# JunweiLiang/Multiverse

Measured on NVIDIA H100. Metric: trajectories/sec (obs8->pred12, K=20), higher is better.
Workload: dtype f32

## Files before the change

### include/multiverse_b200.h

```cpp
#ifndef MULTIVERSE_B200_H_
#define MULTIVERSE_B200_H_

#include <stdint.h>

#ifdef __cplusplus
extern "C" {
#endif

const char* mvb_last_error(void);
int mvb_abi_version(void);
long long mvb_launch_count(void);
void mvb_reset_launch_count(void);


int mvb_cell_cpad(int cx);

#define MVB_PLANES_F16F8 16
int mvb_pack_cell_weights(const float* kernel, const float* biases, void* w_planes,
                          float* bias_packed, int cx, int planes, int comp, void* stream);
int mvb_cell_last_variant(void);
long long mvb_cell_variants_seen(int reset);

int mvb_convlstm_cell_fwd(const void* xh_planes, const void* w_planes, const float* bias_packed,
                          const float* c_in, const int32_t* row_map, float* c_out, float* h32_out,
                          void* hp_out, int64_t hp_plane_stride, int cpad_out, int ch_off_out,
                          int64_t NS, int H, int W, int cpad, int planes, float forget_bias,
                          void* stream);

int mvb_cell_xfold_tables(const float* kernel, const float* biases, const float* We, const float* be,
                          int E, float* table_B, float* table_T2, void* stream);
int mvb_convlstm_cell_fwd_onehot(const void* xh_planes, const void* w_planes, const float* table_B,
                                 const float* table_T2, const int32_t* ids, const float* c_in,
                                 const int32_t* row_map, float* c_out, float* h32_out, void* hp_out,
                                 int64_t hp_plane_stride, int cpad_out, int ch_off_out, int64_t NS, int H,
                                 int W, int cpad, int planes, float forget_bias, void* stream);
int mvb_convlstm_cell_fwd_xdense(const void* xh_planes, const void* w_planes, const float* bias_packed,
                                 const float* x_in, const float* x_weights, const float* c_in, float* c_out,
                                 float* h32_out, void* hp_out, int64_t hp_plane_stride, int cpad_out, int ch_off_out,
                                 int64_t NS, int H, int W, int cpad, int planes, float forget_bias, void* stream);
int mvb_cell_xdense_weights(const float* kernel_tf, float* x_weights, void* stream);
int mvb_convlstm_cell_fwd_xsparse(const void* xh_planes, const void* w_planes, const float* bias_packed,
                                  const float* x_table, const int32_t* label, const float* c_in, float* c_out,
                                  float* h32_out, void* hp_out, int64_t hp_plane_stride, int cpad_out, int ch_off_out,
                                  int64_t NS, int H, int W, int cpad, int planes, float forget_bias, void* stream);
int mvb_cell_xsparse_weights(const float* kernel_tf, int cx, float* x_weights, void* stream);
int mvb_cell_xsparse_table(const float* scene_conv, const int32_t* frame_idx, const int32_t* label,
                           const float* x_weights, float* x_table, int64_t NS, int H, int W, void* stream);

int mvb_convlstm_cell_fwd_onehot_fanout(const void* xh_planes, const void* w_planes, const float* table_B,
                                        const float* table_T2, const int32_t* ids, const float* c_in,
                                        float* c_out, float* h32_out, float* workspace, int64_t NS, int fanout,
                                        int H, int W, int cpad, int planes, float forget_bias, void* stream);


int mvb_convlstm_cell_fwd_train(const void* xh_planes, const void* w_planes,
                                const float* bias_packed, const float* c_in, float* c_out,
                                float* h32_out, void* hp_out, int64_t hp_plane_stride, int cpad_out,
                                int ch_off_out, float* gates_out, int64_t NS, int H, int W, int cpad,
                                int planes, float forget_bias, void* stream);
int mvb_lstm_gates_bwd(const float* gates, const float* c_prev, const float* c_new, const float* dh,
                       const float* dc_in, void* dg_planes, int64_t plane_stride, float* dc_prev,
                       float* dbias_packed, int64_t NS, int H, int W, int planes, void* stream);
int mvb_pack_cell_weights_dgrad(const float* kernel, void* wd_planes, int cx, int planes,
                                void* stream);
int mvb_cell_dgrad(const void* dg_planes, const void* wd_planes, float* dxh, int64_t NS, int H,
                   int W, int cpad, int planes, int need_dx, void* stream);
int mvb_cell_wgrad_direct(const void* dg_planes, const void* xh_planes, float* dw_packed, int64_t NS,
                          int H, int W, int cpad, int planes, void* stream);
int mvb_unpack_cell_wgrad(const float* dw_packed, const float* dbias_packed, float* dkernel,
                          float* dbiases, int cx, int comp, int accumulate, int slabs, void* stream);
int mvb_cell_wgrad_slabs(int cpad);

int mvb_loss_fwd_bwd(const float* logits, const int32_t* labels, float* dlogits, int64_t rows, int V,
                     float cls_weight, const float* reg, const float* target, float* dreg,
                     int64_t nreg, float reg_weight, float* loss_out, void* stream);
int mvb_soft_ce_fwd_bwd(const float* logits, const float* labels, float* dlogits, int64_t rows, int V,
                        float cls_weight, float* loss_out, void* stream);
int mvb_fg_count(const float* soft_labels, const int32_t* labels, int64_t rows, int V, double* fg_count,
                 void* stream);
int mvb_masked_huber_fwd_bwd(const float* reg, const float* target, float* dreg, const float* soft_labels,
                             const int32_t* labels, int64_t rows, int V, const double* fg_count, float reg_weight,
                             float* loss_out, void* stream);
int mvb_head_bwd(const float* h32, const float* dout, const float* Wo, int Pout, float* dWo,
                 float* dh, int accumulate_dh, int64_t NS, int H, int W, void* stream);
int mvb_emb_bwd(const float* dxh, int cpad, const int32_t* ids, const float* in_map, const float* We,
                const float* be, int E, int Pout, float* dWe, float* dbe, float* d_in,
                int accumulate_din, int64_t NS, int H, int W, void* stream);
int mvb_gnn_attend_bwd(const float* h32, const float* scene_mean, const float* gout, float* work,
                       float* dh, int accumulate_dh, float* dscene_mean, int64_t NS, int H, int W,
                       void* stream);
int mvb_scene_conv_bwd(const float* in, const float* W, const float* out, const float* dout,
                       float* dW, float* db, float* din, int64_t F, int IH, int IW, int Cin, int Cout,
                       void* stream);
int mvb_enc_class_input_bwd(const float* dxh, int cpad, const int32_t* frame_idx,
                            const int32_t* label, float* dscene, int64_t NS, int H, int W,
                            void* stream);
int mvb_scene_time_mean_bwd(const float* dmean, const int32_t* frame_idx, float* dscene, int64_t N,
                            int T, int64_t HWC, void* stream);
int mvb_clip_adadelta(float* w, const float* grad, float* acc, float* acc_upd, int64_t n, float lr,
                      float rho, float eps, float clip, float wd, float grad_scale, void* stream);


int mvb_nhwc_to_planes(const float* src, void* dst_planes, int64_t plane_stride, int cpad,
                       int ch_off, int64_t NS, int H, int W, int C, int planes, int comp,
                       void* stream);
int mvb_nhwc_to_halo(const float* src, float* dst, int64_t NS, int H, int W, int C, void* stream);
int mvb_halo_to_nhwc(const float* src, float* dst, int64_t NS, int H, int W, int C, void* stream);

int mvb_enc_class_input(const float* scene_conv, const int32_t* frame_idx, const int32_t* label,
                        const int32_t* prev_label, void* xh_planes, int64_t plane_stride, int cpad,
                        int64_t NS, int H, int W, int planes, void* stream);

int mvb_scene_conv_fwd(const float* in, const float* W, const float* b, float* out, int64_t F,
                       int IH, int IW, int Cin, int Cout, void* stream);
int mvb_scene_time_mean(const float* scene_conv, const int32_t* frame_idx, float* out, int64_t N,
                        int T, int64_t HWC, void* stream);

int mvb_gnn_attend_fwd(const float* h32, const int32_t* row_map, const float* scene_mean,
                       int beam, void* hp_out, int64_t hp_plane_stride, int cpad_out,
                       int ch_off_out, int64_t NS, int H, int W, int planes, void* stream);

int mvb_head_class_fwd(const float* h32, const float* Wo, float* logits_out, int32_t* ids_out,
                       const float* We, const float* be, int E, void* xh_next,
                       int64_t plane_stride, int cpad, int64_t NS, int H, int W, int planes,
                       void* stream);
int mvb_head_class_fwd_dense(const float* h32, const float* Wo, float* logits_out, int32_t* ids_out,
                             const float* We, const float* be, int E, void* xh_next, int64_t plane_stride, int cpad,
                             int64_t NS, int H, int W, int planes, void* stream);
int mvb_head_reg_fwd(const float* h32, const float* Wo, float* off_out, const float* We,
                     const float* be, int E, void* xh_next, int64_t plane_stride, int cpad,
                     int64_t NS, int H, int W, int planes, void* stream);
int mvb_emb_onehot_fwd(const int32_t* ids, const float* We, const float* be, int E, void* xh_next,
                       int64_t plane_stride, int cpad, int64_t NS, int H, int W, int planes,
                       void* stream);
int mvb_emb_dense_fwd(const float* x, const float* We, const float* be, int E, void* xh_next,
                      int64_t plane_stride, int cpad, int64_t NS, int H, int W, int planes,
                      void* stream);

int mvb_beam_step(const float* logits, const float* score_in, float* score_out, int32_t* ids_out,
                  int32_t* parents_out, int32_t* row_map_out, int64_t N, int B, int V,
                  int first_step, int zero_scores, int diverse, float log_gamma, void* stream);
int mvb_clip_update(float* w, const float* grad, float* slot1, float* slot2, int64_t n, int kind, float lr, float p1,
                    float p2, float eps, float clip, float wd, float grad_scale, void* stream);

int mvb_adv_step(const float* x, const float* adv, const float* grad, float* out, float eps, float step, int64_t n,
                 void* stream);
int mvb_mix(const float* a, const float* b, float* out, float w, int64_t n, void* stream);
int mvb_ce_rows(const float* logits, const int32_t* labels, float* loss, int64_t rows, int V, void* stream);
int mvb_enc_class_input_mix(const float* scene_conv, const int32_t* frame_idx, const int32_t* label,
                            const int32_t* label2, float beta, void* xh_planes, int64_t plane_stride, int cpad,
                            int64_t NS, int H, int W, int planes, void* stream);
int mvb_enc_class_input_mix_bwd(const float* dxh, int cpad, const int32_t* frame_idx, const int32_t* label,
                                const int32_t* label2, float beta, float* dscene, int64_t NS, int H, int W,
                                void* stream);

int mvb_min_ade_fde(const float* pred, const float* gt, const int32_t* gt_len, double* ade_err, int32_t* ade_idx,
                    double* fde, int32_t* fde_idx, int64_t N, int G, int K, int Tp, int Tg, void* stream);
int mvb_beam_nll(const float* logits, const float* logprobs, const int32_t* gt_idx, const int32_t* steps, double* nll,
                 int32_t* count, int64_t N, int K, int Tp, int V, int J, int G, void* stream);

int mvb_beam_backtrace(const int32_t* step_ids, const int32_t* step_parents,
                       const float* step_logits, int32_t* out_ids, float* out_logits, int64_t N,
                       int B, int Tp, int V, void* stream);

int mvb_beam_gather_h_f16f8(const float* h32, const int32_t* row_map, void* hp_out, int64_t hp_plane_stride,
                            int cpad_out, int64_t NS, int H, int W, void* stream);

int mvb_traj_to_grid(const double* traj, const double* centers, double h_gap, double w_gap, int32_t* labels,
                     float* regress, int64_t NT, int H, int W, void* stream);

int mvb_decode_trajectories(const int32_t* ids, const float* offsets, const float* centers, float* out,
                            int64_t N, int K, int Tp, int V, void* stream);

#ifdef __cplusplus
}
#endif
#endif
```

### multiverse_b200/_lib.py

```python
from __future__ import annotations

import ctypes as C
import os

_HERE = os.path.dirname(os.path.abspath(__file__))
LIB_PATH = os.path.join(_HERE, "libmultiverse_b200.so")

_vp, _i, _i64, _f = C.c_void_p, C.c_int, C.c_int64, C.c_float

SIGNATURES = {
    "mvb_last_error": [],
    "mvb_abi_version": [],
    "mvb_launch_count": [],
    "mvb_reset_launch_count": [],
    "mvb_cell_cpad": [_i],
    "mvb_cell_last_variant": [],
    "mvb_cell_variants_seen": [_i],
    "mvb_pack_cell_weights": [_vp, _vp, _vp, _vp, _i, _i, _i, _vp],
    "mvb_convlstm_cell_fwd": [_vp, _vp, _vp, _vp, _vp, _vp, _vp, _vp, _i64, _i, _i, _i64, _i, _i,
                              _i, _i, _f, _vp],
    "mvb_cell_xfold_tables": [_vp, _vp, _vp, _vp, _i, _vp, _vp, _vp],
    "mvb_convlstm_cell_fwd_xdense": [_vp, _vp, _vp, _vp, _vp, _vp, _vp, _vp, _vp, _i64, _i, _i, _i64, _i, _i,
                                     _i, _i, _f, _vp],
    "mvb_cell_xdense_weights": [_vp, _vp, _vp],
    "mvb_convlstm_cell_fwd_xsparse": [_vp, _vp, _vp, _vp, _vp, _vp, _vp, _vp, _vp, _i64, _i, _i, _i64, _i, _i,
                                      _i, _i, _f, _vp],
    "mvb_cell_xsparse_weights": [_vp, _i, _vp, _vp],
    "mvb_cell_xsparse_table": [_vp, _vp, _vp, _vp, _vp, _i64, _i, _i, _vp],
    "mvb_convlstm_cell_fwd_onehot_fanout": [_vp, _vp, _vp, _vp, _vp, _vp, _vp, _vp, _vp, _i64, _i, _i, _i, _i, _i, _f, _vp],
    "mvb_convlstm_cell_fwd_onehot": [_vp, _vp, _vp, _vp, _vp, _vp, _vp, _vp, _vp, _vp, _i64, _i, _i, _i64,
                                     _i, _i, _i, _i, _f, _vp],
    "mvb_convlstm_cell_fwd_train": [_vp, _vp, _vp, _vp, _vp, _vp, _vp, _i64, _i, _i, _vp, _i64, _i, _i,
                                    _i, _i, _f, _vp],
    "mvb_lstm_gates_bwd": [_vp, _vp, _vp, _vp, _vp, _vp, _i64, _vp, _vp, _i64, _i, _i, _i, _vp],
    "mvb_pack_cell_weights_dgrad": [_vp, _vp, _i, _i, _vp],
    "mvb_cell_dgrad": [_vp, _vp, _vp, _i64, _i, _i, _i, _i, _i, _vp],
    "mvb_cell_wgrad_direct": [_vp, _vp, _vp, _i64, _i, _i, _i, _i, _vp],
    "mvb_unpack_cell_wgrad": [_vp, _vp, _vp, _vp, _i, _i, _i, _i, _vp],
    "mvb_cell_wgrad_slabs": [_i],
    "mvb_loss_fwd_bwd": [_vp, _vp, _vp, _i64, _i, _f, _vp, _vp, _vp, _i64, _f, _vp, _vp],
    "mvb_soft_ce_fwd_bwd": [_vp, _vp, _vp, _i64, _i, _f, _vp, _vp],
    "mvb_fg_count": [_vp, _vp, _i64, _i, _vp, _vp],
    "mvb_masked_huber_fwd_bwd": [_vp, _vp, _vp, _vp, _vp, _i64, _i, _vp, _f, _vp, _vp],
    "mvb_head_bwd": [_vp, _vp, _vp, _i, _vp, _vp, _i, _i64, _i, _i, _vp],
    "mvb_emb_bwd": [_vp, _i, _vp, _vp, _vp, _vp, _i, _i, _vp, _vp, _vp, _i, _i64, _i, _i, _vp],
    "mvb_gnn_attend_bwd": [_vp, _vp, _vp, _vp, _vp, _i, _vp, _i64, _i, _i, _vp],
    "mvb_scene_conv_bwd": [_vp, _vp, _vp, _vp, _vp, _vp, _vp, _i64, _i, _i, _i, _i, _vp],
    "mvb_enc_class_input_bwd": [_vp, _i, _vp, _vp, _vp, _i64, _i, _i, _vp],
    "mvb_scene_time_mean_bwd": [_vp, _vp, _vp, _i64, _i, _i64, _vp],
    "mvb_clip_adadelta": [_vp, _vp, _vp, _vp, _i64, _f, _f, _f, _f, _f, _f, _vp],
    "mvb_nhwc_to_planes": [_vp, _vp, _i64, _i, _i, _i64, _i, _i, _i, _i, _i, _vp],
    "mvb_nhwc_to_halo": [_vp, _vp, _i64, _i, _i, _i, _vp],
    "mvb_halo_to_nhwc": [_vp, _vp, _i64, _i, _i, _i, _vp],
    "mvb_enc_class_input": [_vp, _vp, _vp, _vp, _vp, _i64, _i, _i64, _i, _i, _i, _vp],
    "mvb_scene_conv_fwd": [_vp, _vp, _vp, _vp, _i64, _i, _i, _i, _i, _vp],
    "mvb_scene_time_mean": [_vp, _vp, _vp, _i64, _i, _i64, _vp],
    "mvb_gnn_attend_fwd": [_vp, _vp, _vp, _i, _vp, _i64, _i, _i, _i64, _i, _i, _i, _vp],
    "mvb_head_class_fwd": [_vp, _vp, _vp, _vp, _vp, _vp, _i, _vp, _i64, _i, _i64, _i, _i, _i, _vp],
    "mvb_head_class_fwd_dense": [_vp, _vp, _vp, _vp, _vp, _vp, _i, _vp, _i64, _i, _i64, _i, _i, _i, _vp],
    "mvb_head_reg_fwd": [_vp, _vp, _vp, _vp, _vp, _i, _vp, _i64, _i, _i64, _i, _i, _i, _vp],
    "mvb_emb_onehot_fwd": [_vp, _vp, _vp, _i, _vp, _i64, _i, _i64, _i, _i, _i, _vp],
    "mvb_emb_dense_fwd": [_vp, _vp, _vp, _i, _vp, _i64, _i, _i64, _i, _i, _i, _vp],
    "mvb_beam_step": [_vp, _vp, _vp, _vp, _vp, _vp, _i64, _i, _i, _i, _i, _i, _f, _vp],
    "mvb_traj_to_grid": [_vp, _vp, C.c_double, C.c_double, _vp, _vp, _i64, _i, _i, _vp],
    "mvb_decode_trajectories": [_vp, _vp, _vp, _vp, _i64, _i, _i, _i, _vp],
    "mvb_clip_update": [_vp, _vp, _vp, _vp, _i64, _i, _f, _f, _f, _f, _f, _f, _f, _vp],
    "mvb_adv_step": [_vp, _vp, _vp, _vp, _f, _f, _i64, _vp],
    "mvb_ce_rows": [_vp, _vp, _vp, _i64, _i, _vp],
    "mvb_enc_class_input_mix": [_vp, _vp, _vp, _vp, _f, _vp, _i64, _i, _i64, _i, _i, _i, _vp],
    "mvb_enc_class_input_mix_bwd": [_vp, _i, _vp, _vp, _vp, _f, _vp, _i64, _i, _i, _vp],
    "mvb_mix": [_vp, _vp, _vp, _f, _i64, _vp],
    "mvb_min_ade_fde": [_vp, _vp, _vp, _vp, _vp, _vp, _vp, _i64, _i, _i, _i, _i, _vp],
    "mvb_beam_nll": [_vp, _vp, _vp, _vp, _vp, _vp, _i64, _i, _i, _i, _i, _i, _vp],
    "mvb_beam_backtrace": [_vp, _vp, _vp, _vp, _vp, _i64, _i, _i, _i, _vp],
    "mvb_beam_gather_h_f16f8": [_vp, _vp, _vp, _i64, _i, _i64, _i, _i, _vp],
}
_RESTYPES = {"mvb_last_error": C.c_char_p, "mvb_launch_count": C.c_longlong, "mvb_cell_variants_seen": C.c_longlong,
             "mvb_reset_launch_count": None}

_lib = None


def load():
  global _lib
  if _lib is not None:
    return _lib
  if not os.path.exists(LIB_PATH):
    raise RuntimeError(
        "libmultiverse_b200.so is not built (%s). Run `python -m multiverse_b200.build`; "
        "there is no CPU or PyTorch fallback for the hot path." % LIB_PATH)
  lib = C.CDLL(LIB_PATH)
  for name, args in SIGNATURES.items():
    fn = getattr(lib, name)
    fn.argtypes = args
    fn.restype = _RESTYPES.get(name, C.c_int)
  _lib = lib
  return lib


def check(rc, what):
  if rc != 0:
    msg = load().mvb_last_error()
    raise RuntimeError("%s failed (code %d): %s" % (what, rc, msg.decode() if msg else "?"))


def call(name, *args):
  check(getattr(load(), name)(*args), name)
```

### multiverse_b200/csrc/mvb_api.cu

```cuda
#include "mvb_common.cuh"
#include "mvb_kernels.h"
#include "../../include/multiverse_b200.h"

#include <string.h>

namespace mvb {

static thread_local char g_err[512] = "";
static thread_local long long g_launches = 0;

void set_error(const char* fmt, ...) {
  va_list ap;
  va_start(ap, fmt);
  vsnprintf(g_err, sizeof(g_err), fmt, ap);
  va_end(ap);
}
const char* get_error() { return g_err; }
void count_launch(int n) { g_launches += n; }

typedef CUresult (*EncodeTiledFn)(CUtensorMap*, CUtensorMapDataType, cuuint32_t, void*,
                                  const cuuint64_t*, const cuuint64_t*, const cuuint32_t*,
                                  const cuuint32_t*, CUtensorMapInterleave, CUtensorMapSwizzle,
                                  CUtensorMapL2promotion, CUtensorMapFloatOOBfill);

// ... 13 lines not shown
}

static int encode_tmap_3d_any(CUtensorMapDataType dt, CUtensorMap* out, const void* base, uint64_t d0, uint64_t d1, uint64_t d2,
                        uint64_t stride1_bytes, uint64_t stride2_bytes, uint32_t b0, uint32_t b1,
                        uint32_t b2, int swizzle_bytes) {
  EncodeTiledFn fn = get_encode_fn();
  if (!fn) return MVB_ERR_DRIVER;
  cuuint64_t dims[3] = {d0, d1, d2};
  cuuint64_t strides[2] = {stride1_bytes, stride2_bytes};
  cuuint32_t box[3] = {b0, b1, b2};
  cuuint32_t estr[3] = {1, 1, 1};
  CUtensorMapSwizzle sw = swizzle_bytes == 128  ? CU_TENSOR_MAP_SWIZZLE_128B
                          : swizzle_bytes == 64 ? CU_TENSOR_MAP_SWIZZLE_64B
                          : swizzle_bytes == 32 ? CU_TENSOR_MAP_SWIZZLE_32B
                                                : CU_TENSOR_MAP_SWIZZLE_NONE;
  CUresult r = fn(out, dt, 3, const_cast<void*>(base), dims, strides,
                  box, estr, CU_TENSOR_MAP_INTERLEAVE_NONE, sw, CU_TENSOR_MAP_L2_PROMOTION_L2_256B,
                  CU_TENSOR_MAP_FLOAT_OOB_FILL_NONE);
  if (r != CUDA_SUCCESS) {
    set_error("cuTensorMapEncodeTiled failed with CUresult %d (dims %llu,%llu,%llu box %u,%u,%u)",
              (int)r, (unsigned long long)d0, (unsigned long long)d1, (unsigned long long)d2, b0,
              b1, b2);
    return MVB_ERR_DRIVER;
  }
  return MVB_OK;
}

int encode_tmap_3d_bf16(CUtensorMap* out, const void* base, uint64_t d0, uint64_t d1, uint64_t d2,
                        uint64_t stride1_bytes, uint64_t stride2_bytes, uint32_t b0, uint32_t b1,
                        uint32_t b2, int swizzle_bytes) {
  return encode_tmap_3d_any(CU_TENSOR_MAP_DATA_TYPE_BFLOAT16, out, base, d0, d1, d2, stride1_bytes, stride2_bytes,
                            b0, b1, b2, swizzle_bytes);
}
int encode_tmap_3d_u8(CUtensorMap* out, const void* base, uint64_t d0, uint64_t d1, uint64_t d2,
                      uint64_t stride1_bytes, uint64_t stride2_bytes, uint32_t b0, uint32_t b1, uint32_t b2,
                      int swizzle_bytes) {
  return encode_tmap_3d_any(CU_TENSOR_MAP_DATA_TYPE_UINT8, out, base, d0, d1, d2, stride1_bytes, stride2_bytes,
                            b0, b1, b2, swizzle_bytes);
}

static int encode_tmap_4d_any(CUtensorMapDataType dt, CUtensorMap* out, const void* base, const uint64_t (&dims)[4],
                              const uint64_t (&strides_bytes)[3], const uint32_t (&box)[4], int swizzle_bytes) {
  EncodeTiledFn fn = get_encode_fn();
  if (!fn) return MVB_ERR_DRIVER;
  cuuint64_t d[4] = {dims[0], dims[1], dims[2], dims[3]};
  cuuint64_t st[3] = {strides_bytes[0], strides_bytes[1], strides_bytes[2]};
  cuuint32_t bx[4] = {box[0], box[1], box[2], box[3]};
  cuuint32_t estr[4] = {1, 1, 1, 1};
  CUtensorMapSwizzle sw = swizzle_bytes == 128  ? CU_TENSOR_MAP_SWIZZLE_128B
                          : swizzle_bytes == 64 ? CU_TENSOR_MAP_SWIZZLE_64B
                          : swizzle_bytes == 32 ? CU_TENSOR_MAP_SWIZZLE_32B
                                                : CU_TENSOR_MAP_SWIZZLE_NONE;
  CUresult r = fn(out, dt, 4, const_cast<void*>(base), d, st, bx, estr,
                  CU_TENSOR_MAP_INTERLEAVE_NONE, sw, CU_TENSOR_MAP_L2_PROMOTION_L2_256B,
                  CU_TENSOR_MAP_FLOAT_OOB_FILL_NONE);
  if (r != CUDA_SUCCESS) {
    set_error("cuTensorMapEncodeTiled(4d) failed with CUresult %d (dims %llu,%llu,%llu,%llu)", (int)r,
              (unsigned long long)dims[0], (unsigned long long)dims[1], (unsigned long long)dims[2],
              (unsigned long long)dims[3]);
    return MVB_ERR_DRIVER;
  }
  return MVB_OK;
}

int encode_tmap_4d_bf16(CUtensorMap* out, const void* base, const uint64_t (&dims)[4],
                        const uint64_t (&strides_bytes)[3], const uint32_t (&box)[4],
                        int swizzle_bytes) {
  return encode_tmap_4d_any(CU_TENSOR_MAP_DATA_TYPE_BFLOAT16, out, base, dims, strides_bytes, box, swizzle_bytes);
}
int encode_tmap_4d_u8(CUtensorMap* out, const void* base, const uint64_t (&dims)[4],
                      const uint64_t (&strides_bytes)[3], const uint32_t (&box)[4], int swizzle_bytes) {
  return encode_tmap_4d_any(CU_TENSOR_MAP_DATA_TYPE_UINT8, out, base, dims, strides_bytes, box, swizzle_bytes);
}

}

using namespace mvb;

static inline cudaStream_t S(void* s) { return reinterpret_cast<cudaStream_t>(s); }

extern "C" {

const char* mvb_last_error(void) { return get_error(); }
int mvb_abi_version(void) { return 14; }
int mvb_cell_last_variant(void) { return cell_last_variant(); }
long long mvb_cell_variants_seen(int reset) { return (long long)cell_variants_seen(reset); }
long long mvb_launch_count(void) { return g_launches; }
void mvb_reset_launch_count(void) { g_launches = 0; }

int mvb_cell_cpad(int cx) { return (cx + 31) / 32 * 32 + kHidden; }

int mvb_pack_cell_weights(const float* kernel, const float* biases, void* w_planes,
                          float* bias_packed, int cx, int planes, int comp, void* stream) {
  return pack_cell_weights(kernel, biases, w_planes, bias_packed, cx, planes, comp, S(stream));
}

int mvb_convlstm_cell_fwd(const void* xh_planes, const void* w_planes, const float* bias_packed,
                          const float* c_in, const int32_t* row_map, float* c_out, float* h32_out,
                          void* hp_out, int64_t hp_plane_stride, int cpad_out, int ch_off_out,
                          int64_t NS, int H, int W, int cpad, int planes, float forget_bias,
                          void* stream) {
  CellStep s{};
  s.xh = xh_planes; s.w = w_planes; s.bias = bias_packed; s.c_in = c_in; s.row_map = row_map; s.c_out = c_out;
  s.h32_out = h32_out; s.hp_out = hp_out; s.hp_plane_stride = hp_plane_stride; s.cpad_out = cpad_out;
  s.ch_off_out = ch_off_out; s.NS = NS; s.H = H; s.W = W; s.cpad = cpad; s.planes = planes; s.forget_bias = forget_bias;
  return cell_fwd(s, S(stream));
}
int mvb_cell_xfold_tables(const float* kernel, const float* biases, const float* We, const float* be,
                          int E, float* table_B, float* table_T2, void* stream) {
  return cell_xfold_tables(kernel, biases, We, be, E, table_B, table_T2, S(stream));
}
int mvb_convlstm_cell_fwd_onehot(const void* xh_planes, const void* w_planes, const float* table_B,
                                 const float* table_T2, const int32_t* ids, const float* c_in,
                                 const int32_t* row_map, float* c_out, float* h32_out, void* hp_out,
                                 int64_t hp_plane_stride, int cpad_out, int ch_off_out, int64_t NS, int H,
                                 int W, int cpad, int planes, float forget_bias, void* stream) {
  CellStep s{};
  s.xh = xh_planes; s.w = w_planes; s.xf_B = table_B; s.xf_T2 = table_T2; s.xf_ids = ids; s.c_in = c_in;
  s.row_map = row_map; s.c_out = c_out; s.h32_out = h32_out; s.hp_out = hp_out; s.hp_plane_stride = hp_plane_stride;
  s.cpad_out = cpad_out; s.ch_off_out = ch_off_out; s.NS = NS; s.H = H; s.W = W; s.cpad = cpad; s.planes = planes;
  s.forget_bias = forget_bias;
  return cell_fwd(s, S(stream));
}
int mvb_convlstm_cell_fwd_xdense(const void* xh_planes, const void* w_planes, const float* bias_packed,
                                 const float* x_in, const float* x_weights, const float* c_in, float* c_out,
                                 float* h32_out, void* hp_out, int64_t hp_plane_stride, int cpad_out, int ch_off_out,
                                 int64_t NS, int H, int W, int cpad, int planes, float forget_bias, void* stream) {
  MVB_REQUIRE(x_in && x_weights, "mvb_convlstm_cell_fwd_xdense: null x input / weights");
  CellStep s{};
  s.xh = xh_planes; s.w = w_planes; s.bias = bias_packed; s.xr_in = x_in; s.xr_W = x_weights; s.c_in = c_in;
  s.c_out = c_out; s.h32_out = h32_out; s.hp_out = hp_out; s.hp_plane_stride = hp_plane_stride; s.cpad_out = cpad_out;
  s.ch_off_out = ch_off_out; s.NS = NS; s.H = H; s.W = W; s.cpad = cpad; s.planes = planes; s.forget_bias = forget_bias;
  return cell_fwd(s, S(stream));
}
int mvb_cell_xdense_weights(const float* kernel_tf, float* x_weights, void* stream) {
  return cell_xdense_weights(kernel_tf, x_weights, S(stream));
}
int mvb_convlstm_cell_fwd_xsparse(const void* xh_planes, const void* w_planes, const float* bias_packed,
                                  const float* x_table, const int32_t* label, const float* c_in, float* c_out,
                                  float* h32_out, void* hp_out, int64_t hp_plane_stride, int cpad_out, int ch_off_out,
                                  int64_t NS, int H, int W, int cpad, int planes, float forget_bias, void* stream) {
  MVB_REQUIRE(x_table && label, "mvb_convlstm_cell_fwd_xsparse: null table / labels");
  CellStep s{};
  s.xh = xh_planes; s.w = w_planes; s.bias = bias_packed; s.xs_tab = x_table; s.xs_label = label; s.c_in = c_in;
  s.c_out = c_out; s.h32_out = h32_out; s.hp_out = hp_out; s.hp_plane_stride = hp_plane_stride; s.cpad_out = cpad_out;
  s.ch_off_out = ch_off_out; s.NS = NS; s.H = H; s.W = W; s.cpad = cpad; s.planes = planes; s.forget_bias = forget_bias;
  return cell_fwd(s, S(stream));
}
int mvb_cell_xsparse_weights(const float* kernel_tf, int cx, float* x_weights, void* stream) {
  return cell_xsparse_weights(kernel_tf, cx, x_weights, S(stream));
}
int mvb_cell_xsparse_table(const float* scene_conv, const int32_t* frame_idx, const int32_t* label,
                           const float* x_weights, float* x_table, int64_t NS, int H, int W, void* stream) {
  return cell_xsparse_table(scene_conv, frame_idx, label, x_weights, x_table, NS, H, W, S(stream));
}
int mvb_convlstm_cell_fwd_onehot_fanout(const void* xh_planes, const void* w_planes, const float* table_B,
                                        const float* table_T2, const int32_t* ids, const float* c_in,
                                        float* c_out, float* h32_out, float* workspace, int64_t NS, int fanout, int H,
                                        int W, int cpad, int planes, float forget_bias, void* stream) {
  CellStep s{};
  s.xh = xh_planes; s.w = w_planes; s.xf_B = table_B; s.xf_T2 = table_T2; s.xf_ids = ids; s.c_in = c_in;
  s.c_out = c_out; s.h32_out = h32_out; s.fanout_ws = workspace; s.NS = NS; s.fanout = fanout; s.H = H; s.W = W;
  s.cpad = cpad; s.planes = planes; s.forget_bias = forget_bias;
  return cell_fwd(s, S(stream));
}

int mvb_convlstm_cell_fwd_train(const void* xh_planes, const void* w_planes,
                                const float* bias_packed, const float* c_in, float* c_out,
                                float* h32_out, void* hp_out, int64_t hp_plane_stride, int cpad_out,
                                int ch_off_out, float* gates_out, int64_t NS, int H, int W, int cpad,
                                int planes, float forget_bias, void* stream) {
  CellStep s{};
  s.xh = xh_planes; s.w = w_planes; s.bias = bias_packed; s.c_in = c_in; s.c_out = c_out; s.h32_out = h32_out;
  s.hp_out = hp_out; s.hp_plane_stride = hp_plane_stride; s.cpad_out = cpad_out; s.ch_off_out = ch_off_out;
  s.gates_out = gates_out; s.NS = NS; s.H = H; s.W = W; s.cpad = cpad; s.planes = planes; s.forget_bias = forget_bias;
  return cell_fwd(s, S(stream));
}
int mvb_lstm_gates_bwd(const float* gates, const float* c_prev, const float* c_new, const float* dh,
                       const float* dc_in, void* dg_planes, int64_t plane_stride, float* dc_prev,
                       float* dbias_packed, int64_t NS, int H, int W, int planes, void* stream) {
  return lstm_gates_bwd(gates, c_prev, c_new, dh, dc_in, dg_planes, plane_stride, dc_prev,
                        dbias_packed, NS, H, W, planes, S(stream));
}
int mvb_pack_cell_weights_dgrad(const float* kernel, void* wd_planes, int cx, int planes,
                                void* stream) {
  return pack_cell_weights_dgrad(kernel, wd_planes, cx, planes, S(stream));
}
int mvb_cell_dgrad(const void* dg_planes, const void* wd_planes, float* dxh, int64_t NS, int H,
                   int W, int cpad, int planes, int need_dx, void* stream) {
  return cell_dgrad(dg_planes, wd_planes, dxh, NS, H, W, cpad, planes, need_dx, S(stream));
}
int mvb_cell_wgrad_direct(const void* dg_planes, const void* xh_planes, float* dw_packed, int64_t NS,
                          int H, int W, int cpad, int planes, void* stream) {
  return cell_wgrad_mn(dg_planes, xh_planes, dw_packed, NS, H, W, cpad, planes, S(stream));
}
int mvb_unpack_cell_wgrad(const float* dw_packed, const float* dbias_packed, float* dkernel,
                          float* dbiases, int cx, int comp, int accumulate, int slabs, void* stream) {
  return unpack_cell_wgrad(dw_packed, dbias_packed, dkernel, dbiases, cx, comp, accumulate, slabs,
                           S(stream));
}
int mvb_cell_wgrad_slabs(int cpad) { return cell_wgrad_mn_slabs(cpad); }

int mvb_loss_fwd_bwd(const float* logits, const int32_t* labels, float* dlogits, int64_t rows, int V,
                     float cls_weight, const float* reg, const float* target, float* dreg,
// ... 91 lines not shown
int mvb_head_class_fwd(const float* h32, const float* Wo, float* logits_out, int32_t* ids_out,
                       const float* We, const float* be, int E, void* xh_next,
                       int64_t plane_stride, int cpad, int64_t NS, int H, int W, int planes,
                       void* stream) {
  return head_fwd(h32, Wo, 1, logits_out, ids_out, We, be, E, xh_next, plane_stride, cpad, NS, H,
                  W, planes, S(stream));
}
int mvb_head_class_fwd_dense(const float* h32, const float* Wo, float* logits_out, int32_t* ids_out,
                             const float* We, const float* be, int E, void* xh_next, int64_t plane_stride, int cpad,
                             int64_t NS, int H, int W, int planes, void* stream) {
  return head_class_fwd_dense(h32, Wo, logits_out, ids_out, We, be, E, xh_next, plane_stride, cpad, NS, H, W,
                              planes, S(stream));
}
int mvb_head_reg_fwd(const float* h32, const float* Wo, float* off_out, const float* We,
                     const float* be, int E, void* xh_next, int64_t plane_stride, int cpad,
                     int64_t NS, int H, int W, int planes, void* stream) {
  return head_fwd(h32, Wo, 2, off_out, nullptr, We, be, E, xh_next, plane_stride, cpad, NS, H, W,
                  planes, S(stream));
}
int mvb_emb_onehot_fwd(const int32_t* ids, const float* We, const float* be, int E, void* xh_next,
                       int64_t plane_stride, int cpad, int64_t NS, int H, int W, int planes,
                       void* stream) {
  return emb_onehot_fwd(ids, We, be, E, xh_next, plane_stride, cpad, NS, H, W, planes, S(stream));
}
int mvb_emb_dense_fwd(const float* x, const float* We, const float* be, int E, void* xh_next,
                      int64_t plane_stride, int cpad, int64_t NS, int H, int W, int planes,
                      void* stream) {
  return emb_dense_fwd(x, We, be, E, xh_next, plane_stride, cpad, NS, H, W, planes, S(stream));
}

int mvb_beam_step(const float* logits, const float* score_in, float* score_out, int32_t* ids_out,
                  int32_t* parents_out, int32_t* row_map_out, int64_t N, int B, int V,
                  int first_step, int zero_scores, int diverse, float log_gamma, void* stream) {
  return beam_step(logits, score_in, score_out, ids_out, parents_out, row_map_out, N, B, V,
                   first_step, zero_scores, diverse, log_gamma, S(stream));
}
int mvb_decode_trajectories(const int32_t* ids, const float* offsets, const float* centers, float* out,
                            int64_t N, int K, int Tp, int V, void* stream) {
  return decode_trajectories(ids, offsets, centers, out, N, K, Tp, V, S(stream));
}
int mvb_clip_update(float* w, const float* grad, float* slot1, float* slot2, int64_t n, int kind, float lr, float p1,
                    float p2, float eps, float clip, float wd, float grad_scale, void* stream) {
  return clip_update(w, grad, slot1, slot2, n, kind, lr, p1, p2, eps, clip, wd, grad_scale, S(stream));
}
int mvb_adv_step(const float* x, const float* adv, const float* grad, float* out, float eps, float step, int64_t n,
                 void* stream) {
  return adv_step(x, adv, grad, out, eps, step, n, S(stream));
}
int mvb_mix(const float* a, const float* b, float* out, float w, int64_t n, void* stream) {
  return mix(a, b, out, w, n, S(stream));
}
int mvb_ce_rows(const float* logits, const int32_t* labels, float* loss, int64_t rows, int V, void* stream) {
  return ce_rows(logits, labels, loss, rows, V, S(stream));
}
int mvb_enc_class_input_mix(const float* scene_conv, const int32_t* frame_idx, const int32_t* label,
                            const int32_t* label2, float beta, void* xh_planes, int64_t plane_stride, int cpad,
                            int64_t NS, int H, int W, int planes, void* stream) {
  return enc_class_input_mix(scene_conv, frame_idx, label, label2, beta, xh_planes, plane_stride, cpad, NS, H, W,
                             planes, S(stream));
}
int mvb_enc_class_input_mix_bwd(const float* dxh, int cpad, const int32_t* frame_idx, const int32_t* label,
                                const int32_t* label2, float beta, float* dscene, int64_t NS, int H, int W,
                                void* stream) {
  return enc_class_input_mix_bwd(dxh, cpad, frame_idx, label, label2, beta, dscene, NS, H, W, S(stream));
}
int mvb_min_ade_fde(const float* pred, const float* gt, const int32_t* gt_len, double* ade_err, int32_t* ade_idx,
                    double* fde, int32_t* fde_idx, int64_t N, int G, int K, int Tp, int Tg, void* stream) {
  return min_ade_fde(pred, gt, gt_len, ade_err, ade_idx, fde, fde_idx, N, G, K, Tp, Tg, S(stream));
}
int mvb_beam_nll(const float* logits, const float* logprobs, const int32_t* gt_idx, const int32_t* steps, double* nll,
                 int32_t* count, int64_t N, int K, int Tp, int V, int J, int G, void* stream) {
  return beam_nll(logits, logprobs, gt_idx, steps, nll, count, N, K, Tp, V, J, G, S(stream));
}
int mvb_beam_backtrace(const int32_t* step_ids, const int32_t* step_parents,
                       const float* step_logits, int32_t* out_ids, float* out_logits, int64_t N,
                       int B, int Tp, int V, void* stream) {
  return beam_backtrace(step_ids, step_parents, step_logits, out_ids, out_logits, N, B, Tp, V,
                        S(stream));
}
int mvb_beam_gather_h_f16f8(const float* h32, const int32_t* row_map, void* hp_out, int64_t hp_plane_stride,
                            int cpad_out, int64_t NS, int H, int W, void* stream) {
  return beam_gather_h(h32, row_map, hp_out, hp_plane_stride, cpad_out, NS, H, W, S(stream));
}

}
```

### multiverse_b200/csrc/mvb_beam.cu

```cuda
#include <cstdlib>
#include "mvb_common.cuh"
#include "mvb_kernels.h"

namespace mvb {

constexpr int BEAM_THREADS = 256;

__device__ __forceinline__ void block_argmax(float& v, int& i, float* red_v, int* red_i) {
  const int warp = threadIdx.x >> 5, lane = threadIdx.x & 31;
#pragma unroll
  for (int o = 16; o > 0; o >>= 1) {
    const float ov = __shfl_xor_sync(0xffffffffu, v, o);
    const int oi = __shfl_xor_sync(0xffffffffu, i, o);
    if (ov > v || (ov == v && oi < i)) { v = ov; i = oi; }
  }
  if (lane == 0) { red_v[warp] = v; red_i[warp] = i; }
  __syncthreads();
  if (threadIdx.x == 0) {
    float bv = red_v[0]; int bi = red_i[0];
    for (int w = 1; w < BEAM_THREADS / 32; ++w)
      if (red_v[w] > bv || (red_v[w] == bv && red_i[w] < bi)) { bv = red_v[w]; bi = red_i[w]; }
    red_v[0] = bv; red_i[0] = bi;
  }
  __syncthreads();
// ... 179 lines not shown
    const int id = ids[i];
    const float2 c = *reinterpret_cast<const float2*>(centers + 2 * id);
    const float2 o = *reinterpret_cast<const float2*>(offs + (((long long)t * N + n) * V + id) * 2);
    *reinterpret_cast<float2*>(out + 2 * i) = make_float2(c.x + o.x, c.y + o.y);
  }
}

int decode_trajectories(const int* ids, const float* offs, const float* centers, float* out, long long N,
                        int K, int Tp, int V, cudaStream_t stream) {
  MVB_REQUIRE(ids && offs && centers && out && N > 0 && K > 0 && Tp > 0 && V > 0, "decode_trajectories: bad args");
  const long long total = N * K * Tp;
  const int blocks = (int)((total + 255) / 256 < sm_count() * 8 ? (total + 255) / 256 : sm_count() * 8);
  decode_traj_kernel<<<blocks, 256, 0, stream>>>(ids, offs, centers, out, N, K, Tp, V);
  MVB_CHECK_CUDA(cudaGetLastError());
  count_launch(1);
  return MVB_OK;
}

int beam_step(const float* logits, const float* score_in, float* score_out, int* ids_out,
              int* parents_out, int* row_map_out, long long N, int B, int V, int first_step,
              int zero_scores, int diverse, float log_gamma, cudaStream_t stream) {
  MVB_REQUIRE(logits && score_out && ids_out && parents_out && row_map_out, "beam_step: null pointer");
  MVB_REQUIRE(N > 0 && B >= 1 && V >= B, "beam_step: bad sizes N=%lld B=%d V=%d", N, B, V);
  const char* full = getenv("MVB_BEAM_FULL_RANK");
  if ((!diverse || log_gamma <= 0.f) && !(full && full[0] == '1')) {
    const size_t smem_t = sizeof(float) * ((size_t)B * V + 2 * (size_t)B * B);
    MVB_REQUIRE(smem_t <= 227 * 1024, "beam_step: B*V=%d too large for shared memory", B * V);
    static SmemOptIn opt_t;
    if (smem_t > 48 * 1024) MVB_CHECK_CUDA(smem_opt_in(opt_t, beam_step_topk_kernel, smem_t));
    beam_step_topk_kernel<<<(unsigned)N, BEAM_THREADS, smem_t, stream>>>(logits, score_in, score_out, ids_out,
                                                                         parents_out, row_map_out, B, V, first_step,
                                                                         zero_scores, diverse, log_gamma);
    MVB_CHECK_CUDA(cudaGetLastError());
    count_launch(1);
    return MVB_OK;
  }
  const size_t smem = sizeof(float) * 2 * (size_t)B * V;
  MVB_REQUIRE(smem <= 227 * 1024, "beam_step: B*V=%d too large for shared memory", B * V);
  static SmemOptIn opt;
  if (smem > 48 * 1024) MVB_CHECK_CUDA(smem_opt_in(opt, beam_step_kernel, smem));
  beam_step_kernel<<<(unsigned)N, BEAM_THREADS, smem, stream>>>(logits, score_in, score_out, ids_out,
                                                                parents_out, row_map_out, B, V, first_step,
                                                                zero_scores, diverse, log_gamma);
  MVB_CHECK_CUDA(cudaGetLastError());
  count_launch(1);
  return MVB_OK;
}

__global__ void __launch_bounds__(256)
beam_gather_h_kernel(const float* __restrict__ h32, const int* __restrict__ row_map, __nv_bfloat16* __restrict__ hp_out,
                     long long plane_stride, int cpad_out, long long cells, Grid g) {
  const int lane = threadIdx.x & 31;
  const long long cell = (long long)blockIdx.x * 8 + (threadIdx.x >> 5);
  if (cell >= cells) return;
  const long long hw = (long long)g.H * g.W;
  const long long s = cell / hw;
  const int p = (int)(cell - s * hw);
  const int y = p / g.W, x = p - y * g.W;
  const long long off = (long long)y * g.Wp + x;
  const float4* src = reinterpret_cast<const float4*>(h32 + ((long long)row_map[s] * g.S + off) * kHidden + lane * 8);
  const float4 a = __ldg(src), b = __ldg(src + 1);
  const float v[8] = {a.x, a.y, a.z, a.w, b.x, b.y, b.z, b.w};
  store_f16f8_x8(hp_out, plane_stride, s * g.S + off, cpad_out - kHidden + lane * 8, cpad_out, v);
}

int beam_gather_h(const float* h32, const int* row_map, void* hp_out, long long hp_plane_stride, int cpad_out,
                  long long NS, int H, int W, cudaStream_t stream) {
  MVB_REQUIRE(h32 && row_map && hp_out, "beam_gather_h: null pointer");
  MVB_REQUIRE(NS > 0 && H > 0 && W > 0, "beam_gather_h: bad sizes NS=%lld H=%d W=%d", NS, H, W);
  MVB_REQUIRE(cpad_out >= kHidden && cpad_out % 32 == 0,
              "beam_gather_h: cpad_out=%d is not an operand pitch (a multiple of 32, >= 256)", cpad_out);
  const Grid g = make_grid(H, W);
  MVB_REQUIRE(hp_plane_stride == NS * g.S * (long long)cpad_out,
              "beam_gather_h: plane stride %lld is not NS*(H+1)*(W+1)*cpad_out", hp_plane_stride);
  const long long cells = NS * H * W;
  MVB_REQUIRE((cells + 7) / 8 < (1ll << 31), "beam_gather_h: NS=%lld too large", NS);
  beam_gather_h_kernel<<<(unsigned)((cells + 7) / 8), 256, 0, stream>>>(
      h32, row_map, reinterpret_cast<__nv_bfloat16*>(hp_out), hp_plane_stride, cpad_out, cells, g);
  MVB_CHECK_CUDA(cudaGetLastError());
  count_launch(1);
  return MVB_OK;
}

int beam_backtrace(const int* step_ids, const int* step_parents, const float* step_logits,
                   int* out_ids, float* out_logits, long long N, int B, int Tp, int V,
                   cudaStream_t stream) {
  MVB_REQUIRE(step_ids && step_parents && step_logits && out_ids && out_logits, "beam_backtrace: null pointer");
  MVB_REQUIRE(N > 0 && B >= 1 && Tp >= 1 && V >= 1, "beam_backtrace: bad sizes");
  beam_backtrace_kernel<<<(unsigned)(N * B), 256, sizeof(int) * Tp, stream>>>(
      step_ids, step_parents, step_logits, out_ids, out_logits, N, B, Tp, V);
  MVB_CHECK_CUDA(cudaGetLastError());
  count_launch(1);
  return MVB_OK;
}

}
```

### multiverse_b200/csrc/mvb_cell.cu

```cuda
#include "mvb_common.cuh"
#include "mvb_kernels.h"
#include <stdlib.h>

namespace mvb {

constexpr int BLOCK_M = 128;
constexpr int BLOCK_N = 256;
constexpr int XPAD = 32;
constexpr int kMaxXBlock = 256;
constexpr int CHUNK = 64;
constexpr int ROW_BYTES = 128;
constexpr int MMA_K = 16;
constexpr int TILE_CH = 64;
constexpr int N_TILES = kGates / BLOCK_N;
constexpr int NUM_THREADS = 384;
constexpr int B_SLOT_BYTES = BLOCK_N * ROW_BYTES;
constexpr uint32_t SW128_LAYOUT = kSwizzle128B;
constexpr uint32_t SW128_SBO = 8 * ROW_BYTES;

constexpr int kSmemLimit = 227 * 1024;
constexpr int kSmemExtra = 1024  + 512 ;
constexpr int kMaxBSlots = 8;
constexpr int kMaxAStages = 4;
static_assert((2 * kMaxBSlots + 2 * kMaxAStages) * 8 <= 512, "the barrier area holds every ring's barriers");

struct CellRing {
  int b_slots, a_stages, a_stage_bytes;
  constexpr int smem_bytes() const { return b_slots * B_SLOT_BYTES + a_stages * a_stage_bytes + kSmemExtra; }
};

template <int FMT>
struct CellCfg {
  static constexpr int MAX_RA8 = 256;
  static constexpr CellRing ring(int ra8) {
    if (FMT == 0) {
      const int a = kBf16Planes * ra8 * ROW_BYTES;
      return CellRing{(4 * B_SLOT_BYTES + 2 * a + 2048 <= kSmemLimit) ? 4 : 3, 2, a};
    }
    const int a = ra8 * ROW_BYTES;
    int b = (kSmemLimit - kSmemExtra - 2 * a) / B_SLOT_BYTES;
    if (b > kMaxBSlots) b = kMaxBSlots;
    return CellRing{b, CellRing{b, 3, a}.smem_bytes() <= kSmemLimit ? 3 : 2, a};
  }
};
static_assert(CellCfg<1>::ring(168).b_slots == 5 && CellCfg<1>::ring(168).a_stages == 3, "36x18: 5 slots, 3 stages");
static_assert(CellCfg<1>::ring(152).b_slots == 5 && CellCfg<1>::ring(152).a_stages == 3, "18x9: 5 slots, 3 stages");
static_assert(CellCfg<1>::ring(200).b_slots == 5 && CellCfg<1>::ring(200).a_stages == 2, "18x32: 5 slots, 2 stages");
static_assert(CellCfg<1>::ring(256).b_slots == 5 && CellCfg<1>::ring(256).a_stages == 2 &&
              CellCfg<1>::ring(256).smem_bytes() <= kSmemLimit, "4x62: 5 slots, 2 stages");
static_assert(CellCfg<0>::ring(168).b_slots == 4 && CellCfg<0>::ring(200).b_slots == 3, "bf16x2 rings unchanged");

enum CellProbePhase {
  kProbeFullWait, kProbeAFullWait, kProbeMmaWait, kProbeEpilogue, kProbeConsumer,
  kProbeEmptyWait, kProbeAEmptyWait, kProbeProducer,
  kProbeFreeWait, kProbeStagedWait, kProbeEpiBusy,
  kProbeTiles, kProbePhases
};
#ifdef MVB_CELL_PROBE
__device__ unsigned long long g_cell_probe[kProbePhases];
#define CELL_PROBE(...) __VA_ARGS__
#define CELL_PROBED(ph, ...) do { const long long t0_ = clock64(); __VA_ARGS__; probe[ph] += clock64() - t0_; } while (0)
#else
#define CELL_PROBE(...)
#define CELL_PROBED(ph, ...) __VA_ARGS__
#endif

struct CellParams {
  const float* bias;
  const float* col_scale;
  const float* c_in;
  const int* row_map;
  float* c_out;
  float* h32_out;
  float* gates_out;
  const float* xf_B;
  const float* xf_T2;
  const int* xf_ids;
  int skip_x;
  const float* xs_tab;
  const int* xs_label;
  const float* xr_in;
  const float* xr_W;
  int order;
  CellRing ring;
  float* preact_out;
  int hp_mixed;
  __nv_bfloat16* hp_out;
  long long hp_plane_stride;
  int cpad_out;
  int ch_off_out;
  long long R;
  int H, W;
  int cpad;
  float forget_bias;
};

struct GateOut { float ai, aj, af, ao, c, h; };
__device__ __forceinline__ GateOut lstm_update(float xi, float xj, float xf, float xo, float cprev, float forget_bias) {
  GateOut r;
  r.ai = sigmoid_acc(xi); r.aj = tanh_acc(xj); r.af = sigmoid_acc(__fadd_rn(xf, forget_bias)); r.ao = sigmoid_acc(xo);
  r.c = __fmaf_rn(r.af, cprev, __fmul_rn(r.ai, r.aj));
  r.h = __fmul_rn(tanh_acc(r.c), r.ao);
  return r;
}
template <int FMT>
__device__ __forceinline__ float preact(float acc, float scale, float q) {
  return FMT ? __fmaf_rn(acc, scale, q) : __fadd_rn(acc, q);
}

struct EpiRow {
  long long row, src_row, psmp;
  int py, px;
  bool valid;
  const float* xfb;
  const float* xft;
};

__device__ __forceinline__ EpiRow epi_row(const CellParams& prm, const Grid& g, long long row) {
  EpiRow r;
  r.row = row; r.src_row = row; r.psmp = 0; r.py = 0; r.px = 0; r.xfb = nullptr; r.xft = nullptr;
  r.valid = row < prm.R;
  if (!r.valid) return r;
  const long long smp = row / g.S;
  const int rem = (int)(row - smp * g.S);
  const int y = rem / g.Wp, x = rem - y * g.Wp;
  r.valid = (x < g.W) && (y < g.H);
  if (!r.valid) return r;
  if (prm.row_map) r.src_row = (long long)prm.row_map[smp] * g.S + rem;
  r.py = y; r.px = x; r.psmp = smp;
  if (prm.xf_B) {
    const int cy = y == 0 ? 0 : (y == g.H - 1 ? 2 : 1), cx = x == 0 ? 0 : (x == g.W - 1 ? 2 : 1);
    r.xfb = prm.xf_B + (cy * 3 + cx) * kGates;
    const int a = prm.xf_ids[smp];
    const int ay = a / g.W, ax = a - ay * g.W;
    const int ry = y - ay, rx = x - ax;
    if (ry >= -2 && ry <= 2 && rx >= -2 && rx <= 2) {
      const int acy = ay == 0 ? 0 : (ay == g.H - 1 ? 2 : 1), acx = ax == 0 ? 0 : (ax == g.W - 1 ? 2 : 1);
      r.xft = prm.xf_T2 + ((long long)(acy * 3 + acx) * 25 + (ry + 2) * 5 + (rx + 2)) * kGates;
    }
  }
  if (prm.xs_tab) {
    const int l = prm.xs_label[smp];
    if (l >= 0 && l < g.H * g.W) {
      const int ly = l / g.W, dy = ly - y, dx = (l - ly * g.W) - x;
      if (dy >= -1 && dy <= 1 && dx >= -1 && dx <= 1)
        r.xft = prm.xs_tab + ((long long)smp * 9 + (dy + 1) * 3 + (dx + 1)) * kGates;
    }
  }
  return r;
}

__device__ __forceinline__ float2 epi_cprev(const CellParams& prm, const EpiRow& r, int ch) {
  return (prm.c_in && !prm.preact_out && r.valid)
             ? __ldg(reinterpret_cast<const float2*>(prm.c_in + r.src_row * kHidden + ch)) : make_float2(0.f, 0.f);
}

struct EpiIn { float q[4][2], sc[4][2]; };
template <int FMT>
__device__ __forceinline__ EpiIn epi_inputs(const CellParams& prm, const Grid& g, const EpiRow& r, int nt, int j) {
  EpiIn in = {};
  if (prm.preact_out || !r.valid) return in;
  const int col = nt * BLOCK_N + j;
  const float* bptr = (r.xfb ? r.xfb : prm.bias) + col;
  float (&q)[4][2] = in.q;
#pragma unroll
  for (int gt = 0; gt < 4; ++gt) {
    const float2 b = __ldg(reinterpret_cast<const float2*>(bptr + gt * TILE_CH));
    q[gt][0] = b.x; q[gt][1] = b.y;
  }
  if (r.xft) {
#pragma unroll
    for (int gt = 0; gt < 4; ++gt) {
      const float2 t = __ldg(reinterpret_cast<const float2*>(r.xft + col + gt * TILE_CH));
      q[gt][0] = __fadd_rn(q[gt][0], t.x); q[gt][1] = __fadd_rn(q[gt][1], t.y);
    }
  }
  if (prm.xr_W) {
#pragma unroll 1
    for (int k = 0; k < 18; ++k) {
      const int tp = k >> 1, yy = r.py + tp / 3 - 1, xx = r.px + tp % 3 - 1;
      const float xk = (yy >= 0 && yy < g.H && xx >= 0 && xx < g.W)
                           ? __ldg(prm.xr_in + ((r.psmp * g.H + yy) * g.W + xx) * 2 + (k & 1)) : 0.f;
#pragma unroll
      for (int gt = 0; gt < 4; ++gt) {
        const float2 w = __ldg(reinterpret_cast<const float2*>(prm.xr_W + k * kGates + col + gt * TILE_CH));
        q[gt][0] = __fmaf_rn(xk, w.x, q[gt][0]); q[gt][1] = __fmaf_rn(xk, w.y, q[gt][1]);
      }
    }
  }
  if (FMT == 1) {
#pragma unroll
    for (int gt = 0; gt < 4; ++gt) {
      const float2 s2 = __ldg(reinterpret_cast<const float2*>(prm.col_scale + col + gt * TILE_CH));
      in.sc[gt][0] = s2.x; in.sc[gt][1] = s2.y;
    }
  }
  return in;
}

template <int FMT>
__device__ __forceinline__ void epi_pair(const CellParams& prm, const EpiRow& r, int nt, int j, const float (&a)[4][2],
                                         float2 cprev, const EpiIn& in) {
  const int col = nt * BLOCK_N + j;
  const int ch = nt * TILE_CH + j;
  if (prm.preact_out) {
    float* gp = prm.preact_out + r.row * kGates + col;
#pragma unroll
    for (int gt = 0; gt < 4; ++gt) *reinterpret_cast<float2*>(gp + gt * TILE_CH) = make_float2(a[gt][0], a[gt][1]);
    return;
  }
  const float (&q)[4][2] = in.q;
  const float (&sc)[4][2] = in.sc;
  GateOut o[2];
#pragma unroll
  for (int e = 0; e < 2; ++e)
    o[e] = lstm_update(preact<FMT>(a[0][e], sc[0][e], q[0][e]), preact<FMT>(a[1][e], sc[1][e], q[1][e]),
                       preact<FMT>(a[2][e], sc[2][e], q[2][e]), preact<FMT>(a[3][e], sc[3][e], q[3][e]),
                       e ? cprev.y : cprev.x, prm.forget_bias);
  if (prm.gates_out) {
    float* gp = prm.gates_out + r.row * kGates + col;
    *reinterpret_cast<float2*>(gp + 0 * TILE_CH) = make_float2(o[0].ai, o[1].ai);
    *reinterpret_cast<float2*>(gp + 1 * TILE_CH) = make_float2(o[0].aj, o[1].aj);
    *reinterpret_cast<float2*>(gp + 2 * TILE_CH) = make_float2(o[0].af, o[1].af);
    *reinterpret_cast<float2*>(gp + 3 * TILE_CH) = make_float2(o[0].ao, o[1].ao);
  }
  *reinterpret_cast<float2*>(prm.c_out + r.row * kHidden + ch) = make_float2(o[0].c, o[1].c);
  if (prm.h32_out) *reinterpret_cast<float2*>(prm.h32_out + r.row * kHidden + ch) = make_float2(o[0].h, o[1].h);
  if (prm.hp_out && prm.hp_mixed) {
    uint32_t h2, e0, e1;
    split_f16f8_x2(o[0].h, o[1].h, h2, e0, e1);
    const int c = prm.ch_off_out + ch;
    *reinterpret_cast<uint32_t*>(reinterpret_cast<__half*>(prm.hp_out) + r.row * prm.cpad_out + c) = h2;
    uint8_t* b8 = reinterpret_cast<uint8_t*>(prm.hp_out) + 2 * prm.hp_plane_stride + r.row * 2 * prm.cpad_out;
    *reinterpret_cast<uint16_t*>(b8 + f8_off(c, 0, prm.cpad_out)) = (uint16_t)e0;
    *reinterpret_cast<uint16_t*>(b8 + f8_off(c, 1, prm.cpad_out)) = (uint16_t)e1;
  } else if (prm.hp_out) {
    __nv_bfloat16 p0[kBf16Planes], p1[kBf16Planes];
    split_planes(o[0].h, p0);
    split_planes(o[1].h, p1);
#pragma unroll
    for (int p = 0; p < kBf16Planes; ++p)
      *reinterpret_cast<uint32_t*>(prm.hp_out + p * prm.hp_plane_stride + r.row * prm.cpad_out + prm.ch_off_out + ch) =
          pack_bf16x2(p0[p], p1[p]);
  }
}

__device__ __forceinline__ void x_chunk_steps(int q, int cxp, int cpad, int& ks16, int& ks8, uint32_t& poff) {
  const int c16 = q * CHUNK, width = cxp - c16 < CHUNK ? cxp - c16 : CHUNK;
  ks16 = width / MMA_K;
  ks8 = width / 32;
  poff = (uint32_t)(f8_off(c16, 1, cpad) - f8_off(c16, 0, cpad)) >> 4;
}

template <bool MC, int FMT>
__global__ void __launch_bounds__(NUM_THREADS, 1)
cell_fwd_kernel(const __grid_constant__ CUtensorMap tmA, const __grid_constant__ CUtensorMap tmB,
                const __grid_constant__ CUtensorMap tmA8, const __grid_constant__ CUtensorMap tmB8,
                const CellParams prm) {
  extern __shared__ uint8_t smem_raw[];
  const uint32_t raw_addr = smem_u32(smem_raw);
  uint8_t* smem = smem_raw + ((1024u - (raw_addr & 1023u)) & 1023u);
  const int ra8 = (BLOCK_M + 2 * (prm.W + 2) + 7) & ~7;
  const int a_stage_bytes = prm.ring.a_stage_bytes;
  const int a_load_bytes = FMT ? ra8 * ROW_BYTES : a_stage_bytes;
  const int b_slots = prm.ring.b_slots, a_stages = prm.ring.a_stages;
  uint8_t* smem_a = smem + b_slots * B_SLOT_BYTES;
  uint64_t* full_bar = reinterpret_cast<uint64_t*>(smem_a + a_stages * a_stage_bytes);
  uint64_t* empty_bar = full_bar + kMaxBSlots;
  uint64_t* afull_bar = empty_bar + kMaxBSlots;
  uint64_t* aempty_bar = afull_bar + kMaxAStages;
  CELL_PROBE(long long probe[kProbePhases] = {};)

  const int warp = threadIdx.x >> 5;
  const int lane = threadIdx.x & 31;
  const int wg = warp >> 2;
  const Grid g = make_grid(prm.H, prm.W);
  const int cxp = prm.cpad - kHidden;
  const int nqx = (cxp + CHUNK - 1) / CHUNK;
  const int q_begin = prm.skip_x ? nqx : 0;
  const int NQ = nqx + kHidden / CHUNK;
  constexpr int NPASS = FMT ? 2 : 1;
  constexpr int NS = FMT ? 1 : kBf16Planes;
  const long long num_m_tiles = (prm.R + BLOCK_M - 1) / BLOCK_M;
  const uint32_t rank = MC ? cluster_ctarank() : 0u;
  const long long num_tiles = (MC ? (num_m_tiles + 1) / 2 : num_m_tiles) * N_TILES;
  const long long w_begin = MC ? (long long)(blockIdx.x >> 1) : (long long)blockIdx.x;
  const long long w_step = MC ? (long long)(gridDim.x >> 1) : (long long)gridDim.x;
  auto work_index = [&](long long it) -> long long {
    return prm.order ? (w_begin + (it / N_TILES) * w_step) * N_TILES + it % N_TILES : w_begin + it * w_step;
  };
  auto tile_m0 = [&](long long w) -> long long { return ((w / N_TILES) * (MC ? 2 : 1) + rank) * BLOCK_M; };

  if (warp == 0 && lane == 0) {
    prefetch_tmap(&tmA);
    prefetch_tmap(&tmB);
    if (FMT == 1) { prefetch_tmap(&tmA8); prefetch_tmap(&tmB8); }
#pragma unroll 1
    for (int s = 0; s < b_slots; ++s) { mbar_init(&full_bar[s], 1); mbar_init(&empty_bar[s], MC ? 4 : 2); }
#pragma unroll 1
    for (int s = 0; s < a_stages; ++s) { mbar_init(&afull_bar[s], 1); mbar_init(&aempty_bar[s], 2); }
    fence_barrier_init();
  }
  __syncthreads();
  if (MC) cluster_sync_all();

  if (wg == 0) {
    regs_dealloc<40>();
    if (warp == 0 && lane == 0) {
      int slot = 0, astage = 0; uint32_t phase = 0, aphase = 0;
      CELL_PROBE(const long long probe_t0 = clock64();)
      for (long long it = 0, t; (t = work_index(it)) < num_tiles; ++it) {
        const long long m0 = tile_m0(t);
        const int n0 = (int)(t % N_TILES) * BLOCK_N;
        for (int pass = 0; pass < NPASS; ++pass)
        for (int q = q_begin; q < NQ; ++q) {
          const int c16 = q < nqx ? q * CHUNK : cxp + (q - nqx) * CHUNK;
          const int c8 = f8_off(c16, 0, prm.cpad);
          const bool f8 = FMT == 1 && pass == 0;
          CELL_PROBED(kProbeAEmptyWait, mbar_wait(&aempty_bar[astage], aphase ^ 1));
          uint8_t* sa = smem_a + astage * a_stage_bytes;
          mbar_expect_tx(&afull_bar[astage], a_load_bytes);
          if (f8) tma_load_3d(sa, &tmA8, &afull_bar[astage], c8, (int)(m0 - g.Wp - 1), 0);
          else tma_load_3d(sa, &tmA, &afull_bar[astage], c16, (int)(m0 - g.Wp - 1), 0);
          if (++astage == a_stages) { astage = 0; aphase ^= 1; }
          for (int tap = 0; tap < 9; ++tap) {
#pragma unroll
            for (int sl = 0; sl < NS; ++sl) {
              CELL_PROBED(kProbeEmptyWait, mbar_wait(&empty_bar[slot], phase ^ 1));
              uint8_t* sb = smem + slot * B_SLOT_BYTES;
              mbar_expect_tx(&full_bar[slot], B_SLOT_BYTES);
              const CUtensorMap* tm = f8 ? &tmB8 : &tmB;
              const int kcol = f8 ? tap * 2 * prm.cpad + c8 : tap * prm.cpad + c16;
              if (MC) tma_load_3d_mc(sb + rank * (B_SLOT_BYTES / 2), tm, &full_bar[slot], kcol,
                                     n0 + (int)rank * (BLOCK_N / 2), sl, (uint16_t)3);
              else tma_load_3d(sb, tm, &full_bar[slot], kcol, n0, sl);
              if (++slot == b_slots) { slot = 0; phase ^= 1; }
            }
          }
        }
      }
#ifdef MVB_CELL_PROBE
      atomicAdd(&g_cell_probe[kProbeEmptyWait], (unsigned long long)probe[kProbeEmptyWait]);
      atomicAdd(&g_cell_probe[kProbeAEmptyWait], (unsigned long long)probe[kProbeAEmptyWait]);
      atomicAdd(&g_cell_probe[kProbeProducer], (unsigned long long)(clock64() - probe_t0));
#endif
    }
  } else {
    regs_alloc<232>();
    const int c = wg - 1;
    const bool leader = (threadIdx.x & 127) == 0;
    constexpr uint32_t kHi = smem_desc_hi(SW128_SBO, SW128_LAYOUT);
    const uint32_t a_plane_lo = (uint32_t)(ra8 * ROW_BYTES) >> 4;
    const uint32_t a_wg_lo = (uint32_t)(64 * c) * (ROW_BYTES >> 4);
    int slot = 0, astage = 0; uint32_t phase = 0, aphase = 0;
    float acc[128];
    int rel_slot = -1, rel_astage = -1;
    auto release = [&]() {
      if (leader && rel_slot >= 0) {
        if (MC) { mbar_arrive_remote(&empty_bar[rel_slot], 0); mbar_arrive_remote(&empty_bar[rel_slot], 1); }
        else mbar_arrive(&empty_bar[rel_slot]);
        if (rel_astage >= 0) mbar_arrive(&aempty_bar[rel_astage]);
      }
      rel_slot = -1; rel_astage = -1;
    };
    CELL_PROBE(const long long probe_t0 = clock64();)
    for (long long it = 0, t; (t = work_index(it)) < num_tiles; ++it) {
      CELL_PROBE(++probe[kProbeTiles];)
      const long long m0 = tile_m0(t);
      const int nt = (int)(t % N_TILES);
      uint32_t fresh = 1;
      auto mma16 = [&](uint32_t a_lo, uint32_t b_lo) {
        if (FMT == 1) wgmma_f16<256, 0, 0>(acc, desc_of(a_lo, kHi), desc_of(b_lo, kHi), fresh ^ 1u);
        else wgmma_bf16<256, 0, 0>(acc, desc_of(a_lo, kHi), desc_of(b_lo, kHi), fresh ^ 1u);
        fresh = 0;
      };
      auto mma8 = [&](uint32_t a_lo, uint32_t b_lo) {
        wgmma_e4m3_n256(acc, desc_of(a_lo, kHi), desc_of(b_lo, kHi), fresh ^ 1u);
        fresh = 0;
      };
      for (int pass = 0; pass < NPASS; ++pass)
      for (int q = q_begin; q < NQ; ++q) {
        const bool f8 = FMT == 1 && pass == 0;
        CELL_PROBED(kProbeAFullWait, mbar_wait(&afull_bar[astage], aphase));
        const uint32_t sa_lo = (smem_u32(smem_a + astage * a_stage_bytes) >> 4) + a_wg_lo;
        for (int tap = 0; tap < 9; ++tap) {
          const uint32_t a_lo = sa_lo + (uint32_t)((tap / 3) * g.Wp + (tap % 3)) * (ROW_BYTES >> 4);
#pragma unroll
          for (int sl = 0; sl < NS; ++sl) {
            CELL_PROBED(kProbeFullWait, mbar_wait(&full_bar[slot], phase));
            const uint32_t b_lo = smem_u32(smem + slot * B_SLOT_BYTES) >> 4;
            wgmma_fence_regs(acc);
            wgmma_fence();
            if (q >= nqx) {
              if (f8) {
                for (int k = 0; k < 4; ++k) mma8(a_lo + 2 * k, b_lo + 2 * k);
              } else {
#pragma unroll
                for (int pa = 0; pa < (FMT ? 1 : kBf16Planes - sl); ++pa)
#pragma unroll
                  for (int k = 0; k < 4; ++k) mma16(a_lo + pa * a_plane_lo + 2 * k, b_lo + 2 * k);
              }
            } else {
              int ks16, ks8; uint32_t poff;
              x_chunk_steps(q, cxp, prm.cpad, ks16, ks8, poff);
              if (f8) {
                for (int pk = 0; pk < 2 * ks8; ++pk) {
                  const uint32_t o = (pk / ks8) * poff + (pk % ks8) * 2;
                  mma8(a_lo + o, b_lo + o);
                }
              } else {
                for (int pa = 0; pa < (FMT ? 1 : kBf16Planes - sl); ++pa)
                  for (int k = 0; k < ks16; ++k) mma16(a_lo + pa * a_plane_lo + 2 * k, b_lo + 2 * k);
              }
            }
            wgmma_commit();
            wgmma_fence_regs(acc);
            CELL_PROBED(kProbeMmaWait, wgmma_wait<1>());
            release();
            rel_slot = slot;
            if (tap == 8 && sl == NS - 1) rel_astage = astage;
            if (++slot == b_slots) { slot = 0; phase ^= 1; }
          }
        }
        if (++astage == a_stages) { astage = 0; aphase ^= 1; }
      }
      CELL_PROBE(const long long probe_e0 = clock64();)
      const long long rbase = m0 + 64 * c + 16 * (warp & 3) + (lane >> 2);
      EpiRow rows[2];
      float2 cprev[2][8];
#pragma unroll
      for (int hr = 0; hr < 2; ++hr) {
        rows[hr] = epi_row(prm, g, rbase + 8 * hr);
#pragma unroll
        for (int ip = 0; ip < 8; ++ip) cprev[hr][ip] = epi_cprev(prm, rows[hr], nt * TILE_CH + 8 * ip + 2 * (lane & 3));
      }
      CELL_PROBE(const long long probe_w0 = clock64();)
      wgmma_wait<0>();
      CELL_PROBE(const long long probe_w = clock64() - probe_w0; probe[kProbeMmaWait] += probe_w;)
      wgmma_fence_regs(acc);
      release();
#pragma unroll
      for (int ip = 0; ip < 8; ++ip) {
        const int j = 8 * ip + 2 * (lane & 3);
        EpiIn in[2];
#pragma unroll
        for (int hr = 0; hr < 2; ++hr) in[hr] = epi_inputs<FMT>(prm, g, rows[hr], nt, j);
#pragma unroll
        for (int hr = 0; hr < 2; ++hr) {
          if (!rows[hr].valid) continue;
          float a[4][2];
#pragma unroll
          for (int gt = 0; gt < 4; ++gt) {
            a[gt][0] = acc[4 * (8 * gt + ip) + 2 * hr];
            a[gt][1] = acc[4 * (8 * gt + ip) + 2 * hr + 1];
          }
          epi_pair<FMT>(prm, rows[hr], nt, j, a, cprev[hr][ip], in[hr]);
        }
      }
      CELL_PROBE(probe[kProbeEpilogue] += clock64() - probe_e0 - probe_w;)
    }
#ifdef MVB_CELL_PROBE
    if (leader) {
      for (int p = kProbeFullWait; p <= kProbeEpilogue; ++p) atomicAdd(&g_cell_probe[p], (unsigned long long)probe[p]);
      atomicAdd(&g_cell_probe[kProbeConsumer], (unsigned long long)(clock64() - probe_t0));
      atomicAdd(&g_cell_probe[kProbeTiles], (unsigned long long)probe[kProbeTiles]);
    }
#endif
  }

  __syncthreads();
  if (MC) cluster_sync_all();
}

constexpr int EW_BLOCK_N = 128;
constexpr int EW_TILE_CH = EW_BLOCK_N / 4;
constexpr int EW_N_TILES = kGates / EW_BLOCK_N;
constexpr int EW_THREADS = 512;
constexpr int EW_SLOT_BYTES = EW_BLOCK_N * ROW_BYTES;
constexpr int EW_STAGING_BYTES = BLOCK_M * EW_BLOCK_N * 4;
constexpr int kEwRegsProducer = 40, kEwRegsMma = 152, kEwRegsEpi = 168;
static_assert(128 * (kEwRegsProducer + 2 * kEwRegsMma + kEwRegsEpi) <= 65536, "the four warpgroups fit the register file");

struct CellEpiCfg {
  static constexpr int slots(int a, int stages) {
    const int b = (kSmemLimit - kSmemExtra - EW_STAGING_BYTES - stages * a) / EW_SLOT_BYTES;
    return b > kMaxBSlots ? kMaxBSlots : b;
  }
  static constexpr CellRing ring(int ra8) {
    const int a = ra8 * ROW_BYTES;
    return slots(a, 3) >= 6 ? CellRing{slots(a, 3), 3, a} : CellRing{slots(a, 2), 2, a};
  }
  static constexpr int smem_bytes(const CellRing& r) {
    return EW_STAGING_BYTES + r.b_slots * EW_SLOT_BYTES + r.a_stages * r.a_stage_bytes + kSmemExtra;
  }
};
static_assert((2 * kMaxBSlots + 2 * kMaxAStages + 2) * 8 <= 512, "the barrier area holds the staging barriers too");
static_assert(CellEpiCfg::ring(168).b_slots == 6 && CellEpiCfg::ring(168).a_stages == 3 &&
              CellEpiCfg::smem_bytes(CellEpiCfg::ring(168)) <= kSmemLimit, "36x18: 6 slots, 3 stages");
static_assert(CellEpiCfg::ring(152).b_slots == 6 && CellEpiCfg::ring(152).a_stages == 3 &&
              CellEpiCfg::smem_bytes(CellEpiCfg::ring(152)) <= kSmemLimit, "18x9: 6 slots, 3 stages");
static_assert(CellEpiCfg::ring(200).b_slots == 6 && CellEpiCfg::ring(200).a_stages == 2 && CellEpiCfg::smem_bytes(CellEpiCfg::ring(200)) <= kSmemLimit,
              "18x32: 6 slots, 2 stages");
static_assert(CellEpiCfg::ring(256).b_slots == 6 && CellEpiCfg::ring(256).a_stages == 2 && CellEpiCfg::smem_bytes(CellEpiCfg::ring(256)) <= kSmemLimit,
              "4x62: 6 slots, 2 stages");

__device__ __forceinline__ int staging_off(int r, int col) {
  return r * EW_BLOCK_N + ((((col >> 2) ^ ((r & 3) << 1))) << 2) + (col & 3);
}

template <bool MC>
__global__ void __launch_bounds__(EW_THREADS, 1)
cell_fwd_epi_kernel(const __grid_constant__ CUtensorMap tmA, const __grid_constant__ CUtensorMap tmB,
                    const __grid_constant__ CUtensorMap tmA8, const __grid_constant__ CUtensorMap tmB8,
                    const CellParams prm) {
  extern __shared__ uint8_t smem_raw[];
  const uint32_t raw_addr = smem_u32(smem_raw);
  uint8_t* smem = smem_raw + ((1024u - (raw_addr & 1023u)) & 1023u);
  const int ra8 = (BLOCK_M + 2 * (prm.W + 2) + 7) & ~7;
  const int a_stage_bytes = prm.ring.a_stage_bytes;
  const int b_slots = prm.ring.b_slots, a_stages = prm.ring.a_stages;
  float* staging = reinterpret_cast<float*>(smem);
  uint8_t* smem_b = smem + EW_STAGING_BYTES;
  uint8_t* smem_a = smem_b + b_slots * EW_SLOT_BYTES;
  uint64_t* full_bar = reinterpret_cast<uint64_t*>(smem_a + a_stages * a_stage_bytes);
  uint64_t* empty_bar = full_bar + kMaxBSlots;
  uint64_t* afull_bar = empty_bar + kMaxBSlots;
  uint64_t* aempty_bar = afull_bar + kMaxAStages;
  uint64_t* staged_bar = aempty_bar + kMaxAStages;
  uint64_t* free_bar = staged_bar + 1;
  CELL_PROBE(long long probe[kProbePhases] = {};)

  const int warp = threadIdx.x >> 5;
  const int lane = threadIdx.x & 31;
  const int wg = warp >> 2;
  const Grid g = make_grid(prm.H, prm.W);
  const int cxp = prm.cpad - kHidden;
  const int nqx = (cxp + CHUNK - 1) / CHUNK;
  const int q_begin = prm.skip_x ? nqx : 0;
  const int NQ = nqx + kHidden / CHUNK;
  const long long num_m_tiles = (prm.R + BLOCK_M - 1) / BLOCK_M;
  const uint32_t rank = MC ? cluster_ctarank() : 0u;
  const long long num_tiles = (MC ? (num_m_tiles + 1) / 2 : num_m_tiles) * EW_N_TILES;
  const long long w_begin = MC ? (long long)(blockIdx.x >> 1) : (long long)blockIdx.x;
  const long long w_step = MC ? (long long)(gridDim.x >> 1) : (long long)gridDim.x;
  auto work_index = [&](long long it) -> long long {
    return prm.order ? (w_begin + (it / EW_N_TILES) * w_step) * EW_N_TILES + it % EW_N_TILES : w_begin + it * w_step;
  };
  auto tile_m0 = [&](long long w) -> long long { return ((w / EW_N_TILES) * (MC ? 2 : 1) + rank) * BLOCK_M; };

  if (warp == 0 && lane == 0) {
    prefetch_tmap(&tmA); prefetch_tmap(&tmB); prefetch_tmap(&tmA8); prefetch_tmap(&tmB8);
#pragma unroll 1
    for (int s = 0; s < b_slots; ++s) { mbar_init(&full_bar[s], 1); mbar_init(&empty_bar[s], MC ? 4 : 2); }
#pragma unroll 1
    for (int s = 0; s < a_stages; ++s) { mbar_init(&afull_bar[s], 1); mbar_init(&aempty_bar[s], 2); }
    mbar_init(staged_bar, 256);
    mbar_init(free_bar, 128);
    fence_barrier_init();
  }
  __syncthreads();
  if (MC) cluster_sync_all();

  if (wg == 0) {
    regs_dealloc<kEwRegsProducer>();
    if (warp == 0 && lane == 0) {
      int slot = 0, astage = 0; uint32_t phase = 0, aphase = 0;
      CELL_PROBE(const long long probe_t0 = clock64();)
      for (long long it = 0, t; (t = work_index(it)) < num_tiles; ++it) {
        const long long m0 = tile_m0(t);
        const int nt = (int)(t % EW_N_TILES);
        const int half = nt & 1, tg0 = (nt >> 1) * 4;
        for (int pass = 0; pass < 2; ++pass)
        for (int q = q_begin; q < NQ; ++q) {
          const int c16 = q < nqx ? q * CHUNK : cxp + (q - nqx) * CHUNK;
          const int c8 = f8_off(c16, 0, prm.cpad);
          const bool f8 = pass == 0;
          CELL_PROBED(kProbeAEmptyWait, mbar_wait(&aempty_bar[astage], aphase ^ 1));
          uint8_t* sa = smem_a + astage * a_stage_bytes;
          mbar_expect_tx(&afull_bar[astage], a_stage_bytes);
          if (f8) tma_load_3d(sa, &tmA8, &afull_bar[astage], c8, (int)(m0 - g.Wp - 1), 0);
          else tma_load_3d(sa, &tmA, &afull_bar[astage], c16, (int)(m0 - g.Wp - 1), 0);
          if (++astage == a_stages) { astage = 0; aphase ^= 1; }
          for (int tap = 0; tap < 9; ++tap) {
            CELL_PROBED(kProbeEmptyWait, mbar_wait(&empty_bar[slot], phase ^ 1));
            uint8_t* sb = smem_b + slot * EW_SLOT_BYTES;
            mbar_expect_tx(&full_bar[slot], EW_SLOT_BYTES);
            const CUtensorMap* tm = f8 ? &tmB8 : &tmB;
            const int kcol = f8 ? tap * 2 * prm.cpad + c8 : tap * prm.cpad + c16;
            if (MC) tma_load_4d_mc(sb + rank * (EW_SLOT_BYTES / 2), tm, &full_bar[slot], kcol, 0, half,
                                   tg0 + 2 * (int)rank, (uint16_t)3);
            else tma_load_4d(sb, tm, &full_bar[slot], kcol, 0, half, tg0);
            if (++slot == b_slots) { slot = 0; phase ^= 1; }
          }
        }
      }
#ifdef MVB_CELL_PROBE
      atomicAdd(&g_cell_probe[kProbeEmptyWait], (unsigned long long)probe[kProbeEmptyWait]);
      atomicAdd(&g_cell_probe[kProbeAEmptyWait], (unsigned long long)probe[kProbeAEmptyWait]);
      atomicAdd(&g_cell_probe[kProbeProducer], (unsigned long long)(clock64() - probe_t0));
#endif
    }
  } else if (wg < 3) {
    regs_alloc<kEwRegsMma>();
    const int c = wg - 1;
    const bool leader = (threadIdx.x & 127) == 0;
    constexpr uint32_t kHi = smem_desc_hi(SW128_SBO, SW128_LAYOUT);
    const uint32_t a_wg_lo = (uint32_t)(64 * c) * (ROW_BYTES >> 4);
    int slot = 0, astage = 0; uint32_t phase = 0, aphase = 0, free_phase = 0;
    float acc[64];
    constexpr int D = 2;
    int rq_slot[D], rq_astage[D];
#pragma unroll
    for (int i = 0; i < D; ++i) { rq_slot[i] = -1; rq_astage[i] = -1; }
    auto release_one = [&](int rs, int ra) {
      if (leader && rs >= 0) {
        if (MC) { mbar_arrive_remote(&empty_bar[rs], 0); mbar_arrive_remote(&empty_bar[rs], 1); }
        else mbar_arrive(&empty_bar[rs]);
        if (ra >= 0) mbar_arrive(&aempty_bar[ra]);
      }
    };
    CELL_PROBE(const long long probe_t0 = clock64();)
    for (long long it = 0, t; (t = work_index(it)) < num_tiles; ++it) {
      CELL_PROBE(++probe[kProbeTiles];)
      uint32_t fresh = 1;
      for (int pass = 0; pass < 2; ++pass)
      for (int q = q_begin; q < NQ; ++q) {
        const bool f8 = pass == 0;
        CELL_PROBED(kProbeAFullWait, mbar_wait(&afull_bar[astage], aphase));
        const uint32_t sa_lo = (smem_u32(smem_a + astage * a_stage_bytes) >> 4) + a_wg_lo;
        for (int tap = 0; tap < 9; ++tap) {
          const uint32_t a_lo = sa_lo + (uint32_t)((tap / 3) * g.Wp + (tap % 3)) * (ROW_BYTES >> 4);
          CELL_PROBED(kProbeFullWait, mbar_wait(&full_bar[slot], phase));
          const uint32_t b_lo = smem_u32(smem_b + slot * EW_SLOT_BYTES) >> 4;
          wgmma_fence_regs(acc);
          wgmma_fence();
          if (q >= nqx) {
            if (f8) {
              for (int k = 0; k < 4; ++k) {
                wgmma_e4m3_n128(acc, desc_of(a_lo + 2 * k, kHi), desc_of(b_lo + 2 * k, kHi), fresh ^ 1u);
                fresh = 0;
              }
            } else {
#pragma unroll
              for (int k = 0; k < 4; ++k) {
                wgmma_f16<128, 0, 0>(acc, desc_of(a_lo + 2 * k, kHi), desc_of(b_lo + 2 * k, kHi), fresh ^ 1u);
                fresh = 0;
              }
            }
          } else {
            int ks16, ks8; uint32_t poff;
            x_chunk_steps(q, cxp, prm.cpad, ks16, ks8, poff);
            if (f8) {
              for (int pk = 0; pk < 2 * ks8; ++pk) {
                const uint32_t o = (pk / ks8) * poff + (pk % ks8) * 2;
                wgmma_e4m3_n128(acc, desc_of(a_lo + o, kHi), desc_of(b_lo + o, kHi), fresh ^ 1u);
                fresh = 0;
              }
            } else {
              for (int k = 0; k < ks16; ++k) {
                wgmma_f16<128, 0, 0>(acc, desc_of(a_lo + 2 * k, kHi), desc_of(b_lo + 2 * k, kHi), fresh ^ 1u);
                fresh = 0;
              }
            }
          }
          wgmma_commit();
          wgmma_fence_regs(acc);
          CELL_PROBED(kProbeMmaWait, wgmma_wait<D>());
          release_one(rq_slot[0], rq_astage[0]);
#pragma unroll
          for (int i = 0; i + 1 < D; ++i) { rq_slot[i] = rq_slot[i + 1]; rq_astage[i] = rq_astage[i + 1]; }
          rq_slot[D - 1] = slot;
          rq_astage[D - 1] = tap == 8 ? astage : -1;
          if (++slot == b_slots) { slot = 0; phase ^= 1; }
        }
        if (++astage == a_stages) { astage = 0; aphase ^= 1; }
      }
      CELL_PROBED(kProbeMmaWait, wgmma_wait<0>());
      wgmma_fence_regs(acc);
#pragma unroll
      for (int i = 0; i < D; ++i) { release_one(rq_slot[i], rq_astage[i]); rq_slot[i] = -1; rq_astage[i] = -1; }
      CELL_PROBED(kProbeFreeWait, mbar_wait(free_bar, free_phase ^ 1));
      free_phase ^= 1;
      CELL_PROBE(const long long probe_e0 = clock64();)
      const int r0 = 64 * c + 16 * (warp & 3) + (lane >> 2);
#pragma unroll
      for (int i = 0; i < EW_BLOCK_N / 8; ++i)
#pragma unroll
        for (int hr = 0; hr < 2; ++hr)
          *reinterpret_cast<float2*>(staging + staging_off(r0 + 8 * hr, 8 * i + 2 * (lane & 3))) =
              make_float2(acc[4 * i + 2 * hr], acc[4 * i + 2 * hr + 1]);
      mbar_arrive(staged_bar);
      CELL_PROBE(probe[kProbeEpilogue] += clock64() - probe_e0;)
    }
#ifdef MVB_CELL_PROBE
    if (leader) {
      for (int p = kProbeFullWait; p <= kProbeEpilogue; ++p) atomicAdd(&g_cell_probe[p], (unsigned long long)probe[p]);
      atomicAdd(&g_cell_probe[kProbeFreeWait], (unsigned long long)probe[kProbeFreeWait]);
      atomicAdd(&g_cell_probe[kProbeConsumer], (unsigned long long)(clock64() - probe_t0));
      atomicAdd(&g_cell_probe[kProbeTiles], (unsigned long long)probe[kProbeTiles]);
    }
#endif
  } else {
    regs_alloc<kEwRegsEpi>();
    const int ew = warp & 3, lc = 2 * (lane & 3);
    uint32_t staged_phase = 0;
    CELL_PROBE(const long long probe_t0 = clock64();)
    for (long long it = 0, t; (t = work_index(it)) < num_tiles; ++it) {
      const long long m0 = tile_m0(t);
      const int nt = (int)(t % EW_N_TILES);
      const int tn = nt >> 1, jh = (nt & 1) * EW_TILE_CH;
      const int rb = 32 * ew + (lane >> 2);
#pragma unroll 1
      for (int k2 = 0; k2 < 4; k2 += 2) {
        EpiRow rows[2];
        float2 cprev[2][4];
#pragma unroll
        for (int hr = 0; hr < 2; ++hr) {
          rows[hr] = epi_row(prm, g, m0 + rb + 8 * (k2 + hr));
#pragma unroll
          for (int ip = 0; ip < 4; ++ip) cprev[hr][ip] = epi_cprev(prm, rows[hr], tn * TILE_CH + jh + 8 * ip + lc);
        }
        if (k2 == 0) {
          CELL_PROBED(kProbeStagedWait, mbar_wait(staged_bar, staged_phase));
          staged_phase ^= 1;
        }
#pragma unroll
        for (int ip = 0; ip < 4; ++ip) {
          const int j = jh + 8 * ip + lc;
          EpiIn in[2];
#pragma unroll
          for (int hr = 0; hr < 2; ++hr) in[hr] = epi_inputs<1>(prm, g, rows[hr], tn, j);
#pragma unroll
          for (int hr = 0; hr < 2; ++hr) {
            if (!rows[hr].valid) continue;
            float a[4][2];
#pragma unroll
            for (int gt = 0; gt < 4; ++gt) {
              const float2 v = *reinterpret_cast<const float2*>(
                  staging + staging_off(rb + 8 * (k2 + hr), gt * EW_TILE_CH + 8 * ip + lc));
              a[gt][0] = v.x; a[gt][1] = v.y;
            }
            epi_pair<1>(prm, rows[hr], tn, j, a, cprev[hr][ip], in[hr]);
          }
        }
      }
      mbar_arrive(free_bar);
    }
#ifdef MVB_CELL_PROBE
    if ((threadIdx.x & 127) == 0) {
      atomicAdd(&g_cell_probe[kProbeStagedWait], (unsigned long long)probe[kProbeStagedWait]);
      atomicAdd(&g_cell_probe[kProbeEpiBusy],
                (unsigned long long)(clock64() - probe_t0 - probe[kProbeStagedWait]));
    }
#endif
  }

  __syncthreads();
  if (MC) cluster_sync_all();
}

template <int FMT>
__global__ void __launch_bounds__(256)
fanout_children_kernel(const float* __restrict__ acc, const float* __restrict__ col_scale,
                       const float* __restrict__ xf_B, const float* __restrict__ xf_T2, const int* __restrict__ ids,
                       const float* __restrict__ c_in, float* __restrict__ c_out, float* __restrict__ h32_out,
                       long long NS, int K, Grid g, float forget_bias) {
  const long long wid = (blockIdx.x * (long long)blockDim.x + threadIdx.x) >> 5;
  const int lane = threadIdx.x & 31;
  const int hw = g.H * g.W;
  if (wid >= NS * hw) return;
  const long long smp = wid / hw;
  const int cell = (int)(wid - smp * hw);
  const int y = cell / g.W, x = cell - y * g.W;
  const int rem = y * g.Wp + x;
  const long long prow = smp * g.S + rem;
  const int ch0 = lane * 8;
  const int col0 = (ch0 / TILE_CH) * BLOCK_N + ch0 % TILE_CH;
  const int cy = y == 0 ? 0 : (y == g.H - 1 ? 2 : 1), cx = x == 0 ? 0 : (x == g.W - 1 ? 2 : 1);
  float a[4][8], q0[4][8], sc[4][8], cp[8];
#pragma unroll
  for (int gt = 0; gt < 4; ++gt) {
    const float4* ap = reinterpret_cast<const float4*>(acc + prow * kGates + col0 + gt * TILE_CH);
    const float4* bp = reinterpret_cast<const float4*>(xf_B + (cy * 3 + cx) * kGates + col0 + gt * TILE_CH);
    const float4* sp = reinterpret_cast<const float4*>((FMT ? col_scale : xf_B) + col0 + gt * TILE_CH);
#pragma unroll
    for (int v = 0; v < 2; ++v) {
      const float4 av = __ldg(ap + v), bv = __ldg(bp + v), sv = __ldg(sp + v);
      a[gt][4 * v] = av.x; a[gt][4 * v + 1] = av.y; a[gt][4 * v + 2] = av.z; a[gt][4 * v + 3] = av.w;
      q0[gt][4 * v] = bv.x; q0[gt][4 * v + 1] = bv.y; q0[gt][4 * v + 2] = bv.z; q0[gt][4 * v + 3] = bv.w;
      sc[gt][4 * v] = sv.x; sc[gt][4 * v + 1] = sv.y; sc[gt][4 * v + 2] = sv.z; sc[gt][4 * v + 3] = sv.w;
    }
  }
  {
    const float4* cq = reinterpret_cast<const float4*>(c_in + prow * kHidden + ch0);
    const float4 c0 = __ldg(cq), c1 = __ldg(cq + 1);
    cp[0] = c0.x; cp[1] = c0.y; cp[2] = c0.z; cp[3] = c0.w; cp[4] = c1.x; cp[5] = c1.y; cp[6] = c1.z; cp[7] = c1.w;
  }
  for (int k = 0; k < K; ++k) {
    const long long osmp = smp * K + k;
    const int id = ids[osmp];
    const int ay = id / g.W, ax = id - ay * g.W;
// ... 218 lines not shown
static int launch_cell_epi(const CellMaps& tm, const CellParams& prm_in, int num_sms, bool multicast,
                           cudaStream_t stream) {
  CellParams prm = prm_in;
  static SmemOptIn opt_plain, opt_mc;
  const int ra8 = (BLOCK_M + 2 * (prm.W + 2) + 7) & ~7;
  prm.ring = CellEpiCfg::ring(ra8);
  const int smem_bytes = CellEpiCfg::smem_bytes(prm.ring);
  MVB_REQUIRE(ra8 <= CellCfg<1>::MAX_RA8 && smem_bytes <= kSmemLimit && prm.ring.b_slots >= 2,
              "cell_fwd: grid width W=%d too large (A stage of %d rows: %d weight slots, %d B shared memory)",
              prm.W, ra8, prm.ring.b_slots, smem_bytes);
  CELL_PROBE(g_probe_ring = prm.ring;)
  MVB_CHECK_CUDA(smem_opt_in(opt_plain, cell_fwd_epi_kernel<false>, smem_bytes));
  MVB_CHECK_CUDA(smem_opt_in(opt_mc, cell_fwd_epi_kernel<true>, smem_bytes));
  const long long m_tiles = (prm.R + BLOCK_M - 1) / BLOCK_M;
  if (multicast && m_tiles >= 2 * (long long)num_sms) {
    prm.order = pick_order(prm_in.order, (m_tiles + 1) / 2, num_sms / 2, EW_N_TILES);
    cudaLaunchConfig_t cfg = {};
    cfg.gridDim = dim3((unsigned)(num_sms / 2 * 2)); cfg.blockDim = dim3(EW_THREADS);
    cfg.dynamicSmemBytes = smem_bytes; cfg.stream = stream;
    cudaLaunchAttribute attr[1];
    attr[0].id = cudaLaunchAttributeClusterDimension;
    attr[0].val.clusterDim.x = 2; attr[0].val.clusterDim.y = 1; attr[0].val.clusterDim.z = 1;
    cfg.attrs = attr; cfg.numAttrs = 1;
    MVB_CHECK_CUDA(cudaLaunchKernelEx(&cfg, cell_fwd_epi_kernel<true>, tm.A, tm.Bqh, tm.A8, tm.B8qh, prm));
    count_launch(1);
    note_variant(1, 1);
    return MVB_OK;
  }
  const long long num_tiles = m_tiles * EW_N_TILES;
  const int grid = (int)(num_tiles < num_sms ? num_tiles : num_sms);
  prm.order = pick_order(prm_in.order, m_tiles, grid, EW_N_TILES);
  cell_fwd_epi_kernel<false><<<grid, EW_THREADS, smem_bytes, stream>>>(tm.A, tm.Bq, tm.A8, tm.B8q, prm);
  MVB_CHECK_CUDA(cudaGetLastError());
  count_launch(1);
  note_variant(1, 0);
  return MVB_OK;
}

constexpr long long kEpiWgMinTilesPerSm = 64;

template <int FMT>
static int launch_cell(const CellMaps& tm, const CellParams& prm_in, int num_sms, bool multicast, int epi_wg,
                       cudaStream_t stream) {
  CellParams prm = prm_in;
  static SmemOptIn opt_plain, opt_mc;
  static const bool format_rings = [] { const char* e = getenv("MVB_CELL_FORMAT_RINGS"); return !(e && e[0] == '0'); }();
  if (FMT == 1 && (epi_wg == 1 || (epi_wg == 2 && (prm.R + BLOCK_M - 1) / BLOCK_M >= kEpiWgMinTilesPerSm * num_sms)))
    return launch_cell_epi(tm, prm, num_sms, multicast, stream);
  const int ra8 = (BLOCK_M + 2 * (prm.W + 2) + 7) & ~7;
  prm.ring = format_rings ? CellCfg<FMT>::ring(ra8) : CellCfg<0>::ring(ra8);
  const int smem_bytes = prm.ring.smem_bytes();
  MVB_REQUIRE(ra8 <= CellCfg<FMT>::MAX_RA8 && smem_bytes <= kSmemLimit && prm.ring.b_slots >= 2 &&
              prm.ring.b_slots <= kMaxBSlots && prm.ring.a_stages >= 2 && prm.ring.a_stages <= kMaxAStages,
              "cell_fwd: grid width W=%d too large (A stage of %d rows: %d weight slots, %d A stages, %d B shared memory)",
              prm.W, ra8, prm.ring.b_slots, prm.ring.a_stages, smem_bytes);
  CELL_PROBE(g_probe_ring = prm.ring;)
  MVB_CHECK_CUDA(smem_opt_in(opt_plain, cell_fwd_kernel<false, FMT>, smem_bytes));
  MVB_CHECK_CUDA(smem_opt_in(opt_mc, cell_fwd_kernel<true, FMT>, smem_bytes));
  const long long m_tiles = (prm.R + BLOCK_M - 1) / BLOCK_M;
  if (multicast && m_tiles >= 2 * (long long)num_sms) {
    prm.order = pick_order(prm_in.order, (m_tiles + 1) / 2, num_sms / 2, N_TILES);
    cudaLaunchConfig_t cfg = {};
    cfg.gridDim = dim3((unsigned)(num_sms / 2 * 2)); cfg.blockDim = dim3(NUM_THREADS);
    cfg.dynamicSmemBytes = smem_bytes; cfg.stream = stream;
    cudaLaunchAttribute attr[1];
    attr[0].id = cudaLaunchAttributeClusterDimension;
    attr[0].val.clusterDim.x = 2; attr[0].val.clusterDim.y = 1; attr[0].val.clusterDim.z = 1;
    cfg.attrs = attr; cfg.numAttrs = 1;
    MVB_CHECK_CUDA(cudaLaunchKernelEx(&cfg, cell_fwd_kernel<true, FMT>, tm.A, tm.Bh, tm.A8, tm.B8h, prm));
    count_launch(1);
    note_variant(FMT, 1);
    return MVB_OK;
  }
  const long long num_tiles = m_tiles * N_TILES;
  const int grid = (int)(num_tiles < num_sms ? num_tiles : num_sms);
  prm.order = pick_order(prm_in.order, m_tiles, grid, N_TILES);
  cell_fwd_kernel<false, FMT><<<grid, NUM_THREADS, smem_bytes, stream>>>(tm.A, tm.B, tm.A8, tm.B8, prm);
  MVB_CHECK_CUDA(cudaGetLastError());
  count_launch(1);
  note_variant(FMT, 0);
  return MVB_OK;
}

int cell_fwd(const CellStep& s, cudaStream_t stream) {
  const int P = s.planes & 0xFF, P_out = (s.planes >> 8) ? (s.planes >> 8) : P;
  MVB_REQUIRE(valid_planes(P) && valid_planes(P_out), "cell_fwd: planes P=%d (output planes %d) not 2 or %d", P, P_out,
              kPlanesF16F8);
  const bool mixed = P == kPlanesF16F8, fan = s.fanout > 1;
  const int x_sources = !!s.xf_B + !!s.xs_tab + !!s.xr_W;
  const long long NS = s.NS; const int H = s.H, W = s.W, cpad = s.cpad;
  MVB_REQUIRE(!mixed || !s.gates_out, "cell_fwd: the f16f8 format is an inference format (no gates_out)");
  MVB_REQUIRE(x_sources <= 1, "cell_fwd: at most one x source (x-fold, sparse or dense x)");
  MVB_REQUIRE(!s.row_map || !(s.xs_tab || s.xr_W), "cell_fwd: a row map goes with the x-fold tables or no x source");
  MVB_REQUIRE(!fan || (s.xf_B && s.c_in && s.h32_out && s.fanout_ws && !s.row_map && !s.hp_out),
              "cell_fwd: fanout=%d needs the x-fold tables, c_in, h32_out, a [R,1024] fp32 workspace and no row_map / hp_out", s.fanout);
  MVB_REQUIRE(!s.xf_B || (s.xf_T2 && s.xf_ids && H >= 3 && W >= 3), "cell_fwd: x-fold needs its tables, ids and a grid of at least 3x3");
  MVB_REQUIRE((!s.xs_tab || s.xs_label) && (!s.xr_W || s.xr_in), "cell_fwd: the sparse x path needs its labels, the dense one its input");
  MVB_REQUIRE(cpad % XPAD == 0 && cpad >= kHidden + XPAD && cpad <= kHidden + kMaxXBlock,
              "cell_fwd: cpad=%d must be a multiple of %d from %d to %d (x block of 32 to %d channels)", cpad, XPAD,
              kHidden + XPAD, kHidden + kMaxXBlock, kMaxXBlock);
  MVB_REQUIRE(NS > 0 && H > 0 && W > 0, "cell_fwd: bad sizes NS=%lld H=%d W=%d", NS, H, W);
  MVB_REQUIRE(s.xh && s.w && (s.bias || s.xf_B) && s.c_out, "cell_fwd: null pointer");
  if (s.hp_out) MVB_REQUIRE(s.cpad_out % 8 == 0 && s.ch_off_out % 8 == 0, "cell_fwd: hp_out pitch/offset must be multiples of 8");
  const Grid g = make_grid(H, W);
  const long long R = NS * g.S;
  MVB_REQUIRE(R + 2LL * g.Wp + 256 < 0x7fffffffLL, "cell_fwd: too many rows (%lld) for int32 TMA coordinates", R);

  static const bool multicast = [] { const char* e = getenv("MVB_CELL_MULTICAST"); return !(e && e[0] == '0'); }();
  static const int epi_wg = [] {
    const char* e = getenv("MVB_CELL_EPI_WG"), *r = getenv("MVB_CELL_FORMAT_RINGS");
    if ((e && e[0] == '0') || (r && r[0] == '0')) return 0;
    return (e && e[0] == '1') ? 1 : 2;
  }();
  CellMaps tm;
  const int P16 = mixed ? 1 : kBf16Planes;
  const uint32_t ra8 = (uint32_t)((BLOCK_M + 2 * (W + 2) + 7) & ~7);
  MVB_REQUIRE(ra8 <= 256, "cell_fwd: grid width W=%d too large for the halo'd A stage (%u rows > 256)", W, ra8);
  int rc = encode_tmap_3d_bf16(&tm.A, s.xh, (uint64_t)cpad, (uint64_t)R, (uint64_t)P16,
                               (uint64_t)cpad * 2, (uint64_t)R * cpad * 2, CHUNK, ra8, P16, 128);
  if (rc) return rc;
  const uint64_t ktot = 9ull * cpad;
  rc = encode_tmap_3d_bf16(&tm.B, s.w, ktot, (uint64_t)kGates, (uint64_t)P16, ktot * 2,
                           ktot * kGates * 2, CHUNK, BLOCK_N, 1, 128);
  if (rc) return rc;
  rc = encode_tmap_3d_bf16(&tm.Bh, s.w, ktot, (uint64_t)kGates, (uint64_t)P16, ktot * 2,
                           ktot * kGates * 2, CHUNK, BLOCK_N / 2, 1, 128);
  if (rc) return rc;
  tm.A8 = tm.A; tm.B8 = tm.B; tm.B8h = tm.Bh;
  const float* col_scale = nullptr;
  if (mixed) {
    const uint8_t* a8 = reinterpret_cast<const uint8_t*>(s.xh) + 2ull * R * cpad;
    const uint8_t* b8 = reinterpret_cast<const uint8_t*>(s.w) + 2ull * kGates * ktot;
    rc = encode_tmap_3d_u8(&tm.A8, a8, 2ull * cpad, (uint64_t)R, 1, 2ull * cpad, 2ull * R * cpad, ROW_BYTES, ra8, 1, 128);
    if (rc) return rc;
    rc = encode_tmap_3d_u8(&tm.B8, b8, 2 * ktot, (uint64_t)kGates, 1, 2 * ktot, 2 * ktot * kGates, ROW_BYTES, BLOCK_N, 1, 128);
    if (rc) return rc;
    rc = encode_tmap_3d_u8(&tm.B8h, b8, 2 * ktot, (uint64_t)kGates, 1, 2 * ktot, 2 * ktot * kGates, ROW_BYTES, BLOCK_N / 2, 1, 128);
    if (rc) return rc;
    col_scale = reinterpret_cast<const float*>(b8 + 2ull * kGates * ktot);
  }
  if (mixed && epi_wg) {
    const uint8_t* b8 = reinterpret_cast<const uint8_t*>(s.w) + 2ull * kGates * ktot;
    const uint64_t d16[4] = {ktot, 32, 2, 16}, s16[3] = {ktot * 2, 32 * ktot * 2, 64 * ktot * 2};
    const uint64_t d8[4] = {2 * ktot, 32, 2, 16}, s8[3] = {2 * ktot, 32 * 2 * ktot, 64 * 2 * ktot};
    const uint32_t q16[4] = {CHUNK, 32, 1, 4}, q16h[4] = {CHUNK, 32, 1, 2};
    const uint32_t q8[4] = {ROW_BYTES, 32, 1, 4}, q8h[4] = {ROW_BYTES, 32, 1, 2};
    if ((rc = encode_tmap_4d_bf16(&tm.Bq, s.w, d16, s16, q16, 128))) return rc;
    if ((rc = encode_tmap_4d_bf16(&tm.Bqh, s.w, d16, s16, q16h, 128))) return rc;
    if ((rc = encode_tmap_4d_u8(&tm.B8q, b8, d8, s8, q8, 128))) return rc;
    if ((rc = encode_tmap_4d_u8(&tm.B8qh, b8, d8, s8, q8h, 128))) return rc;
  }

  CellParams prm;
  prm.bias = s.bias; prm.col_scale = col_scale; prm.c_in = s.c_in; prm.row_map = s.row_map; prm.c_out = s.c_out;
  prm.h32_out = s.h32_out; prm.gates_out = s.gates_out;
  prm.preact_out = fan ? s.fanout_ws : nullptr;
  prm.xf_B = s.xf_B; prm.xf_T2 = s.xf_T2; prm.xf_ids = s.xf_ids;
  prm.xs_tab = s.xs_tab; prm.xs_label = s.xs_label; prm.xr_in = s.xr_in; prm.xr_W = s.xr_W;
  prm.skip_x = x_sources;
  static const int order = [] { const char* e = getenv("MVB_CELL_ORDER"); return e ? atoi(e) : -1; }();
  prm.order = order;
  prm.hp_mixed = P_out == kPlanesF16F8;
  prm.hp_out = reinterpret_cast<__nv_bfloat16*>(s.hp_out);
  prm.hp_plane_stride = s.hp_plane_stride; prm.cpad_out = s.cpad_out; prm.ch_off_out = s.ch_off_out;
  prm.R = R; prm.H = H; prm.W = W; prm.cpad = cpad; prm.forget_bias = s.forget_bias;

  int dev = 0, num_sms = 0;
  MVB_CHECK_CUDA(cudaGetDevice(&dev));
  MVB_CHECK_CUDA(cudaDeviceGetAttribute(&num_sms, cudaDevAttrMultiProcessorCount, dev));
  rc = mixed ? launch_cell<1>(tm, prm, num_sms, multicast, epi_wg, stream)
             : launch_cell<0>(tm, prm, num_sms, multicast, 0, stream);
  if (rc || !fan) return rc;
  const unsigned blocks = (unsigned)((NS * H * W * 32 + 255) / 256);
  auto children = mixed ? fanout_children_kernel<1> : fanout_children_kernel<0>;
  children<<<blocks, 256, 0, stream>>>(s.fanout_ws, col_scale, s.xf_B, s.xf_T2, s.xf_ids, s.c_in, s.c_out, s.h32_out,
                                       NS, s.fanout, g, s.forget_bias);
  MVB_CHECK_CUDA(cudaGetLastError());
  count_launch(1);
  return MVB_OK;
}

__device__ __forceinline__ float packed_weight(const float* __restrict__ kernel, int n, int k, int cx, int cxp,
                                               int cpad) {
  const int tap = k / cpad, kcn = k - tap * cpad;
  const int tile = n / BLOCK_N, gate = (n % BLOCK_N) / TILE_CH, j = n % TILE_CH;
  const int col = gate * kHidden + tile * TILE_CH + j;
  int cin = -1;
  if (kcn >= cxp) cin = cx + (kcn - cxp);
  else if (kcn < cx) cin = kcn;
  return (cin >= 0) ? kernel[((long long)tap * (cx + kHidden) + cin) * kGates + col] : 0.f;
}

__global__ void colscale_kernel(const float* __restrict__ kernel, float* __restrict__ col_scale, int cx) {
  const int n = (blockIdx.x * blockDim.x + threadIdx.x) >> 5, lane = threadIdx.x & 31;
  if (n >= kGates) return;
  const int tile = n / BLOCK_N, gate = (n % BLOCK_N) / TILE_CH, j = n % TILE_CH;
  const int col = gate * kHidden + tile * TILE_CH + j;
  float m = 0.f;
  for (int r = lane; r < 9 * (cx + kHidden); r += 32) m = fmaxf(m, fabsf(kernel[(long long)r * kGates + col]));
  m = warp_max(m);
  if (lane == 0) {
    int e = 0;
    if (m > 0.f) frexpf(m, &e);
    const int S = m > 0.f ? 13 - (e - 1) : 0;
    col_scale[n] = ldexpf(1.0f, -S);
  }
}

__global__ void pack_weights_f16f8_kernel(const float* __restrict__ kernel, const float* __restrict__ biases,
                                          __half* __restrict__ w16, uint8_t* __restrict__ w8,
                                          const float* __restrict__ col_scale, float* __restrict__ bias_packed,
                                          int cx, int cxp, int cpad) {
  const long long ktot = 9LL * cpad;
  const long long total = (long long)kGates * ktot;
  for (long long i = blockIdx.x * (long long)blockDim.x + threadIdx.x; i < total;
       i += (long long)gridDim.x * blockDim.x) {
    const int n = (int)(i / ktot);
    const int k = (int)(i - (long long)n * ktot);
    const float v = packed_weight(kernel, n, k, cx, cxp, cpad) / col_scale[n];
    const __half b0 = __float2half_rn(v);
    const float f0 = __half2float(b0);
    w16[i] = b0;
    const int tap = k / cpad, kcn = k - tap * cpad;
    uint8_t* w8row = w8 + ((long long)n * 9 + tap) * 2 * cpad;
    w8row[f8_off(kcn, 0, cpad)] = to_e4m3(v - f0);
    w8row[f8_off(kcn, 1, cpad)] = to_e4m3(f0 * (1.0f / kF8ResidualScale));
    if (k == 0) {
      const int tile = n / BLOCK_N, gate = (n % BLOCK_N) / TILE_CH, j = n % TILE_CH;
      bias_packed[n] = biases[gate * kHidden + tile * TILE_CH + j];
    }
  }
}


int pack_cell_weights(const float* kernel, const float* biases, void* w_planes, float* bias_packed,
                      int cx, int P, int comp, cudaStream_t stream) {
  MVB_REQUIRE(valid_planes(P), "pack_cell_weights: planes P=%d not 2 or %d", P, kPlanesF16F8);
  MVB_REQUIRE(cx >= 1, "pack_cell_weights: cx=%d", cx);
  const int cxp = (cx + XPAD - 1) / XPAD * XPAD;
  const int cpad = cxp + kHidden;
  if (P == kPlanesF16F8) {
    MVB_REQUIRE(!comp, "pack_cell_weights: the compensated x block exists for bf16 planes only");
    const long long total = (long long)kGates * 9 * cpad;
    __half* w16 = reinterpret_cast<__half*>(w_planes);
    uint8_t* w8 = reinterpret_cast<uint8_t*>(w_planes) + 2 * total;
    float* col_scale = reinterpret_cast<float*>(w8 + 2 * total);
    colscale_kernel<<<kGates / 8, 256, 0, stream>>>(kernel, col_scale, cx);
    pack_weights_f16f8_kernel<<<1184, 256, 0, stream>>>(kernel, biases, w16, w8, col_scale, bias_packed, cx, cxp, cpad);
    MVB_CHECK_CUDA(cudaGetLastError());
    count_launch(2);
    return MVB_OK;
  }
  MVB_REQUIRE(!comp || 4 * cx <= cxp, "pack_cell_weights: compensated x block needs 4*cx <= %d", cxp);
  pack_weights_kernel<<<1184, 256, 0, stream>>>(kernel, biases, reinterpret_cast<__nv_bfloat16*>(w_planes), bias_packed,
                                                cx, cxp, cpad, comp);
  MVB_CHECK_CUDA(cudaGetLastError());
  count_launch(1);
  return MVB_OK;
}

}
```

### multiverse_b200/csrc/mvb_kernels.h

```cpp
#pragma once
#include <cuda_runtime.h>
#include <stdint.h>

namespace mvb {

void count_launch(int n);

struct CellStep {
  const void *xh, *w;
  const float *bias, *c_in;
  const int* row_map;
  float *c_out, *h32_out;
  void* hp_out;
  long long hp_plane_stride; int cpad_out, ch_off_out;
  long long NS; int H, W, cpad;
  int planes; float forget_bias;
  float* gates_out;
  const float *xf_B, *xf_T2; const int* xf_ids;
  const float* xs_tab; const int* xs_label;
  const float *xr_in, *xr_W;
  int fanout;
  float* fanout_ws;
};
int cell_fwd(const CellStep& s, cudaStream_t stream);
int cell_xdense_weights(const float* kernel, float* out, cudaStream_t stream);
int cell_xsparse_weights(const float* kernel, int cx, float* out, cudaStream_t stream);
int cell_xsparse_table(const float* scene_conv, const int* frame_idx, const int* label, const float* Wx, float* tab,
                       long long NS, int H, int W, cudaStream_t stream);
int cell_last_variant();
unsigned long long cell_variants_seen(int reset);
int cell_xfold_tables(const float* kernel, const float* biases, const float* We, const float* be, int E,
                      float* Bt, float* T2, cudaStream_t stream);
int pack_cell_weights(const float* kernel, const float* biases, void* w_planes, float* bias_packed,
                      int cx, int P, int comp, cudaStream_t stream);

int nhwc_to_planes(const float* src, void* dst_planes, long long plane_stride, int cpad, int ch_off,
                   long long NS, int H, int W, int C, int P, int comp, cudaStream_t stream);
int traj_to_grid(const double* traj, const double* centers, double h_gap, double w_gap, int* labels,
                 float* regress, long long NT, int H, int W, cudaStream_t stream);
int nhwc_halo_copy(const float* src, float* dst, long long NS, int H, int W, int C, int to_nhwc,
                   cudaStream_t stream);
int enc_class_input(const float* scene_conv, const int* frame_idx, const int* label,
                    const int* prev_label, void* xh_planes, long long plane_stride, int cpad,
                    long long NS, int H, int W, int P, cudaStream_t stream);

int scene_conv_fwd(const float* in, const float* W, const float* b, float* out, long long F, int IH,
                   int IW, int Cin, int Cout, cudaStream_t stream);
int scene_time_mean(const float* scene_conv, const int* frame_idx, float* out, long long N, int T,
                    long long HWC, cudaStream_t stream);

int gnn_attend_fwd(const float* h32, const int* row_map, const float* scene_mean, int beam,
                   void* hp_out, long long hp_plane_stride, int cpad_out, int ch_off_out,
                   long long NS, int H, int W, int P, cudaStream_t stream);

int head_fwd(const float* h32, const float* Wo, int Pout, float* out, int* ids_out, const float* We,
             const float* be, int E, void* xh_next, long long plane_stride, int cpad, long long NS,
             int H, int W, int P, cudaStream_t stream);
int head_class_fwd_dense(const float* h32, const float* Wo, float* out, int* ids_out, const float* We,
                         const float* be, int E, void* xh_next, long long plane_stride, int cpad, long long NS,
                         int H, int W, int P, cudaStream_t stream);
int emb_onehot_fwd(const int* ids, const float* We, const float* be, int E, void* xh_next,
                   long long plane_stride, int cpad, long long NS, int H, int W, int P,
                   cudaStream_t stream);
int emb_dense_fwd(const float* x, const float* We, const float* be, int E, void* xh_next,
                  long long plane_stride, int cpad, long long NS, int H, int W, int P,
                  cudaStream_t stream);

int decode_trajectories(const int* ids, const float* offs, const float* centers, float* out, long long N,
                        int K, int Tp, int V, cudaStream_t stream);
int beam_step(const float* logits, const float* score_in, float* score_out, int* ids_out,
              int* parents_out, int* row_map_out, long long N, int B, int V, int first_step,
              int zero_scores, int diverse, float log_gamma, cudaStream_t stream);
int beam_backtrace(const int* step_ids, const int* step_parents, const float* step_logits,
                   int* out_ids, float* out_logits, long long N, int B, int Tp, int V,
                   cudaStream_t stream);
int beam_gather_h(const float* h32, const int* row_map, void* hp_out, long long hp_plane_stride, int cpad_out,
                  long long NS, int H, int W, cudaStream_t stream);

int min_ade_fde(const float* pred, const float* gt, const int* gt_len, double* ade_err, int* ade_idx, double* fde,
                int* fde_idx, long long N, int G, int K, int Tp, int Tg, cudaStream_t stream);
int beam_nll(const float* logits, const float* logprobs, const int* gt_idx, const int* steps, double* nll, int* count,
             long long N, int K, int Tp, int V, int J, int G, cudaStream_t stream);

int cell_dgrad(const void* dg_planes, const void* wd_planes, float* dxh, long long NS, int H, int W,
               int cpad, int P, int need_x, cudaStream_t stream);
int cell_wgrad_mn(const void* dg_planes, const void* xh_planes, float* dwp, long long NS, int H, int W,
                  int cpad, int P, cudaStream_t stream);
int lstm_gates_bwd(const float* gates, const float* c_prev, const float* c_new, const float* dh,
                   const float* dc_in, void* dg_planes, long long plane_stride, float* dc_prev,
                   float* dbias_packed, long long NS, int H, int W, int P, cudaStream_t stream);
int pack_cell_weights_dgrad(const float* kernel, void* wd_planes, int cx, int P, cudaStream_t stream);
int unpack_cell_wgrad(const float* dwp, const float* dbias_packed, float* dkernel, float* dbiases,
                      int cx, int comp, int accumulate, int slabs, cudaStream_t stream);
int cell_wgrad_mn_slabs(int cpad);

int loss_fwd_bwd(const float* logits, const int* labels, float* dlogits, long long rows, int V,
                 float cls_scale, const float* reg, const float* target, float* dreg, long long nreg,
                 float reg_scale, float* loss_out, cudaStream_t stream);
int soft_ce_fwd_bwd(const float* logits, const float* labels, float* dlogits, long long rows, int V, float cls_scale,
                    float* loss_out, cudaStream_t stream);
int fg_count(const float* soft, const int* labels, long long rows, int V, double* count, cudaStream_t stream);
int masked_huber_fwd_bwd(const float* reg, const float* target, float* dreg, const float* soft, const int* labels,
                         long long rows, int V, const double* count, float reg_scale, float* loss_out,
                         cudaStream_t stream);
int head_bwd(const float* h32, const float* dout, const float* Wo, int Pout, float* dWo, float* dh,
             int accumulate_dh, long long NS, int H, int W, cudaStream_t stream);
int emb_bwd(const float* dxh, int cpad, const int* ids, const float* in_map, const float* We,
            const float* be, int E, int Pout, float* dWe, float* dbe, float* d_in, int accumulate_din,
            long long NS, int H, int W, cudaStream_t stream);
int gnn_bwd(const float* h32, const float* scene_mean, const float* gout, float* work, float* dh,
            int accumulate_dh, float* dscene_mean, long long NS, int H, int W, cudaStream_t stream);
int scene_conv_bwd(const float* in, const float* W, const float* out, const float* dout, float* dW,
                   float* db, float* din, long long F, int IH, int IW, int Cin, int Cout,
                   cudaStream_t stream);
int enc_class_input_bwd(const float* dxh, int cpad, const int* frame_idx, const int* label,
                        float* dscene, long long NS, int H, int W, cudaStream_t stream);
int scene_mean_bwd(const float* dmean, const int* frame_idx, float* dscene, long long N, int T,
                   long long HWC, cudaStream_t stream);
int clip_update(float* w, const float* grad, float* s1, float* s2, long long n, int kind, float lr, float p1, float p2,
                float eps, float clip, float wd, float gscale, cudaStream_t stream);
int adv_step(const float* x, const float* adv, const float* grad, float* out, float eps, float step, long long n,
             cudaStream_t stream);
int mix(const float* a, const float* b, float* out, float w, long long n, cudaStream_t stream);
int ce_rows(const float* logits, const int* labels, float* loss, long long rows, int V, cudaStream_t stream);
int enc_class_input_mix(const float* scene_conv, const int* frame_idx, const int* label, const int* label2, float beta,
                        void* xh_planes, long long plane_stride, int cpad, long long NS, int H, int W, int P,
                        cudaStream_t stream);
int enc_class_input_mix_bwd(const float* dxh, int cpad, const int* frame_idx, const int* label, const int* label2,
                            float beta, float* dscene, long long NS, int H, int W, cudaStream_t stream);
int clip_adadelta(float* w, const float* grad, float* acc, float* acc_upd, long long n, float lr,
                  float rho, float eps, float clip, float wd, float gscale, cudaStream_t stream);

}
```

### multiverse_b200/engine.py

```python
from __future__ import annotations

import torch

from . import ops

P_ = "person_pred/"
ENC_EMB = (P_ + "grid_emb/W", P_ + "grid_emb/b")


def _names(i):
  return dict(
      enc_class=(P_ + "encoder_grid_class_%d/enc_grid_%d/kernel" % (i, i),
                 P_ + "encoder_grid_class_%d/enc_grid_%d/biases" % (i, i)),
      enc_reg=(P_ + "encoder_grid_reg_%d/enc_grid_regress_%d/kernel" % (i, i),
               P_ + "encoder_grid_reg_%d/enc_grid_regress_%d/biases" % (i, i)),
      dec_class=(P_ + "decoder_grid_class_%d/decoder_rnn/dec_grid_%d/kernel" % (i, i),
                 P_ + "decoder_grid_class_%d/decoder_rnn/dec_grid_%d/biases" % (i, i)),
      dec_reg=(P_ + "decoder_grid_reg_%d/decoder_rnn/dec_grid_reg_%d/kernel" % (i, i),
               P_ + "decoder_grid_reg_%d/decoder_rnn/dec_grid_reg_%d/biases" % (i, i)),
      emb_class=(P_ + "decoder_grid_class_%d/decoder_rnn/grid_emb/W" % i,
                 P_ + "decoder_grid_class_%d/decoder_rnn/grid_emb/b" % i),
      emb_reg=(P_ + "decoder_grid_reg_%d/decoder_rnn/grid_emb/W" % i,
               P_ + "decoder_grid_reg_%d/decoder_rnn/grid_emb/b" % i),
      head_class=P_ + "hidden2grid_decoder_grid_class_%d/out_dec_grid/W" % i,
      head_reg=P_ + "hidden2grid_decoder_grid_reg_%d/out_dec_grid/W" % i)


class ScaleWeights(object):

  def __init__(self, weights, i, planes, fast_class=False, fast=False, scene_enc=True):
    nm = _names(i)
    f = lambda n: weights[n].detach().to(torch.float32).contiguous()
    fp = ops.PLANES_F16F8 if fast else planes
    self.enc_class = ops.PackedCell(f(nm["enc_class"][0]), f(nm["enc_class"][1]), fp)
    self.enc_reg = ops.PackedCell(f(nm["enc_reg"][0]), f(nm["enc_reg"][1]), planes, comp=True)
    self.enc_class_xs = None
    if fast and scene_enc and weights[nm["enc_class"][0]].shape[2] == 64 + ops.HIDDEN:
      self.enc_class_xs = ops.XSparse(f(nm["enc_class"][0]))
    self.enc_reg_fast = self.enc_reg_xd = None
    if fast and weights[nm["enc_reg"][0]].shape[2] == 2 + ops.HIDDEN:
      self.enc_reg_fast = ops.PackedCell(f(nm["enc_reg"][0]), f(nm["enc_reg"][1]), ops.PLANES_F16F8)
      self.enc_reg_xd = ops.XDense(f(nm["enc_reg"][0]))
    self.dec_class = ops.PackedCell(f(nm["dec_class"][0]), f(nm["dec_class"][1]),
                                    ops.PLANES_F16F8 if fast_class else planes)
    self.dec_reg = ops.PackedCell(f(nm["dec_reg"][0]), f(nm["dec_reg"][1]), fp)
    self.emb_class = (f(nm["emb_class"][0]), f(nm["emb_class"][1]))
    self.emb_reg = (f(nm["emb_reg"][0]), f(nm["emb_reg"][1]))
    self.head_class = f(nm["head_class"])
    self.head_reg = f(nm["head_reg"])
    self.dec_class_xf = ops.XFold(f(nm["dec_class"][0]), f(nm["dec_class"][1]), *self.emb_class)
    self.enc_emb = self._enc_class_xf = None
    if not scene_enc:
      self.enc_emb = (f(ENC_EMB[0]), f(ENC_EMB[1]))
      self._enc_cell = (f(nm["enc_class"][0]), f(nm["enc_class"][1]))

  def enc_class_fold(self):
    if self._enc_class_xf is None:
      self._enc_class_xf = ops.XFold(*self._enc_cell, *self.enc_emb)
    return self._enc_class_xf


class ConvRNNEngine(object):
  GRAPH_CACHE = 4
  ALLOW_F16F8 = True

  def __init__(self, cfg, weights, device=None, planes=ops.PLANES_BF16X2):
    assert planes == ops.PLANES_BF16X2, \
        "planes=%r: the engines run the bf16x2 operand format (planes=2), with f16f8 where inference allows" % (planes,)
    self.cfg = cfg
    self.device = device or torch.device("cuda", torch.cuda.current_device())
    self.planes = planes
    self.fast_class = self.ALLOW_F16F8 and bool(cfg.use_gnn or cfg.use_beam_search)
    self.class_planes = ops.PLANES_F16F8 if self.fast_class else self.planes
    self.fast = self.ALLOW_F16F8
    self.fast_planes = ops.PLANES_F16F8 if self.fast else self.planes
    assert cfg.enc_hidden_size == ops.HIDDEN and cfg.dec_hidden_size == ops.HIDDEN, \
        "the kernels are specialised for hidden size 256 (every published config)"
    assert cfg.convlstm_kernel == 3 and cfg.scene_conv_kernel == 3
    assert cfg.scene_conv_dim == 64
    assert getattr(cfg, "activation_func", "tanh") in ("tanh",) or \
        getattr(cfg.activation_func, "__name__", "") == "tanh", "kernels implement tanh"
    self.set_weights(weights)
    self._bufs = {}
    self.cell_events = None
    self._graphs = {}
    self._graph_seen = set()

  @property
  def gnn_scene_in_greedy(self):
    return bool(self.scene_enc and getattr(self.cfg, "gnn_scene_in_greedy", True))

  @property
  def scene_enc(self):
    return bool(getattr(self.cfg, "use_scene_enc", True))

  def set_weights(self, weights):
    dev = self.device
    if getattr(self, "_graphs", None) is not None:
      self._graphs.clear()
      self._graph_seen.clear()
    w = {k: (v if torch.is_tensor(v) else torch.as_tensor(v)).to(dev) for k, v in weights.items()}
    scene_enc = self.scene_enc
    self.scene_w = [(w[P_ + "scene_conv%d/W" % (i + 1)].float().contiguous(),
                     w[P_ + "scene_conv%d/b" % (i + 1)].float().contiguous())
                    for i in range(len(self.cfg.scene_grid_strides))] if scene_enc else []
    self.scales = [ScaleWeights(w, i, self.planes, self.fast_class, self.fast, scene_enc) if self.cfg.use_grids[i]
                   else None for i in range(len(self.cfg.scene_grids))]

  def _buf(self, key, maker):
    b = self._bufs.get(key)
    if b is None:
      b = maker()
      self._bufs[key] = b
    return b

  def _xh(self, tag, ns, h, w, cpad, planes=None):
    planes = planes or self.planes
    return [self._buf((tag, j, ns, h, w, cpad, planes),
                      lambda: ops.alloc_xh(ns, h, w, cpad, planes, self.device))
            for j in range(2)]

  def _state(self, tag, ns, h, w):
    return self._buf((tag, ns, h, w), lambda: ops.alloc_state(ns, h, w, self.device))

  def _cell(self, tag, shape, launch, *args, **kw):
    if self.cell_events is None:
      return launch(*args, **kw)
    e0, e1 = torch.cuda.Event(enable_timing=True), torch.cuda.Event(enable_timing=True)
    e0.record()
    launch(*args, **kw)
    e1.record()
    self.cell_events.append((tag, shape, e0, e1))

  def scene_cnn(self, scene_feat, obs_scene):
    if not self.scene_enc:
      return [None] * len(self.cfg.scene_grids), [None] * len(self.cfg.scene_grids)
    x = scene_feat
    convs, means = [], []
    for (W, b) in self.scene_w:
      x = ops.scene_conv_fwd(x, W, b)
      convs.append(x)
      means.append(ops.scene_time_mean(x, obs_scene))
# ... 60 lines not shown
      return c[t_len % 2], h32
    xh = self._xh("enc_reg", n, h, w, sw.enc_reg.cpad)
    c = [self._state("encr_c0", n, h, w), self._state("encr_c1", n, h, w)]
    h32 = self._state("encr_h32", n, h, w)
    xh[0][:, :, sw.enc_reg.cxp:].zero_()
    for t in range(t_len):
      cur, nxt = xh[t % 2], xh[(t + 1) % 2]
      ops.nhwc_to_planes(obs_reg_t[t], cur, 0, h, w, comp=sw.enc_reg.comp)
      last = t == t_len - 1
      self._cell("enc_reg", (h, w, n), ops.cell_fwd, cur, sw.enc_reg, None if t == 0 else c[t % 2],
                 c[(t + 1) % 2], h32 if last else None, xh_out if last else nxt, h, w, n)
    return c[t_len % 2], h32

  def decode_class_greedy(self, i, c_enc, h32_enc, first_ids, scene_mean, pred_len):
    cfg = self.cfg
    h, w = cfg.scene_grids[i]
    n = first_ids.shape[0]
    sw = self.scales[i]
    xh = self._xh("dec_class", n, h, w, sw.dec_class.cpad, self.class_planes)
    c = [self._state("dec_c0", n, h, w), self._state("dec_c1", n, h, w)]
    h32 = self._state("dec_h32", n, h, w)
    logits = torch.empty((pred_len, n, h * w), dtype=torch.float32, device=self.device)
    ids = torch.empty((pred_len, n), dtype=torch.int32, device=self.device)
    h_src, c_src, ids_prev = h32_enc, c_enc, first_ids
    for t in range(pred_len):
      cur, nxt = xh[t % 2], xh[(t + 1) % 2]
      if cfg.use_gnn:
        ops.gnn_attend_fwd(h_src, scene_mean if self.gnn_scene_in_greedy else None, cur, h, w, n)
      self._cell("dec_class", (h, w, n), ops.cell_fwd_onehot, cur, sw.dec_class, sw.dec_class_xf, ids_prev, c_src,
                 c[(t + 1) % 2], h32, None if cfg.use_gnn else nxt, h, w, n)
      c_src, h_src = c[(t + 1) % 2], h32
      ops.head_class_fwd(h32, sw.head_class, logits[t], ids[t], None, None, None, h, w, n,
                         planes=self.planes)
      ids_prev = ids[t]
    return logits, ids

  def decode_reg(self, i, c_enc, first_input, pred_len, xh):
    h, w = self.cfg.scene_grids[i]
    n = first_input.shape[0]
    sw = self.scales[i]
    c = [self._state("decr_c0", n, h, w), self._state("decr_c1", n, h, w)]
    h32 = self._state("decr_h32", n, h, w)
    offs = torch.empty((pred_len, n, h * w, 2), dtype=torch.float32, device=self.device)
    We, be = sw.emb_reg
    ops.emb_dense_fwd(first_input, We, be, xh[0], h, w)
    c_src = c_enc
    for t in range(pred_len):
      cur, nxt = xh[t % 2], xh[(t + 1) % 2]
      self._cell("dec_reg", (h, w, n), ops.cell_fwd, cur, sw.dec_reg, c_src, c[(t + 1) % 2], h32, nxt, h, w, n)
      c_src = c[(t + 1) % 2]
      last = t == pred_len - 1
      ops.head_reg_fwd(h32, sw.head_reg, offs[t], None if last else We, None if last else be,
                       None if last else nxt, h, w, n, planes=self.planes)
    return offs

  def decode_class_beam(self, i, c_enc, h32_enc, first_ids, scene_mean, pred_len):
    cfg = self.cfg
    h, w = cfg.scene_grids[i]
    n, b, v = first_ids.shape[0], cfg.beam_size, h * w
    ns = n * b
    dev = self.device
    sw = self.scales[i]
    xh = self._xh("beam", ns, h, w, sw.dec_class.cpad, self.class_planes)
    c = [self._state("beam_c0", ns, h, w), self._state("beam_c1", ns, h, w)]
    h32 = self._state("beam_h32", ns, h, w)
    step_logits = torch.empty((pred_len, n, b, v), dtype=torch.float32, device=dev)
    step_ids = torch.empty((pred_len, n, b), dtype=torch.int32, device=dev)
    step_par = torch.empty((pred_len, n, b), dtype=torch.int32, device=dev)
    scores = [torch.zeros((n, b), dtype=torch.float32, device=dev) for _ in range(2)]
    row_map = torch.empty((ns,), dtype=torch.int32, device=dev)
    xf = sw.dec_class_xf
    assert cfg.use_gnn or self.class_planes == ops.PLANES_F16F8, \
        "beam search without use_gnn runs on f16f8 operands (inference engine)"
    xh1 = self._xh("beam_t0", n, h, w, sw.dec_class.cpad, self.class_planes)
    c_t0 = self._state("beam_c_t0", n, h, w)
    h32_t0 = self._state("beam_h32_t0", n, h, w)
    logits_t0 = torch.empty((n, v), dtype=torch.float32, device=dev)
    if cfg.use_gnn:
      ops.gnn_attend_fwd(h32_enc, scene_mean, xh1[0], h, w, n, beam=1, row_map=None)
    self._cell("beam_t0", (h, w, n), ops.cell_fwd_onehot, xh1[0], sw.dec_class, xf, first_ids.contiguous(), c_enc,
               c_t0, h32_t0, None if cfg.use_gnn else xh1[1], h, w, n)
    ops.head_class_fwd(h32_t0, sw.head_class, logits_t0, None, None, None, None, h, w, n, planes=self.planes)
    step_logits[0].copy_(logits_t0.unsqueeze(1).expand(n, b, v))
    h_src, c_src, cur_c = h32_t0, c_t0, 1
    for time in range(1, pred_len + 1):
      if time > 1:
        ops.head_class_fwd(h32, sw.head_class, step_logits[time - 1], None, None, None, None, h, w,
                           ns, planes=self.planes)
      s_in, s_out = scores[(time - 1) % 2], scores[time % 2]
      ops.beam_step(step_logits[time - 1], s_in, s_out, step_ids[time - 1], step_par[time - 1],
                    row_map, n, b, v, first_step=(time <= 1),
                    zero_scores=(time <= cfg.fix_num_timestep), diverse=cfg.diverse_beam,
                    gamma=cfg.diverse_gamma)
      if time == pred_len:
        break
      nxt = xh[time % 2]
      if time == 1:
        if cfg.use_gnn:
          ops.gnn_attend_fwd(h32_t0, scene_mean, xh1[1], h, w, n, beam=1, row_map=None)
        ws = self._buf(("beam_fanout_ws", n, h, w), lambda: torch.empty(
            (ops.halo_rows(n, h, w), 4 * ops.HIDDEN), dtype=torch.float32, device=dev))
        self._cell("beam_fanout", (h, w, n), ops.cell_fwd_onehot_fanout, xh1[1], sw.dec_class, xf,
                   step_ids[0].view(-1), c_t0, c[1 - cur_c], h32, h, w, n, b, workspace=ws)
      else:
        if cfg.use_gnn:
          ops.gnn_attend_fwd(h_src, scene_mean, nxt, h, w, ns, beam=b, row_map=row_map)
        else:
          ops.beam_gather_h(h_src, row_map, nxt, h, w, ns)
        self._cell("beam", (h, w, ns), ops.cell_fwd_onehot, nxt, sw.dec_class, xf, step_ids[time - 1].view(-1), c_src,
                   c[1 - cur_c], h32, None, h, w, ns, row_map=row_map)
      cur_c = 1 - cur_c
      h_src, c_src = h32, c[cur_c]
    out_ids = torch.empty((n, b, pred_len), dtype=torch.int32, device=dev)
    out_logits = torch.empty((n, b, pred_len, v), dtype=torch.float32, device=dev)
    ops.beam_backtrace(step_ids, step_par, step_logits, out_ids, out_logits)
    return out_logits, out_ids, scores[pred_len % 2], dict(ids=step_ids, parents=step_par,
                                                           logits=step_logits)

  def branches(self):
    return [(kind, i) for i in range(len(self.cfg.scene_grids)) if self.cfg.use_grids[i] for kind in ("class", "reg")]

  def forward(self, feeds, pred_len=None, on_output=None, branches=None):
    cfg = self.cfg
    emit = on_output if on_output is not None else (lambda *a: None)
    run = set(self.branches() if branches is None else branches)
    tp = int(pred_len) if pred_len else cfg.pred_len
    obs_scene = feeds["obs_scene"].to(torch.int32).contiguous()
    obs_scene_t = obs_scene.t().contiguous()
    n = obs_scene.shape[0]
    convs = means = None
    if any(kind == "class" for kind, _ in run):
      convs, means = self.scene_cnn(feeds["scene_feat"].float().contiguous(), obs_scene)
    out = dict(grid_pred_decoded=[], grid_pred_reg_decoded=[], beam_outputs=None)
    for i, (h, w) in enumerate(cfg.scene_grids):
      if not cfg.use_grids[i]:
        out["grid_pred_decoded"].append([])
        out["grid_pred_reg_decoded"].append([])
        continue
      sw = self.scales[i]
      dec = reg = None
      if ("class", i) in run:
        labels = feeds["grid_obs_labels"][i].to(torch.int32)
        labels_t = labels.t().contiguous()
        xh_dec = self._xh("beam_t0" if cfg.use_beam_search and not cfg.use_gnn else "dec_class", n, h, w,
                          sw.dec_class.cpad, self.class_planes)
        c_e, h_e = self.encode_class(i, convs[i], obs_scene_t, labels_t,
                                     None if cfg.use_gnn else xh_dec[0])
        if cfg.use_beam_search:
          logits, ids, logprobs, _ = self.decode_class_beam(i, c_e, h_e, labels_t[-1].contiguous(),
                                                            means[i], tp)
          out["beam_outputs"] = [logits, ids, logprobs]
          dec = logits[:, 0].reshape(n, tp, h, w, 1)
          for j, t in enumerate(out["beam_outputs"]):
            emit("beam_outputs", j, t)
        else:
          lg, _ = self.decode_class_greedy(i, c_e, h_e, labels_t[-1].contiguous(), means[i], tp)
          dec = lg.permute(1, 0, 2).reshape(n, tp, h, w, 1)
        emit("grid_pred_decoded", i, dec)
      if ("reg", i) in run:
        obs_reg = feeds["grid_obs_regress"][i].float()
        obs_reg_t = obs_reg.transpose(0, 1).contiguous()
        xh_reg = self._xh("dec_reg", n, h, w, sw.dec_reg.cpad, self.fast_planes)
        c_r, _ = self.encode_reg(i, obs_reg_t, xh_reg[0])
        offs = self.decode_reg(i, c_r, obs_reg_t[-1], tp, xh_reg)
        reg = offs.permute(1, 0, 2, 3).reshape(n, tp, h, w, 2)
        emit("grid_pred_reg_decoded", i, reg)
        out.setdefault("_offs", {})[i] = offs
      out["grid_pred_decoded"].append(dec)
      out["grid_pred_reg_decoded"].append(reg)
    return out

  @staticmethod
  def _flat_feeds(feeds):
    items = [("scene_feat", feeds["scene_feat"]), ("obs_scene", feeds["obs_scene"])]
    for name in ("grid_obs_labels", "grid_obs_regress"):
      for i, t in enumerate(feeds[name]):
        if t is not None:
          items.append(("%s/%d" % (name, i), t))
    return items

  def forward_graph(self, feeds, pred_len=None, on_output=None):
    tp = int(pred_len) if pred_len else self.cfg.pred_len
    sf = feeds["scene_feat"]
    f_pad = -(-int(sf.shape[0]) // 64) * 64
    flat = self._flat_feeds(feeds)
    key = (tp, f_pad) + tuple((k, tuple(t.shape[1:] if k == "scene_feat" else t.shape), t.dtype) for k, t in flat)
    ent = self._graphs.get(key)
    main = torch.cuda.current_stream(self.device)
    if ent is None:
      if self.cell_events is not None:
        raise RuntimeError("forward_graph: per-launch event recording (cell_events) is an eager-mode feature")
      if key not in self._graph_seen:
        if len(self._graph_seen) >= 64:
          self._graph_seen.clear()
        self._graph_seen.add(key)
        return self.forward(feeds, tp, on_output=on_output)
      static = dict(scene_feat=torch.zeros((f_pad,) + tuple(sf.shape[1:]), dtype=sf.dtype, device=sf.device),
                    obs_scene=feeds["obs_scene"].clone(),
                    grid_obs_labels=[None if t is None else t.clone() for t in feeds["grid_obs_labels"]],
                    grid_obs_regress=[None if t is None else t.clone() for t in feeds["grid_obs_regress"]])
      static["scene_feat"][:sf.shape[0]].copy_(sf)
      self.forward(static, tp)
      torch.cuda.synchronize(self.device)
      chains = []
      for bi, br in enumerate(self.branches()):
        stream = self._buf(("graph_stream", bi), lambda: torch.cuda.Stream(device=self.device,
                                                                          priority=-1 if br[0] == "class" else 0))
        done = []
        stream.wait_stream(main)
        with torch.cuda.stream(stream):
          graph = torch.cuda.CUDAGraph()
          graph.capture_begin(capture_error_mode="thread_local")
          try:
            part = self.forward(static, tp, branches=[br], on_output=lambda *a: done.append(a))
          finally:
            graph.capture_end()
        main.wait_stream(stream)
        chains.append((br, stream, graph, done, part))
      out = dict(grid_pred_decoded=[[] for _ in self.cfg.scene_grids],
                 grid_pred_reg_decoded=[[] for _ in self.cfg.scene_grids], beam_outputs=None)
      for (kind, i), _, _, _, part in chains:
        if kind == "class":
          out["grid_pred_decoded"][i] = part["grid_pred_decoded"][i]
          if part["beam_outputs"] is not None:
            out["beam_outputs"] = part["beam_outputs"]
        else:
          out["grid_pred_reg_decoded"][i] = part["grid_pred_reg_decoded"][i]
          out.setdefault("_offs", {})[i] = part["_offs"][i]
      ent = (chains, static, out)
      while len(self._graphs) >= self.GRAPH_CACHE:
        self._graphs.pop(next(iter(self._graphs)))
      self._graphs[key] = ent
    chains, static, out = ent
    for (name, dst), (_, src) in zip(self._flat_feeds(static), flat):
      (dst[:src.shape[0]] if name == "scene_feat" else dst).copy_(src, non_blocking=True)
    fed = main.record_event()
    for br, stream, graph, done, _ in sorted(chains, key=lambda c: c[0][0] != "reg"):
      stream.wait_event(fed)
      with torch.cuda.stream(stream):
        graph.replay()
        if on_output is not None:
          for name, index, t in done:
            on_output(name, index, t)
    for _, stream, _, _, _ in chains:
      main.wait_stream(stream)
    return out

  def grid_feeds_from_traj(self, obs_traj, centers=None, video_h=1080, video_w=1920):
    import numpy as np
    cfg = self.cfg
    vh, vw = getattr(cfg, "video_h", video_h), getattr(cfg, "video_w", video_w)
    if torch.is_tensor(obs_traj):
      traj = obs_traj.to(self.device, torch.float64).contiguous()
    else:
      a = np.ascontiguousarray(obs_traj, dtype=np.float64)
      stage = self._buf(("traj_stage", a.shape), lambda: torch.empty(a.shape, dtype=torch.float64).pin_memory())
      ev = self._bufs.get(("traj_stage_event", a.shape))
      if ev is not None:
        ev.synchronize()
      stage.copy_(torch.from_numpy(a))
      traj = stage.to(self.device, non_blocking=True)
      ev = torch.cuda.Event()
      ev.record(torch.cuda.current_stream(self.device))
      self._bufs[("traj_stage_event", a.shape)] = ev
    n, t = traj.shape[0], traj.shape[1]
    labels, regress = [], []
    for i, (h, w) in enumerate(cfg.scene_grids):
      if not cfg.use_grids[i]:
        labels.append(None); regress.append(None)
# ... 39 lines not shown
```

### multiverse_b200/ops.py

```python
from __future__ import annotations

import ctypes as C
import math

import torch

from . import _lib

HIDDEN = 256
PLANES_BF16X2 = 2
PLANES_F16F8 = 16


def planes_of(t):
  return getattr(t, "mvb_planes", t.shape[0])


def cell_variants_seen(reset=False):
  m = int(_lib.load().mvb_cell_variants_seen(int(bool(reset))))
  return {((PLANES_BF16X2, PLANES_F16F8)[b // 2], bool(b % 2)) for b in range(4) if m >> b & 1}


def cell_last_variant():
  return int(_lib.load().mvb_cell_last_variant())
# ... 65 lines not shown
  t = torch.zeros((2, halo_rows(ns, h, w), cpad), dtype=torch.bfloat16, device=device)
  if planes == PLANES_F16F8:
    t.mvb_planes = PLANES_F16F8
  return t


def operand_values(xh):
  if planes_of(xh) != PLANES_F16F8:
    return xh.float().sum(0), None
  r, cpad = xh.shape[1], xh.shape[2]
  raw = xh.view(torch.uint8).reshape(-1)
  n = r * cpad
  a0 = raw[:2 * n].view(torch.float16).reshape(r, cpad).float()
  f8 = raw[2 * n:].view(torch.float8_e4m3fn).reshape(r, 2 * cpad).float()
  cxp = cpad - HIDDEN
  c = torch.arange(cpad, device=xh.device)
  c0 = torch.where(c >= cxp, cxp + (c - cxp) // 64 * 64, c // 64 * 64)
  width = torch.where(c >= cxp, 64, (cxp - c0).clamp(max=64))
  off0 = 2 * c0 + (c - c0)
  off1 = off0 + width
  return a0 + f8[:, off1] / 4096.0, f8[:, off0]


def alloc_state(ns, h, w, device, zero=True):
  f = torch.zeros if zero else torch.empty
  return f((halo_rows(ns, h, w), HIDDEN), dtype=torch.float32, device=device)


def cell_fwd(xh, packed, c_in, c_out, h32_out, xh_next, h, w, ns, row_map=None,
             forget_bias=1.0):
  hp = _hp_out(xh, packed, xh_next)
  _lib.call("mvb_convlstm_cell_fwd", _p(xh), _p(packed.w), _p(packed.bias), _p(c_in), _p(row_map), _p(c_out),
            _p(h32_out), *hp, ns, h, w, packed.cpad, _planes_arg(packed, xh_next), float(forget_bias), _stream())


class XDense(object):

  def __init__(self, kernel):
    assert kernel.dim() == 4 and kernel.shape[2] == 2 + HIDDEN, "the dense x path is for 2-channel inputs"
    self.W = torch.empty((18, 4 * HIDDEN), dtype=torch.float32, device=kernel.device)
    _lib.call("mvb_cell_xdense_weights", _p(kernel.detach().float().contiguous()), _p(self.W), _stream())


def cell_fwd_xdense(xh, packed, xdense, x_in, c_in, c_out, h32_out, xh_next, h, w, ns, forget_bias=1.0):
  hp = _hp_out(xh, packed, xh_next)
  assert x_in.dtype == torch.float32 and x_in.is_contiguous() and x_in.numel() == ns * h * w * 2
  _lib.call("mvb_convlstm_cell_fwd_xdense", _p(xh), _p(packed.w), _p(packed.bias), _p(x_in), _p(xdense.W), _p(c_in),
            _p(c_out), _p(h32_out), *hp, ns, h, w, packed.cpad, _planes_arg(packed, xh_next), float(forget_bias),
            _stream())


class XSparse(object):

  def __init__(self, kernel):
    assert kernel.dim() == 4 and kernel.shape[2] == 64 + HIDDEN, "the sparse x path is for the 64 scene channels"
    self.W = torch.empty((9 * 64, 4 * HIDDEN), dtype=torch.float32, device=kernel.device)
    _lib.call("mvb_cell_xsparse_weights", _p(kernel.detach().float().contiguous()), 64, _p(self.W), _stream())


def cell_xsparse_table(scene_conv, frame_idx, label, xsparse, table, h, w):
  _lib.call("mvb_cell_xsparse_table", _p(scene_conv), _p(frame_idx), _p(label), _p(xsparse.W), _p(table),
            label.shape[0], h, w, _stream())


def cell_fwd_xsparse(xh, packed, table, label, c_in, c_out, h32_out, xh_next, h, w, ns, forget_bias=1.0):
  hp = _hp_out(xh, packed, xh_next)
  _lib.call("mvb_convlstm_cell_fwd_xsparse", _p(xh), _p(packed.w), _p(packed.bias), _p(table), _p(label), _p(c_in),
            _p(c_out), _p(h32_out), *hp, ns, h, w, packed.cpad, _planes_arg(packed, xh_next), float(forget_bias),
            _stream())


class XFold(object):

  def __init__(self, kernel, biases, We, be):
    dev = kernel.device
    self.B = torch.empty((9, 4 * HIDDEN), dtype=torch.float32, device=dev)
    self.T2 = torch.empty((9, 25, 4 * HIDDEN), dtype=torch.float32, device=dev)
    _lib.call("mvb_cell_xfold_tables", _p(kernel.detach().float().contiguous()),
              _p(biases.detach().float().contiguous()), _p(We), _p(be), We.shape[3], _p(self.B),
              _p(self.T2), _stream())


def cell_fwd_onehot(xh, packed, xf, ids, c_in, c_out, h32_out, xh_next, h, w, ns, row_map=None,
                    forget_bias=1.0):
  hp = _hp_out(xh, packed, xh_next)
  _lib.call("mvb_convlstm_cell_fwd_onehot", _p(xh), _p(packed.w), _p(xf.B), _p(xf.T2), _p(ids), _p(c_in),
            _p(row_map), _p(c_out), _p(h32_out), *hp, ns, h, w, packed.cpad, _planes_arg(packed, xh_next),
            float(forget_bias), _stream())


def cell_fwd_onehot_fanout(xh, packed, xf, ids, c_in, c_out, h32_out, h, w, ns, fanout, forget_bias=1.0,
                           workspace=None):
  assert xh.shape[2] == packed.cpad and planes_of(xh) == packed.planes
  if workspace is None:
    workspace = torch.empty((halo_rows(ns, h, w), 4 * HIDDEN), dtype=torch.float32, device=xh.device)
  assert workspace.numel() >= halo_rows(ns, h, w) * 4 * HIDDEN and workspace.dtype == torch.float32
  _lib.call("mvb_convlstm_cell_fwd_onehot_fanout", _p(xh), _p(packed.w), _p(xf.B), _p(xf.T2), _p(ids), _p(c_in),
            _p(c_out), _p(h32_out), _p(workspace), ns, fanout, h, w, packed.cpad, packed.planes, float(forget_bias),
            _stream())


def nhwc_to_planes(src, xh, ch_off, h, w, comp=False):
  ns, c = src.shape[0], src.shape[-1]
  _lib.call("mvb_nhwc_to_planes", _p(src), _p(xh), xh.stride(0), xh.shape[2], ch_off, ns, h, w,
            c, planes_of(xh), int(comp), _stream())


def nhwc_to_halo(src, dst, h, w):
  _lib.call("mvb_nhwc_to_halo", _p(src), _p(dst), src.shape[0], h, w, src.shape[-1], _stream())


def halo_to_nhwc(src, dst, h, w):
  _lib.call("mvb_halo_to_nhwc", _p(src), _p(dst), dst.shape[0], h, w, dst.shape[-1], _stream())


def enc_class_input(scene_conv, frame_idx, label, prev_label, xh, h, w):
  _lib.call("mvb_enc_class_input", _p(scene_conv), _p(frame_idx), _p(label), _p(prev_label),
            _p(xh), xh.stride(0), xh.shape[2], label.shape[0], h, w, planes_of(xh), _stream())


def enc_class_input_mix(scene_conv, frame_idx, label, label2, beta, xh, h, w):
  _lib.call("mvb_enc_class_input_mix", _p(scene_conv), _p(frame_idx), _p(label), _p(label2), float(beta),
            _p(xh), xh.stride(0), xh.shape[2], label.shape[0], h, w, planes_of(xh), _stream())


def scene_conv_fwd(x, W, b):
  f, ih, iw, cin = x.shape
  cout = W.shape[3]
  out = torch.empty((f, (ih + 1) // 2, (iw + 1) // 2, cout), dtype=torch.float32, device=x.device)
  _lib.call("mvb_scene_conv_fwd", _p(x), _p(W), _p(b), _p(out), f, ih, iw, cin, cout, _stream())
  return out


def scene_time_mean(scene_conv, frame_idx):
  n, t = frame_idx.shape
  hwc = scene_conv[0].numel()
  out = torch.empty((n,) + tuple(scene_conv.shape[1:]), dtype=torch.float32,
                    device=scene_conv.device)
  _lib.call("mvb_scene_time_mean", _p(scene_conv), _p(frame_idx), _p(out), n, t, hwc, _stream())
  return out


def gnn_attend_fwd(h32, scene_mean, xh_next, h, w, ns, beam=1, row_map=None):
  _lib.call("mvb_gnn_attend_fwd", _p(h32), _p(row_map), _p(scene_mean), beam, _p(xh_next),
            xh_next.stride(0), xh_next.shape[2], xh_next.shape[2] - HIDDEN, ns, h, w,
            planes_of(xh_next), _stream())


def head_class_fwd(h32, Wo, logits_out, ids_out, We, be, xh_next, h, w, ns, planes=PLANES_BF16X2):
  e = 0 if We is None else We.shape[3]
  if xh_next is not None:
    stride, cpad, planes = xh_next.stride(0), xh_next.shape[2], planes_of(xh_next)
  else:
    stride, cpad = 0, 0
  _lib.call("mvb_head_class_fwd", _p(h32), _p(Wo), _p(logits_out), _p(ids_out), _p(We), _p(be), e,
            _p(xh_next), stride, cpad, ns, h, w, planes, _stream())


def head_class_fwd_dense(h32, Wo, logits_out, ids_out, We, be, xh_next, h, w, ns, planes=PLANES_BF16X2):
  e = 0 if We is None else We.shape[3]
  if xh_next is not None:
    stride, cpad, planes = xh_next.stride(0), xh_next.shape[2], planes_of(xh_next)
  else:
    stride, cpad = 0, 0
  _lib.call("mvb_head_class_fwd_dense", _p(h32), _p(Wo), _p(logits_out), _p(ids_out), _p(We), _p(be), e,
            _p(xh_next), stride, cpad, ns, h, w, planes, _stream())


def head_reg_fwd(h32, Wo, off_out, We, be, xh_next, h, w, ns, planes=PLANES_BF16X2):
  e = 0 if We is None else We.shape[3]
  if xh_next is not None:
    stride, cpad, planes = xh_next.stride(0), xh_next.shape[2], planes_of(xh_next)
  else:
    stride, cpad = 0, 0
  _lib.call("mvb_head_reg_fwd", _p(h32), _p(Wo), _p(off_out), _p(We), _p(be), e, _p(xh_next),
            stride, cpad, ns, h, w, planes, _stream())


def emb_onehot_fwd(ids, We, be, xh_next, h, w):
  _lib.call("mvb_emb_onehot_fwd", _p(ids), _p(We), _p(be), We.shape[3], _p(xh_next),
            xh_next.stride(0), xh_next.shape[2], ids.numel(), h, w, planes_of(xh_next), _stream())


def emb_dense_fwd(x, We, be, xh_next, h, w):
  _lib.call("mvb_emb_dense_fwd", _p(x), _p(We), _p(be), We.shape[3], _p(xh_next),
            xh_next.stride(0), xh_next.shape[2], x.shape[0], h, w, planes_of(xh_next), _stream())


def beam_step(logits, score_in, score_out, ids_out, parents_out, row_map_out, n, b, v,
              first_step, zero_scores, diverse, gamma):
  lg = math.log(gamma) if diverse else 0.0
  _lib.call("mvb_beam_step", _p(logits), _p(score_in), _p(score_out), _p(ids_out),
            _p(parents_out), _p(row_map_out), n, b, v, int(first_step), int(zero_scores),
            int(diverse), float(lg), _stream())


def beam_gather_h(h32, row_map, xh_next, h, w, ns):
  assert planes_of(xh_next) == PLANES_F16F8, "beam_gather_h writes the f16f8 operand format only"
  assert xh_next.shape[1] == halo_rows(ns, h, w) and row_map.dtype == torch.int32 and row_map.numel() == ns
  _lib.call("mvb_beam_gather_h_f16f8", _p(h32), _p(row_map), _p(xh_next), xh_next.stride(0), xh_next.shape[2], ns,
            h, w, _stream())


def beam_backtrace(step_ids, step_parents, step_logits, out_ids, out_logits):
  tp, n, b = step_ids.shape
  v = step_logits.shape[-1]
  _lib.call("mvb_beam_backtrace", _p(step_ids), _p(step_parents), _p(step_logits), _p(out_ids),
            _p(out_logits), n, b, tp, v, _stream())


def cell_fwd_train(xh, packed, c_in, c_out, h32_out, xh_next, gates_out, h, w, ns, forget_bias=1.0):
  hp = _hp_out(xh, packed, xh_next)
  _lib.call("mvb_convlstm_cell_fwd_train", _p(xh), _p(packed.w), _p(packed.bias), _p(c_in), _p(c_out), _p(h32_out),
            *hp, _p(gates_out), ns, h, w, packed.cpad, packed.planes, float(forget_bias), _stream())


def pack_dgrad(packed, kernel):
  if getattr(packed, "wd", None) is None:
    packed.wd = torch.empty((packed.planes, packed.cpad, 9 * 4 * HIDDEN), dtype=torch.bfloat16,
                            device=kernel.device)
  _lib.call("mvb_pack_cell_weights_dgrad", _p(kernel.detach().float().contiguous()), _p(packed.wd),
            packed.cx, packed.planes, _stream())
  return packed.wd


def lstm_gates_bwd(gates, c_prev, c_new, dh, dc_in, dg_planes, dc_prev, dbias_packed, h, w, ns):
  _lib.call("mvb_lstm_gates_bwd", _p(gates), _p(c_prev), _p(c_new), _p(dh), _p(dc_in),
            _p(dg_planes), dg_planes.stride(0), _p(dc_prev), _p(dbias_packed), ns, h, w,
            dg_planes.shape[0], _stream())


def cell_dgrad(dg_planes, wd, dxh, h, w, ns, need_dx=True):
  _lib.call("mvb_cell_dgrad", _p(dg_planes), _p(wd), _p(dxh), ns, h, w, dxh.shape[1],
            dg_planes.shape[0], int(need_dx), _stream())


def cell_wgrad_direct(dg_planes, xh, dw_packed, h, w, ns):
  _lib.call("mvb_cell_wgrad_direct", _p(dg_planes), _p(xh), _p(dw_packed), ns, h, w, xh.shape[2],
            xh.shape[0], _stream())


def wgrad_slabs(cpad):
  return int(_lib.load().mvb_cell_wgrad_slabs(cpad))


def unpack_cell_wgrad(dw_packed, dbias_packed, dkernel, dbiases, cx, comp=False, accumulate=False):
  slabs = dw_packed.shape[0] if dw_packed.dim() == 3 else 1
  _lib.call("mvb_unpack_cell_wgrad", _p(dw_packed), _p(dbias_packed), _p(dkernel), _p(dbiases), cx,
            int(comp), int(accumulate), slabs, _stream())


def loss_fwd_bwd(logits, labels, dlogits, cls_weight, reg, target, dreg, reg_weight, loss_out):
  rows, v = (logits.numel() // logits.shape[-1], logits.shape[-1]) if logits is not None else (0, 0)
  nreg = reg.numel() if reg is not None else 0
  _lib.call("mvb_loss_fwd_bwd", _p(logits), _p(labels), _p(dlogits), rows, v, float(cls_weight),
            _p(reg), _p(target), _p(dreg), nreg, float(reg_weight), _p(loss_out), _stream())


def soft_ce_fwd_bwd(logits, labels, dlogits, cls_weight, loss_out):
  v = logits.shape[-1]
  assert labels.dtype == torch.float32 and labels.numel() == logits.numel()
  _lib.call("mvb_soft_ce_fwd_bwd", _p(logits), _p(labels), _p(dlogits), logits.numel() // v, v, float(cls_weight),
            _p(loss_out), _stream())


def fg_count(labels, v, count):
  soft = labels.dtype == torch.float32
  rows = labels.numel() // v if soft else labels.numel()
  _lib.call("mvb_fg_count", _p(labels) if soft else None, None if soft else _p(labels), rows, v, _p(count),
            _stream())


def masked_huber_fwd_bwd(reg, target, dreg, labels, count, reg_weight, loss_out):
  v = reg.shape[-2]
  soft = labels.dtype == torch.float32
  rows = reg.numel() // (2 * v)
  assert count.dtype == torch.float64 and (labels.numel() == rows * v if soft else labels.numel() == rows)
  _lib.call("mvb_masked_huber_fwd_bwd", _p(reg), _p(target), _p(dreg), _p(labels) if soft else None,
            None if soft else _p(labels), rows, v, _p(count), float(reg_weight), _p(loss_out), _stream())


def head_bwd(h32, dout, Wo, dWo, dh, accumulate_dh, h, w, ns):
  _lib.call("mvb_head_bwd", _p(h32), _p(dout), _p(Wo), Wo.shape[3], _p(dWo), _p(dh),
            int(accumulate_dh), ns, h, w, _stream())
# ... 93 lines not shown
```

Measured before the change: 370.8.

## Restrict beam decoder ConvLSTM to per-beam row bands around the one-hot cell

Adds a beam-band scheme to beam-search decoding. Rows outside a band around each beam's chosen grid cell, widened each step by the conv receptive radius, match a shared base trajectory fed a null id. A small single-block kernel builds the bands and a compacted M-tile list, and the cell kernel iterates only those tiles. A copy kernel then fills the rows outside the bands from a base ConvLSTM run over N samples instead of N*K. This trades full-grid GEMMs for band tiles plus an extra base cell step, a scan kernel and copies. Exactness relies on the band radius covering the receptive-field growth, and the path can be turned off with an environment variable.

```diff
diff --git a/include/multiverse_b200.h b/include/multiverse_b200.h
--- a/include/multiverse_b200.h
+++ b/include/multiverse_b200.h
@@ -31,7 +31,8 @@
                           int E, float* table_B, float* table_T2, void* stream);
 int mvb_convlstm_cell_fwd_onehot(const void* xh_planes, const void* w_planes, const float* table_B,
                                  const float* table_T2, const int32_t* ids, const float* c_in,
-                                 const int32_t* row_map, float* c_out, float* h32_out, void* hp_out,
+                                 const int32_t* row_map, const int32_t* tiles, const int32_t* tile_count,
+                                 float* c_out, float* h32_out, void* hp_out,
                                  int64_t hp_plane_stride, int cpad_out, int ch_off_out, int64_t NS, int H,
                                  int W, int cpad, int planes, float forget_bias, void* stream);
 int mvb_convlstm_cell_fwd_xdense(const void* xh_planes, const void* w_planes, const float* bias_packed,
@@ -166,6 +167,12 @@
 int mvb_beam_gather_h_f16f8(const float* h32, const int32_t* row_map, void* hp_out, int64_t hp_plane_stride,
                             int cpad_out, int64_t NS, int H, int W, void* stream);
 
+int mvb_beam_band(const int32_t* ids, const int32_t* parents, const int32_t* band_in, int32_t* band_out,
+                  int32_t* tiles, int64_t tiles_cap, int32_t* tile_count, int64_t NS, int K, int radius, int H, int W,
+                  void* stream);
+int mvb_beam_band_copy(const float* base_c, const float* base_h32, const int32_t* band, float* c, float* h32,
+                       int64_t NS, int K, int H, int W, void* stream);
+
 int mvb_traj_to_grid(const double* traj, const double* centers, double h_gap, double w_gap, int32_t* labels,
                      float* regress, int64_t NT, int H, int W, void* stream);
 
diff --git a/multiverse_b200/_lib.py b/multiverse_b200/_lib.py
--- a/multiverse_b200/_lib.py
+++ b/multiverse_b200/_lib.py
@@ -28,7 +28,7 @@
     "mvb_cell_xsparse_weights": [_vp, _i, _vp, _vp],
     "mvb_cell_xsparse_table": [_vp, _vp, _vp, _vp, _vp, _i64, _i, _i, _vp],
     "mvb_convlstm_cell_fwd_onehot_fanout": [_vp, _vp, _vp, _vp, _vp, _vp, _vp, _vp, _vp, _i64, _i, _i, _i, _i, _i, _f, _vp],
-    "mvb_convlstm_cell_fwd_onehot": [_vp, _vp, _vp, _vp, _vp, _vp, _vp, _vp, _vp, _vp, _i64, _i, _i, _i64,
+    "mvb_convlstm_cell_fwd_onehot": [_vp, _vp, _vp, _vp, _vp, _vp, _vp, _vp, _vp, _vp, _vp, _vp, _i64, _i, _i, _i64,
                                      _i, _i, _i, _i, _f, _vp],
     "mvb_convlstm_cell_fwd_train": [_vp, _vp, _vp, _vp, _vp, _vp, _vp, _i64, _i, _i, _vp, _i64, _i, _i,
                                     _i, _i, _f, _vp],
@@ -74,6 +74,8 @@
     "mvb_beam_nll": [_vp, _vp, _vp, _vp, _vp, _vp, _i64, _i, _i, _i, _i, _i, _vp],
     "mvb_beam_backtrace": [_vp, _vp, _vp, _vp, _vp, _i64, _i, _i, _i, _vp],
     "mvb_beam_gather_h_f16f8": [_vp, _vp, _vp, _i64, _i, _i64, _i, _i, _vp],
+    "mvb_beam_band": [_vp, _vp, _vp, _vp, _vp, _i64, _vp, _i64, _i, _i, _i, _i, _vp],
+    "mvb_beam_band_copy": [_vp, _vp, _vp, _vp, _vp, _i64, _i, _i, _i, _vp],
 }
 _RESTYPES = {"mvb_last_error": C.c_char_p, "mvb_launch_count": C.c_longlong, "mvb_cell_variants_seen": C.c_longlong,
              "mvb_reset_launch_count": None}
diff --git a/multiverse_b200/csrc/mvb_api.cu b/multiverse_b200/csrc/mvb_api.cu
--- a/multiverse_b200/csrc/mvb_api.cu
+++ b/multiverse_b200/csrc/mvb_api.cu
@@ -119,7 +119,7 @@
 extern "C" {
 
 const char* mvb_last_error(void) { return get_error(); }
-int mvb_abi_version(void) { return 14; }
+int mvb_abi_version(void) { return 15; }
 int mvb_cell_last_variant(void) { return cell_last_variant(); }
 long long mvb_cell_variants_seen(int reset) { return (long long)cell_variants_seen(reset); }
 long long mvb_launch_count(void) { return g_launches; }
@@ -149,14 +149,15 @@
 }
 int mvb_convlstm_cell_fwd_onehot(const void* xh_planes, const void* w_planes, const float* table_B,
                                  const float* table_T2, const int32_t* ids, const float* c_in,
-                                 const int32_t* row_map, float* c_out, float* h32_out, void* hp_out,
+                                 const int32_t* row_map, const int32_t* tiles, const int32_t* tile_count,
+                                 float* c_out, float* h32_out, void* hp_out,
                                  int64_t hp_plane_stride, int cpad_out, int ch_off_out, int64_t NS, int H,
                                  int W, int cpad, int planes, float forget_bias, void* stream) {
   CellStep s{};
   s.xh = xh_planes; s.w = w_planes; s.xf_B = table_B; s.xf_T2 = table_T2; s.xf_ids = ids; s.c_in = c_in;
   s.row_map = row_map; s.c_out = c_out; s.h32_out = h32_out; s.hp_out = hp_out; s.hp_plane_stride = hp_plane_stride;
   s.cpad_out = cpad_out; s.ch_off_out = ch_off_out; s.NS = NS; s.H = H; s.W = W; s.cpad = cpad; s.planes = planes;
-  s.forget_bias = forget_bias;
+  s.forget_bias = forget_bias; s.tiles = tiles; s.tile_count = tile_count;
   return cell_fwd(s, S(stream));
 }
 int mvb_convlstm_cell_fwd_xdense(const void* xh_planes, const void* w_planes, const float* bias_packed,
@@ -414,5 +415,14 @@
                             int cpad_out, int64_t NS, int H, int W, void* stream) {
   return beam_gather_h(h32, row_map, hp_out, hp_plane_stride, cpad_out, NS, H, W, S(stream));
 }
-
-}
+int mvb_beam_band(const int32_t* ids, const int32_t* parents, const int32_t* band_in, int32_t* band_out,
+                  int32_t* tiles, int64_t tiles_cap, int32_t* tile_count, int64_t NS, int K, int radius, int H, int W,
+                  void* stream) {
+  return beam_band(ids, parents, band_in, band_out, tiles, tiles_cap, tile_count, NS, K, radius, H, W, S(stream));
+}
+int mvb_beam_band_copy(const float* base_c, const float* base_h32, const int32_t* band, float* c, float* h32,
+                       int64_t NS, int K, int H, int W, void* stream) {
+  return beam_band_copy(base_c, base_h32, band, c, h32, NS, K, H, W, S(stream));
+}
+
+}
diff --git a/multiverse_b200/csrc/mvb_beam.cu b/multiverse_b200/csrc/mvb_beam.cu
--- a/multiverse_b200/csrc/mvb_beam.cu
+++ b/multiverse_b200/csrc/mvb_beam.cu
@@ -285,6 +285,143 @@
   return MVB_OK;
 }
 
+constexpr int BAND_THREADS = 1024;
+
+static long long beam_band_capacity(long long NS, int H, int W) {
+  const Grid g = make_grid(H, W);
+  return NS * ((g.S + 127) / 128 + 1);
+}
+
+template <class Op>
+__device__ long long block_scan_excl(long long v, long long identity, int slot, long long* sh, Op op) {
+  long long x = v;
+  sh[slot] = x;
+  __syncthreads();
+  for (int o = 1; o < BAND_THREADS; o <<= 1) {
+    const long long u = slot >= o ? sh[slot - o] : identity;
+    __syncthreads();
+    x = op(u, x);
+    sh[slot] = x;
+    __syncthreads();
+  }
+  const long long r = slot ? sh[slot - 1] : identity;
+  __syncthreads();
+  return r;
+}
+
+__global__ void __launch_bounds__(BAND_THREADS)
+beam_band_kernel(const int* __restrict__ ids, const int* __restrict__ parents, const int* __restrict__ band_in,
+                 int* band_out, int* __restrict__ tiles, int* __restrict__ tile_count, int NS, int K, int radius,
+                 Grid g) {
+  __shared__ long long sh[BAND_THREADS];
+  const int t = threadIdx.x;
+  const int per = (NS + BAND_THREADS - 1) / BAND_THREADS;
+  const int k0 = min(NS, t * per), k1 = min(NS, k0 + per);
+  for (int k = k0; k < k1; ++k) {
+    const int y = ids[k] / g.W;
+    int lo = y - 2, hi = y + 2;
+    if (band_in) {
+      const int p = k - k % K + parents[k];
+      lo = min(lo, band_in[2 * p] - radius);
+      hi = max(hi, band_in[2 * p + 1] + radius);
+    }
+    band_out[2 * k] = max(lo, 0);
+    band_out[2 * k + 1] = min(hi, g.H - 1);
+  }
+  __syncthreads();
+  auto rows = [&](int k, long long& s, long long& e) {
+    const int lo = band_out[2 * k], hi = band_out[2 * k + 1];
+    s = (long long)k * g.S + (long long)lo * g.Wp;
+    e = hi == g.H - 1 ? (long long)(k + 1) * g.S : (long long)k * g.S + (long long)(hi + 1) * g.Wp;
+  };
+  auto continues = [&](int k) { return k > 0 && k < NS && band_out[2 * k] == 0 && band_out[2 * k - 1] == g.H - 1; };
+  auto lmax = [](long long a, long long b) { return a > b ? a : b; };
+  auto lmin = [](long long a, long long b) { return a < b ? a : b; };
+  auto lsum = [](long long a, long long b) { return a + b; };
+  long long agg = -1, s, e;
+  for (int k = k0; k < k1; ++k) if (!continues(k)) { rows(k, s, e); agg = s; }
+  const long long start_in = block_scan_excl(agg, -1LL, t, sh, lmax);
+  const long long kInf = 0x7fffffffffffffffLL;
+  agg = kInf;
+  for (int k = k0; k < k1; ++k) if (!continues(k + 1)) { rows(k, s, e); agg = e; break; }
+  const long long end_in = block_scan_excl(agg, kInf, BAND_THREADS - 1 - t, sh, lmin);
+  auto own = [](long long s, long long e, long long rs, long long& j0, long long& j1) {
+    j0 = (s - rs + kCellTileRows - 1) / kCellTileRows; j1 = (e - rs + kCellTileRows - 1) / kCellTileRows;
+  };
+  long long rs = start_in, n = 0, j0, j1;
+  for (int k = k0; k < k1; ++k) {
+    rows(k, s, e);
+    if (!continues(k)) rs = s;
+    own(s, e, rs, j0, j1);
+    n += j1 - j0;
+  }
+  long long o = block_scan_excl(n, 0LL, t, sh, lsum);
+  if (t == BAND_THREADS - 1) *tile_count = (int)(o + n);
+  long long re = 0;
+  rs = start_in;
+  for (int k = k0; k < k1; ++k) {
+    rows(k, s, e);
+    if (!continues(k)) rs = s;
+    if (k == k0 || !continues(k)) {
+      int j = k;
+      while (j + 1 < k1 && continues(j + 1)) ++j;
+      long long sj, ej;
+      rows(j, sj, ej);
+      re = (j + 1 == k1 && continues(k1)) ? end_in : ej;
+    }
+    own(s, e, rs, j0, j1);
+    for (long long j = j0; j < j1; ++j, ++o) {
+      const long long m0 = rs + j * kCellTileRows;
+      tiles[2 * o] = (int)m0;
+      tiles[2 * o + 1] = (int)lmin(m0 + kCellTileRows, re);
+    }
+  }
+}
+
+int beam_band(const int* ids, const int* parents, const int* band_in, int* band_out, int* tiles, long long tiles_cap,
+              int* tile_count, long long NS, int K, int radius, int H, int W, cudaStream_t stream) {
+  MVB_REQUIRE(ids && band_out && tiles && tile_count && (!band_in || parents), "beam_band: null pointer");
+  MVB_REQUIRE(band_in != band_out, "beam_band: the parents' bands and the new ones need separate buffers");
+  MVB_REQUIRE(NS > 0 && K > 0 && NS % K == 0 && H > 0 && W > 0 && radius >= 0,
+              "beam_band: bad sizes NS=%lld K=%d H=%d W=%d radius=%d", NS, K, H, W, radius);
+  const Grid g = make_grid(H, W);
+  MVB_REQUIRE(NS * g.S + kCellTileRows < 0x7fffffffLL, "beam_band: NS=%lld too large for int32 rows", NS);
+  MVB_REQUIRE(tiles_cap >= beam_band_capacity(NS, H, W), "beam_band: %lld tile entries, %lld needed", tiles_cap,
+              beam_band_capacity(NS, H, W));
+  beam_band_kernel<<<1, BAND_THREADS, 0, stream>>>(ids, parents, band_in, band_out, tiles, tile_count, (int)NS, K,
+                                                   radius, g);
+  MVB_CHECK_CUDA(cudaGetLastError());
+  count_launch(1);
+  return MVB_OK;
+}
+
+__global__ void __launch_bounds__(256)
+beam_band_copy_kernel(const float4* __restrict__ base_c, const float4* __restrict__ base_h, const int* __restrict__ band,
+                      float4* __restrict__ c, float4* __restrict__ h, int K, Grid g) {
+  const long long k = blockIdx.x / g.H;
+  const int y = (int)(blockIdx.x - k * g.H);
+  if (y >= band[2 * k] && y <= band[2 * k + 1]) return;
+  constexpr int V = kHidden / 4;
+  const long long src = ((k / K) * g.S + (long long)y * g.Wp) * V, dst = (k * g.S + (long long)y * g.Wp) * V;
+  for (int i = threadIdx.x; i < g.W * V; i += blockDim.x) {
+    c[dst + i] = __ldg(base_c + src + i);
+    h[dst + i] = __ldg(base_h + src + i);
+  }
+}
+
+int beam_band_copy(const float* base_c, const float* base_h32, const int* band, float* c, float* h32, long long NS,
+                   int K, int H, int W, cudaStream_t stream) {
+  MVB_REQUIRE(base_c && base_h32 && band && c && h32, "beam_band_copy: null pointer");
+  MVB_REQUIRE(NS > 0 && K > 0 && NS % K == 0 && H > 0 && W > 0 && NS * H < (1ll << 31),
+              "beam_band_copy: bad sizes NS=%lld K=%d H=%d W=%d", NS, K, H, W);
+  beam_band_copy_kernel<<<(unsigned)(NS * H), 256, 0, stream>>>(
+      reinterpret_cast<const float4*>(base_c), reinterpret_cast<const float4*>(base_h32), band,
+      reinterpret_cast<float4*>(c), reinterpret_cast<float4*>(h32), K, make_grid(H, W));
+  MVB_CHECK_CUDA(cudaGetLastError());
+  count_launch(1);
+  return MVB_OK;
+}
+
 int beam_backtrace(const int* step_ids, const int* step_parents, const float* step_logits,
                    int* out_ids, float* out_logits, long long N, int B, int Tp, int V,
                    cudaStream_t stream) {
diff --git a/multiverse_b200/csrc/mvb_cell.cu b/multiverse_b200/csrc/mvb_cell.cu
--- a/multiverse_b200/csrc/mvb_cell.cu
+++ b/multiverse_b200/csrc/mvb_cell.cu
@@ -4,7 +4,7 @@
 
 namespace mvb {
 
-constexpr int BLOCK_M = 128;
+constexpr int BLOCK_M = kCellTileRows;
 constexpr int BLOCK_N = 256;
 constexpr int XPAD = 32;
 constexpr int kMaxXBlock = 256;
@@ -90,6 +90,8 @@
   int cpad_out;
   int ch_off_out;
   long long R;
+  const int* tiles;
+  const int* tile_count;
   int H, W;
   int cpad;
   float forget_bias;
@@ -116,10 +118,10 @@
   const float* xft;
 };
 
-__device__ __forceinline__ EpiRow epi_row(const CellParams& prm, const Grid& g, long long row) {
+__device__ __forceinline__ EpiRow epi_row(const CellParams& prm, const Grid& g, long long row, long long m_end) {
   EpiRow r;
   r.row = row; r.src_row = row; r.psmp = 0; r.py = 0; r.px = 0; r.xfb = nullptr; r.xft = nullptr;
-  r.valid = row < prm.R;
+  r.valid = row < m_end;
   if (!r.valid) return r;
   const long long smp = row / g.S;
   const int rem = (int)(row - smp * g.S);
@@ -148,6 +150,16 @@
     }
   }
   return r;
+}
+
+__device__ __forceinline__ long long m_tile_count(const CellParams& prm) {
+  return prm.tiles ? (long long)__ldg(prm.tile_count) : (prm.R + BLOCK_M - 1) / BLOCK_M;
+}
+__device__ __forceinline__ void m_tile_rows(const CellParams& prm, long long count, long long i, long long& m0,
+                                            long long& m_end) {
+  if (!prm.tiles) { m0 = i * BLOCK_M; m_end = prm.R; }
+  else if (i < count) { m0 = __ldg(prm.tiles + 2 * i); m_end = __ldg(prm.tiles + 2 * i + 1); }
+  else { m0 = 0; m_end = 0; }
 }
 
 __device__ __forceinline__ float2 epi_cprev(const CellParams& prm, const EpiRow& r, int ch) {
@@ -281,7 +293,7 @@
   const int NQ = nqx + kHidden / CHUNK;
   constexpr int NPASS = FMT ? 2 : 1;
   constexpr int NS = FMT ? 1 : kBf16Planes;
-  const long long num_m_tiles = (prm.R + BLOCK_M - 1) / BLOCK_M;
+  const long long num_m_tiles = m_tile_count(prm);
   const uint32_t rank = MC ? cluster_ctarank() : 0u;
   const long long num_tiles = (MC ? (num_m_tiles + 1) / 2 : num_m_tiles) * N_TILES;
   const long long w_begin = MC ? (long long)(blockIdx.x >> 1) : (long long)blockIdx.x;
@@ -289,7 +301,9 @@
   auto work_index = [&](long long it) -> long long {
     return prm.order ? (w_begin + (it / N_TILES) * w_step) * N_TILES + it % N_TILES : w_begin + it * w_step;
   };
-  auto tile_m0 = [&](long long w) -> long long { return ((w / N_TILES) * (MC ? 2 : 1) + rank) * BLOCK_M; };
+  auto tile_rows = [&](long long w, long long& m0, long long& m_end) {
+    m_tile_rows(prm, num_m_tiles, (w / N_TILES) * (MC ? 2 : 1) + rank, m0, m_end);
+  };
 
   if (warp == 0 && lane == 0) {
     prefetch_tmap(&tmA);
@@ -310,7 +324,8 @@
       int slot = 0, astage = 0; uint32_t phase = 0, aphase = 0;
       CELL_PROBE(const long long probe_t0 = clock64();)
       for (long long it = 0, t; (t = work_index(it)) < num_tiles; ++it) {
-        const long long m0 = tile_m0(t);
+        long long m0, m_end;
+        tile_rows(t, m0, m_end);
         const int n0 = (int)(t % N_TILES) * BLOCK_N;
         for (int pass = 0; pass < NPASS; ++pass)
         for (int q = q_begin; q < NQ; ++q) {
@@ -366,7 +381,8 @@
     CELL_PROBE(const long long probe_t0 = clock64();)
     for (long long it = 0, t; (t = work_index(it)) < num_tiles; ++it) {
       CELL_PROBE(++probe[kProbeTiles];)
-      const long long m0 = tile_m0(t);
+      long long m0, m_end;
+      tile_rows(t, m0, m_end);
       const int nt = (int)(t % N_TILES);
       uint32_t fresh = 1;
       auto mma16 = [&](uint32_t a_lo, uint32_t b_lo) {
@@ -430,7 +446,7 @@
       float2 cprev[2][8];
 #pragma unroll
       for (int hr = 0; hr < 2; ++hr) {
-        rows[hr] = epi_row(prm, g, rbase + 8 * hr);
+        rows[hr] = epi_row(prm, g, rbase + 8 * hr, m_end);
 #pragma unroll
         for (int ip = 0; ip < 8; ++ip) cprev[hr][ip] = epi_cprev(prm, rows[hr], nt * TILE_CH + 8 * ip + 2 * (lane & 3));
       }
@@ -538,7 +554,7 @@
   const int nqx = (cxp + CHUNK - 1) / CHUNK;
   const int q_begin = prm.skip_x ? nqx : 0;
   const int NQ = nqx + kHidden / CHUNK;
-  const long long num_m_tiles = (prm.R + BLOCK_M - 1) / BLOCK_M;
+  const long long num_m_tiles = m_tile_count(prm);
   const uint32_t rank = MC ? cluster_ctarank() : 0u;
   const long long num_tiles = (MC ? (num_m_tiles + 1) / 2 : num_m_tiles) * EW_N_TILES;
   const long long w_begin = MC ? (long long)(blockIdx.x >> 1) : (long long)blockIdx.x;
@@ -546,7 +562,9 @@
   auto work_index = [&](long long it) -> long long {
     return prm.order ? (w_begin + (it / EW_N_TILES) * w_step) * EW_N_TILES + it % EW_N_TILES : w_begin + it * w_step;
   };
-  auto tile_m0 = [&](long long w) -> long long { return ((w / EW_N_TILES) * (MC ? 2 : 1) + rank) * BLOCK_M; };
+  auto tile_rows = [&](long long w, long long& m0, long long& m_end) {
+    m_tile_rows(prm, num_m_tiles, (w / EW_N_TILES) * (MC ? 2 : 1) + rank, m0, m_end);
+  };
 
   if (warp == 0 && lane == 0) {
     prefetch_tmap(&tmA); prefetch_tmap(&tmB); prefetch_tmap(&tmA8); prefetch_tmap(&tmB8);
@@ -567,7 +585,8 @@
       int slot = 0, astage = 0; uint32_t phase = 0, aphase = 0;
       CELL_PROBE(const long long probe_t0 = clock64();)
       for (long long it = 0, t; (t = work_index(it)) < num_tiles; ++it) {
-        const long long m0 = tile_m0(t);
+        long long m0, m_end;
+        tile_rows(t, m0, m_end);
         const int nt = (int)(t % EW_N_TILES);
         const int half = nt & 1, tg0 = (nt >> 1) * 4;
         for (int pass = 0; pass < 2; ++pass)
@@ -706,7 +725,8 @@
     uint32_t staged_phase = 0;
     CELL_PROBE(const long long probe_t0 = clock64();)
     for (long long it = 0, t; (t = work_index(it)) < num_tiles; ++it) {
-      const long long m0 = tile_m0(t);
+      long long m0, m_end;
+      tile_rows(t, m0, m_end);
       const int nt = (int)(t % EW_N_TILES);
       const int tn = nt >> 1, jh = (nt & 1) * EW_TILE_CH;
       const int rb = 32 * ew + (lane >> 2);
@@ -716,7 +736,7 @@
         float2 cprev[2][4];
 #pragma unroll
         for (int hr = 0; hr < 2; ++hr) {
-          rows[hr] = epi_row(prm, g, m0 + rb + 8 * (k2 + hr));
+          rows[hr] = epi_row(prm, g, m0 + rb + 8 * (k2 + hr), m_end);
 #pragma unroll
           for (int ip = 0; ip < 4; ++ip) cprev[hr][ip] = epi_cprev(prm, rows[hr], tn * TILE_CH + jh + 8 * ip + lc);
         }
@@ -1101,11 +1121,22 @@
   return MVB_OK;
 }
 
+static int fanout_children(const CellStep& s, const float* col_scale, const Grid& g, cudaStream_t stream) {
+  const unsigned blocks = (unsigned)((s.NS * g.H * g.W * 32 + 255) / 256);
+  auto children = col_scale ? fanout_children_kernel<1> : fanout_children_kernel<0>;
+  children<<<blocks, 256, 0, stream>>>(s.fanout_ws, col_scale, s.xf_B, s.xf_T2, s.xf_ids, s.c_in, s.c_out, s.h32_out,
+                                       s.NS, s.fanout, g, s.forget_bias);
+  MVB_CHECK_CUDA(cudaGetLastError());
+  count_launch(1);
+  return MVB_OK;
+}
+
 int cell_fwd(const CellStep& s, cudaStream_t stream) {
   const int P = s.planes & 0xFF, P_out = (s.planes >> 8) ? (s.planes >> 8) : P;
   MVB_REQUIRE(valid_planes(P) && valid_planes(P_out), "cell_fwd: planes P=%d (output planes %d) not 2 or %d", P, P_out,
               kPlanesF16F8);
-  const bool mixed = P == kPlanesF16F8, fan = s.fanout > 1;
+  const bool mixed = P == kPlanesF16F8, fan = s.fanout > 1 || (s.fanout == 1 && !s.xh);
+  const bool children_only = fan && !s.xh;
   const int x_sources = !!s.xf_B + !!s.xs_tab + !!s.xr_W;
   const long long NS = s.NS; const int H = s.H, W = s.W, cpad = s.cpad;
   MVB_REQUIRE(!mixed || !s.gates_out, "cell_fwd: the f16f8 format is an inference format (no gates_out)");
@@ -1118,8 +1149,9 @@
   MVB_REQUIRE(cpad % XPAD == 0 && cpad >= kHidden + XPAD && cpad <= kHidden + kMaxXBlock,
               "cell_fwd: cpad=%d must be a multiple of %d from %d to %d (x block of 32 to %d channels)", cpad, XPAD,
               kHidden + XPAD, kHidden + kMaxXBlock, kMaxXBlock);
+  MVB_REQUIRE(!s.tiles || (s.tile_count && !fan), "cell_fwd: a work list needs its count and no fan-out");
   MVB_REQUIRE(NS > 0 && H > 0 && W > 0, "cell_fwd: bad sizes NS=%lld H=%d W=%d", NS, H, W);
-  MVB_REQUIRE(s.xh && s.w && (s.bias || s.xf_B) && s.c_out, "cell_fwd: null pointer");
+  MVB_REQUIRE((s.xh || children_only) && s.w && (s.bias || s.xf_B) && s.c_out, "cell_fwd: null pointer");
   if (s.hp_out) MVB_REQUIRE(s.cpad_out % 8 == 0 && s.ch_off_out % 8 == 0, "cell_fwd: hp_out pitch/offset must be multiples of 8");
   const Grid g = make_grid(H, W);
   const long long R = NS * g.S;
@@ -1131,6 +1163,11 @@
     if ((e && e[0] == '0') || (r && r[0] == '0')) return 0;
     return (e && e[0] == '1') ? 1 : 2;
   }();
+  if (children_only) {
+    const float* col_scale = mixed ? reinterpret_cast<const float*>(reinterpret_cast<const uint8_t*>(s.w) +
+                                                                    4ull * kGates * 9 * cpad) : nullptr;
+    return fanout_children(s, col_scale, g, stream);
+  }
   CellMaps tm;
   const int P16 = mixed ? 1 : kBf16Planes;
   const uint32_t ra8 = (uint32_t)((BLOCK_M + 2 * (W + 2) + 7) & ~7);
@@ -1183,6 +1220,7 @@
   prm.hp_out = reinterpret_cast<__nv_bfloat16*>(s.hp_out);
   prm.hp_plane_stride = s.hp_plane_stride; prm.cpad_out = s.cpad_out; prm.ch_off_out = s.ch_off_out;
   prm.R = R; prm.H = H; prm.W = W; prm.cpad = cpad; prm.forget_bias = s.forget_bias;
+  prm.tiles = s.tiles; prm.tile_count = s.tile_count;
 
   int dev = 0, num_sms = 0;
   MVB_CHECK_CUDA(cudaGetDevice(&dev));
@@ -1190,13 +1228,7 @@
   rc = mixed ? launch_cell<1>(tm, prm, num_sms, multicast, epi_wg, stream)
              : launch_cell<0>(tm, prm, num_sms, multicast, 0, stream);
   if (rc || !fan) return rc;
-  const unsigned blocks = (unsigned)((NS * H * W * 32 + 255) / 256);
-  auto children = mixed ? fanout_children_kernel<1> : fanout_children_kernel<0>;
-  children<<<blocks, 256, 0, stream>>>(s.fanout_ws, col_scale, s.xf_B, s.xf_T2, s.xf_ids, s.c_in, s.c_out, s.h32_out,
-                                       NS, s.fanout, g, s.forget_bias);
-  MVB_CHECK_CUDA(cudaGetLastError());
-  count_launch(1);
-  return MVB_OK;
+  return fanout_children(s, col_scale, g, stream);
 }
 
 __device__ __forceinline__ float packed_weight(const float* __restrict__ kernel, int n, int k, int cx, int cxp,
diff --git a/multiverse_b200/csrc/mvb_kernels.h b/multiverse_b200/csrc/mvb_kernels.h
--- a/multiverse_b200/csrc/mvb_kernels.h
+++ b/multiverse_b200/csrc/mvb_kernels.h
@@ -6,6 +6,7 @@
 
 void count_launch(int n);
 
+constexpr int kCellTileRows = 128;
 struct CellStep {
   const void *xh, *w;
   const float *bias, *c_in;
@@ -21,6 +22,7 @@
   const float *xr_in, *xr_W;
   int fanout;
   float* fanout_ws;
+  const int *tiles, *tile_count;
 };
 int cell_fwd(const CellStep& s, cudaStream_t stream);
 int cell_xdense_weights(const float* kernel, float* out, cudaStream_t stream);
@@ -76,6 +78,10 @@
                    cudaStream_t stream);
 int beam_gather_h(const float* h32, const int* row_map, void* hp_out, long long hp_plane_stride, int cpad_out,
                   long long NS, int H, int W, cudaStream_t stream);
+int beam_band(const int* ids, const int* parents, const int* band_in, int* band_out, int* tiles, long long tiles_cap,
+              int* tile_count, long long NS, int K, int radius, int H, int W, cudaStream_t stream);
+int beam_band_copy(const float* base_c, const float* base_h32, const int* band, float* c, float* h32, long long NS,
+                   int K, int H, int W, cudaStream_t stream);
 
 int min_ade_fde(const float* pred, const float* gt, const int* gt_len, double* ade_err, int* ade_idx, double* fde,
                 int* fde_idx, long long N, int G, int K, int Tp, int Tg, cudaStream_t stream);
diff --git a/multiverse_b200/engine.py b/multiverse_b200/engine.py
--- a/multiverse_b200/engine.py
+++ b/multiverse_b200/engine.py
@@ -1,4 +1,6 @@
 from __future__ import annotations
+
+import os
 
 import torch
 
@@ -58,6 +60,10 @@
     if self._enc_class_xf is None:
       self._enc_class_xf = ops.XFold(*self._enc_cell, *self.enc_emb)
     return self._enc_class_xf
+
+
+def beam_band_on():
+  return os.environ.get("MVB_BEAM_BAND", "1") != "0"
 
 
 class ConvRNNEngine(object):
@@ -284,6 +290,20 @@
                c_t0, h32_t0, None if cfg.use_gnn else xh1[1], h, w, n)
     ops.head_class_fwd(h32_t0, sw.head_class, logits_t0, None, None, None, None, h, w, n, planes=self.planes)
     step_logits[0].copy_(logits_t0.unsqueeze(1).expand(n, b, v))
+    band = pred_len > 2 and beam_band_on()
+    if band:
+      bands = [self._buf(("beam_band", j, ns), lambda: torch.empty((ns, 2), dtype=torch.int32, device=dev))
+               for j in range(2)]
+      tiles = self._buf(("beam_band_tiles", ns, h, w), lambda: torch.empty(
+          (ops.beam_band_capacity(ns, h, w), 2), dtype=torch.int32, device=dev))
+      tile_count = torch.empty((pred_len,), dtype=torch.int32, device=dev)
+      base_xh = self._xh("beam_base", n, h, w, sw.dec_class.cpad, self.class_planes)[0]
+      base_c = [self._state("beam_base_c0", n, h, w), self._state("beam_base_c1", n, h, w)]
+      base_h32 = self._state("beam_base_h32", n, h, w)
+      no_ids = self._buf(("beam_base_ids", n, h, w), lambda: torch.full((n,), (h + 3) * w, dtype=torch.int32,
+                                                                        device=dev))
+      rows = self._buf(("beam_base_rows", n), lambda: torch.arange(n, dtype=torch.int32, device=dev))
+      radius = 2 if cfg.use_gnn else 1
     h_src, c_src, cur_c = h32_t0, c_t0, 1
     for time in range(1, pred_len + 1):
       if time > 1:
@@ -296,6 +316,9 @@
                     gamma=cfg.diverse_gamma)
       if time == pred_len:
         break
+      if band:
+        ops.beam_band(step_ids[time - 1], step_par[time - 1], None if time == 1 else bands[time % 2],
+                      bands[1 - time % 2], tiles, tile_count[time:time + 1], b, radius, h, w)
       nxt = xh[time % 2]
       if time == 1:
         if cfg.use_gnn:
@@ -304,13 +327,26 @@
             (ops.halo_rows(n, h, w), 4 * ops.HIDDEN), dtype=torch.float32, device=dev))
         self._cell("beam_fanout", (h, w, n), ops.cell_fwd_onehot_fanout, xh1[1], sw.dec_class, xf,
                    step_ids[0].view(-1), c_t0, c[1 - cur_c], h32, h, w, n, b, workspace=ws)
+        if band:
+          ops.cell_fwd_onehot_fanout(None, sw.dec_class, xf, no_ids, c_t0, base_c[1], base_h32, h, w, n, 1,
+                                     workspace=ws)
       else:
+        if band:
+          if cfg.use_gnn:
+            ops.gnn_attend_fwd(base_h32, scene_mean, base_xh, h, w, n, beam=1, row_map=None)
+          else:
+            ops.beam_gather_h(base_h32, rows, base_xh, h, w, n)
+          self._cell("beam_base", (h, w, n), ops.cell_fwd_onehot, base_xh, sw.dec_class, xf, no_ids,
+                     base_c[(time - 1) % 2], base_c[time % 2], base_h32, None, h, w, n)
         if cfg.use_gnn:
           ops.gnn_attend_fwd(h_src, scene_mean, nxt, h, w, ns, beam=b, row_map=row_map)
         else:
           ops.beam_gather_h(h_src, row_map, nxt, h, w, ns)
         self._cell("beam", (h, w, ns), ops.cell_fwd_onehot, nxt, sw.dec_class, xf, step_ids[time - 1].view(-1), c_src,
-                   c[1 - cur_c], h32, None, h, w, ns, row_map=row_map)
+                   c[1 - cur_c], h32, None, h, w, ns, row_map=row_map,
+                   tiles=(tiles, tile_count[time:time + 1]) if band else None)
+        if band:
+          ops.beam_band_copy(base_c[time % 2], base_h32, bands[1 - time % 2], c[1 - cur_c], h32, b, h, w)
       cur_c = 1 - cur_c
       h_src, c_src = h32, c[cur_c]
     out_ids = torch.empty((n, b, pred_len), dtype=torch.int32, device=dev)
@@ -386,7 +422,8 @@
     sf = feeds["scene_feat"]
     f_pad = -(-int(sf.shape[0]) // 64) * 64
     flat = self._flat_feeds(feeds)
-    key = (tp, f_pad) + tuple((k, tuple(t.shape[1:] if k == "scene_feat" else t.shape), t.dtype) for k, t in flat)
+    key = (tp, f_pad) + tuple((k, tuple(t.shape[1:] if k == "scene_feat" else t.shape), t.dtype) for k, t in flat) + \
+        (("MVB_BEAM_BAND", beam_band_on()),)
     ent = self._graphs.get(key)
     main = torch.cuda.current_stream(self.device)
     if ent is None:
diff --git a/multiverse_b200/ops.py b/multiverse_b200/ops.py
--- a/multiverse_b200/ops.py
+++ b/multiverse_b200/ops.py
@@ -171,16 +171,17 @@
 
 
 def cell_fwd_onehot(xh, packed, xf, ids, c_in, c_out, h32_out, xh_next, h, w, ns, row_map=None,
-                    forget_bias=1.0):
+                    forget_bias=1.0, tiles=None):
   hp = _hp_out(xh, packed, xh_next)
+  tl, tn = tiles if tiles is not None else (None, None)
   _lib.call("mvb_convlstm_cell_fwd_onehot", _p(xh), _p(packed.w), _p(xf.B), _p(xf.T2), _p(ids), _p(c_in),
-            _p(row_map), _p(c_out), _p(h32_out), *hp, ns, h, w, packed.cpad, _planes_arg(packed, xh_next),
-            float(forget_bias), _stream())
+            _p(row_map), _p(tl), _p(tn), _p(c_out), _p(h32_out), *hp, ns, h, w, packed.cpad,
+            _planes_arg(packed, xh_next), float(forget_bias), _stream())
 
 
 def cell_fwd_onehot_fanout(xh, packed, xf, ids, c_in, c_out, h32_out, h, w, ns, fanout, forget_bias=1.0,
                            workspace=None):
-  assert xh.shape[2] == packed.cpad and planes_of(xh) == packed.planes
+  assert xh is None and workspace is not None or xh.shape[2] == packed.cpad and planes_of(xh) == packed.planes
   if workspace is None:
     workspace = torch.empty((halo_rows(ns, h, w), 4 * HIDDEN), dtype=torch.float32, device=xh.device)
   assert workspace.numel() >= halo_rows(ns, h, w) * 4 * HIDDEN and workspace.dtype == torch.float32
@@ -289,6 +290,23 @@
   assert xh_next.shape[1] == halo_rows(ns, h, w) and row_map.dtype == torch.int32 and row_map.numel() == ns
   _lib.call("mvb_beam_gather_h_f16f8", _p(h32), _p(row_map), _p(xh_next), xh_next.stride(0), xh_next.shape[2], ns,
             h, w, _stream())
+
+
+def beam_band_capacity(ns, h, w):
+  return ns * (((h + 1) * (w + 1) + 127) // 128 + 1)
+
+
+def beam_band(ids, parents, band_in, band_out, tiles, tile_count, k, radius, h, w):
+  ns = ids.numel()
+  assert band_out.shape == (ns, 2) and band_out.dtype == torch.int32 and tiles.shape[1] == 2
+  _lib.call("mvb_beam_band", _p(ids), _p(parents), _p(band_in), _p(band_out), _p(tiles), tiles.shape[0],
+            _p(tile_count), ns, k, radius, h, w, _stream())
+
+
+def beam_band_copy(base_c, base_h32, band, c, h32, k, h, w):
+  ns = band.shape[0]
+  assert c.shape[0] == halo_rows(ns, h, w) and base_c.shape[0] * k == c.shape[0]
+  _lib.call("mvb_beam_band_copy", _p(base_c), _p(base_h32), _p(band), _p(c), _p(h32), ns, k, h, w, _stream())
 
 
 def beam_backtrace(step_ids, step_parents, step_logits, out_ids, out_logits):
```

Result: faster. 455.5 (median of 6 runs) (+22.9%).
